# chaofengc/FeMaSR

Hardware: AMD Instinct MI355X
Metric: SR output megapixels/sec at x4 (128->512) (higher is better)
Workload: dtype f32 (1x1 convs / nn.Linear: every fp32 operand split EXACTLY into three bf16 terms, six partial products, fp32 accumulation on the bf16 matrix pipe - closer to fp64 than the fp32 fmaf chain, bit-identical to the CPU oracle)

## Files before the change

femasr_amd/_lib.py:

```python
import ctypes
import os

_HERE = os.path.dirname(os.path.abspath(__file__))
SO_PATH = os.path.join(_HERE, 'csrc', 'libfemasr_hip.so')

c_int, c_i64, c_f32 = ctypes.c_int, ctypes.c_int64, ctypes.c_float
vp, szt = ctypes.c_void_p, ctypes.c_size_t


class FemasrError(RuntimeError):
    pass


MAX_CODEBOOKS = 3


class Config(ctypes.Structure):
    _fields_ = ([(n, ctypes.c_int32) for n in ('in_channel', 'gt_resolution', 'lq_stage', 'scale_factor', 'use_quantize',
                                               'use_residual', 'n_codebooks')] +
                [(n, ctypes.c_int32 * MAX_CODEBOOKS) for n in ('codebook_scale', 'n_e', 'e_dim')] +
                [('device', ctypes.c_int32)])


class ConvArgs(ctypes.Structure):
    _fields_ = [
        ('in_', vp), ('B', ctypes.c_int32), ('H', ctypes.c_int32), ('W', ctypes.c_int32), ('Cin', ctypes.c_int32),
        ('w', vp), ('bias', vp),
        ('Cout', ctypes.c_int32), ('ksz', ctypes.c_int32), ('stride', ctypes.c_int32), ('pad', ctypes.c_int32),
        ('up2', ctypes.c_int32), ('prologue', ctypes.c_int32),
        ('pro_a', vp), ('pro_b', vp), ('pro_c', vp),
        ('act', ctypes.c_int32),
        ('res1', vp), ('res2', vp), ('out', vp),
        ('Ho', ctypes.c_int32), ('Wo', ctypes.c_int32),
        ('w_bf16x3', vp), ('gn_part', vp), ('w_up2', vp), ('w_wino', vp), ('fast_act', ctypes.c_int32), ('in_add', vp), ('w_bf16s', vp),
    ]


ABI_VERSION = 106
PRO_NONE, PRO_GN_SILU, PRO_LN = 0, 1, 2
ACT_NONE, ACT_GELU, ACT_RELU = 0, 1, 2

SIGNATURES = {
    'femasr_last_error': (ctypes.c_char_p, []),
    'femasr_version': (c_int, []),
    'femasr_create': (c_int, [ctypes.POINTER(Config), ctypes.POINTER(vp)]),
    'femasr_destroy': (None, [vp]),
    'femasr_num_weights': (c_int, [vp]),
    'femasr_weight_info': (c_int, [vp, c_int, ctypes.POINTER(ctypes.c_char_p), ctypes.POINTER(c_i64 * 4), ctypes.POINTER(c_int)]),
    'femasr_set_weight': (c_int, [vp, ctypes.c_char_p, vp, ctypes.POINTER(c_i64), c_int]),
    'femasr_finalize_weights': (c_int, [vp]),
    'femasr_set_streams': (c_int, [vp, c_int]),
    'femasr_workspace_bytes': (c_int, [vp, c_int, c_int, c_int, c_int, ctypes.POINTER(szt)]),
    'femasr_forward_shapes': (c_int, [vp, c_int, c_int, c_int, ctypes.POINTER(c_int), ctypes.POINTER(c_int), ctypes.POINTER(c_int),
                                      ctypes.POINTER(c_int * MAX_CODEBOOKS), ctypes.POINTER(c_int * MAX_CODEBOOKS)]),
    'femasr_forward': (c_int, [vp, vp, vp, c_int, c_int, c_int, c_int, vp, vp, vp, szt]),
    'femasr_forward_u8': (c_int, [vp, vp, vp, c_int, c_int, c_int, c_int, c_int, vp, vp, vp, szt]),
    'femasr_pad_u8hwc_to_nhwc': (c_int, [vp, vp, c_int, c_int, c_int, c_int, c_int, c_int, vp]),
    'femasr_crop_nhwc_to_u8hwc': (c_int, [vp, vp, c_int, c_int, c_int, c_int, c_int, c_int, vp]),
    'femasr_decode_workspace_bytes': (c_int, [vp, c_int, c_int, c_int, ctypes.POINTER(szt)]),
    'femasr_decode_indices': (c_int, [vp, vp, vp, c_int, c_int, c_int, vp, vp, szt]),
    'femasr_profile_enable': (c_int, [vp, c_int]),
    'femasr_profile_reset': (c_int, [vp]),
    'femasr_profile_slots': (c_int, [vp]),
    'femasr_profile_name': (ctypes.c_char_p, [vp, c_int]),
    'femasr_profile_get': (c_int, [vp, c_int, ctypes.POINTER(ctypes.c_double), ctypes.POINTER(c_i64),
                                   ctypes.POINTER(ctypes.c_double), ctypes.POINTER(ctypes.c_double)]),
    'femasr_pad_nchw_to_nhwc': (c_int, [vp, vp, c_int, c_int, c_int, c_int, c_int, c_int, vp]),
    'femasr_crop_nhwc_to_nchw': (c_int, [vp, vp, c_int, c_int, c_int, c_int, c_int, c_int, vp]),
    'femasr_conv2d': (c_int, [vp, ctypes.POINTER(ConvArgs)]),
    'femasr_gn_coeffs': (c_int, [vp, vp, c_int, c_int, c_int, c_int, c_int, vp, vp, c_f32, vp, vp, vp]),
    'femasr_gn_coeffs_from_partials': (c_int, [vp, vp, c_int, c_int, c_int, c_int, c_int, c_int, vp, vp, c_f32, vp, vp]),
    'femasr_ln_stats': (c_int, [vp, vp, c_i64, c_int, c_f32, vp]),
    'femasr_layernorm': (c_int, [vp, vp, c_i64, c_int, vp, vp, c_f32, vp]),
    'femasr_gn_scratch_bytes': (szt, [c_int, c_int, c_int, c_int, c_int]),
    'femasr_window_attention': (c_int, [vp, vp, c_int, c_int, c_int, c_int, c_int, c_int, vp, vp]),
    'femasr_vq': (c_int, [vp, vp, c_i64, c_int, vp, vp, vp, c_int, vp, vp, vp]),
    'femasr_row_sqsum': (c_int, [vp, vp, c_i64, c_int, vp]),
    'femasr_vq_twopass_ok': (c_int, [c_int, c_int]),
    'femasr_vq_aux_bytes': (szt, [c_int, c_int]),
    'femasr_vq_prepare': (c_int, [vp, vp, vp, c_int, c_int, vp]),
    'femasr_vq_scratch_bytes': (szt, [c_i64, c_int]),
    'femasr_vq_twopass': (c_int, [vp, vp, c_i64, c_int, vp, vp, vp, c_int, vp, vp, vp]),
    'femasr_vq_candidates': (c_int, [vp, vp, c_i64, c_int, vp, vp, c_int, vp, vp]),
    'femasr_codebook_gather': (c_int, [vp, vp, c_i64, c_int, vp, c_int, vp]),
    'femasr_extract_tiles': (c_int, [vp, vp, c_int, c_int, c_int, c_int, vp, c_int, c_int, c_int, vp]),
    'femasr_paste_tiles': (c_int, [vp, vp, c_int, c_int, c_int, c_int, c_int, vp, c_int, c_int, c_int, vp]),
    'femasr_extract_tiles_u8': (c_int, [vp, vp, c_int, c_int, c_int, vp, c_int, c_int, c_int, vp]),
    'femasr_paste_tiles_u8': (c_int, [vp, vp, c_int, c_int, c_int, c_int, vp, c_int, c_int, c_int, vp]),
    'femasr_blend_tiles': (c_int, [vp, vp, vp, c_int, c_int, c_int, c_int, c_int, c_int, c_int, c_int, vp]),
    'femasr_blend_tiles_u8': (c_int, [vp, vp, vp, c_int, c_int, c_int, c_int, c_int, c_int, c_int, vp]),
    'femasr_concat_resize': (c_int, [vp, vp, c_int, vp, c_int, c_int, c_int, c_int, c_int, c_int, vp]),
    'femasr_repack_oihw': (c_int, [vp, vp, c_int, c_int, c_int, c_int, vp]),
    'femasr_packed_weight_floats': (szt, [c_int, c_int, c_int, c_int]),
    'femasr_up2_weight_floats': (szt, [c_int, c_int]),
    'femasr_wino_weight_floats': (szt, [c_int, c_int]),
    'femasr_repack_oihw_wino': (c_int, [vp, vp, c_int, c_int, vp]),
    'femasr_wino_up2_weight_floats': (szt, [c_int, c_int]),
    'femasr_repack_oihw_wino_up2': (c_int, [vp, vp, c_int, c_int, vp]),
    'femasr_repack_oihw_up2': (c_int, [vp, vp, c_int, c_int, vp]),
    'femasr_packed_weight_bf16x3_bytes': (szt, [c_int, c_int, c_int, c_int]),
    'femasr_repack_oihw_bf16x3': (c_int, [vp, vp, c_int, c_int, c_int, c_int, vp]),
    'femasr_set_decoder_math': (c_int, [vp, c_int]),
    'femasr_set_linear_math': (c_int, [vp, c_int]),
    'femasr_packed_weight_bf16s_bytes': (szt, [c_int, c_int]),
    'femasr_repack_k1_bf16s': (c_int, [vp, vp, c_int, c_int, vp]),
    'femasr_packed_weight_conv3x3_bf16s_bytes': (szt, [c_int, c_int]),
    'femasr_repack_oihw_bf16s': (c_int, [vp, vp, c_int, c_int, vp]),
    'femasr_gn_silu_apply': (c_int, [vp, vp, c_int, c_int, c_int, c_int, vp, vp, vp]),
    'femasr_image_u8_to_f32': (c_int, [vp, vp, c_int, c_int, c_int, vp]),
    'femasr_image_f32_to_u8': (c_int, [vp, vp, c_int, c_int, c_int, vp]),
    'femasr_lpips_create': (c_int, [c_int, c_int, ctypes.POINTER(vp)]),
    'femasr_lpips_destroy': (None, [vp]),
    'femasr_lpips_set_weight': (c_int, [vp, ctypes.c_char_p, vp, ctypes.POINTER(c_i64), c_int]),
    'femasr_lpips_finalize_weights': (c_int, [vp]),
    'femasr_lpips_workspace_bytes': (c_int, [vp, c_int, c_int, c_int, ctypes.POINTER(szt)]),
    'femasr_lpips_forward': (c_int, [vp, vp, vp, vp, c_int, c_int, c_int, vp, vp, vp, szt]),
    'femasr_lpips_scale_input': (c_int, [vp, vp, vp, c_int, c_int, c_int, vp]),
    'femasr_lpips_tap_partials': (c_int, [c_int, c_int]),
    'femasr_lpips_tap': (c_int, [vp, vp, c_int, c_int, c_int, c_int, vp, c_int, vp, vp]),
    'femasr_lpips_finalize': (c_int, [vp, vp, c_int, c_int, ctypes.POINTER(ctypes.c_int32), vp, vp]),
    'femasr_psnr_ssim_workspace_bytes': (c_int, [c_int, c_int, c_int, c_int, c_int, ctypes.POINTER(szt)]),
    'femasr_psnr_ssim': (c_int, [vp, vp, vp, c_int, c_int, c_int, c_int, c_int, vp, vp, vp, vp, szt]),
    'femasr_ssim_window': (c_int, [ctypes.POINTER(ctypes.c_double)]),
    'femasr_imresize_workspace_bytes': (c_int, [c_int, c_int, c_int, c_int, c_int, ctypes.POINTER(szt)]),
    'femasr_imresize': (c_int, [vp, vp, c_int, c_int, c_int, c_int, c_int, c_int, vp, vp, c_int, vp, vp, c_int, vp, vp, szt]),
    'femasr_niqe_workspace_bytes': (c_int, [c_int, c_int, c_int, c_int, ctypes.POINTER(szt)]),
    'femasr_niqe_plane_offsets': (c_int, [c_int, c_int, c_int, c_int, ctypes.POINTER(szt * 4)]),
    'femasr_niqe_features': (c_int, [vp, vp, c_int, c_int, c_int, c_int, vp, vp, vp, vp, c_int, vp, vp, c_int, vp, vp, vp, szt]),
    'femasr_clock_probe': (c_int, [vp, c_int, vp]),
    'femasr_clock_probe_entries': (c_int, []),
}
DEBUG_SIGNATURES = {
    'femasr_debug_set_wino_limits': (c_int, [vp, c_int, c_int]),
    'femasr_debug_mfma_bf16': (c_int, [vp, vp, vp, vp, c_int, vp]),
    'femasr_gemm_force_config': (c_int, [c_int]),
    'femasr_conv_small_launch_blocks': (c_int, [c_int]),
    'femasr_debug_conv_variant_name': (c_int, [ctypes.POINTER(ConvArgs), ctypes.c_char_p, c_int]),
}

_lib = None


def load():
    global _lib
    if _lib is not None:
        return _lib
    if not os.path.exists(SO_PATH):
        raise FemasrError(
            f'{SO_PATH} not found: the HIP extension is not built. Run `python femasr_amd/csrc/build.py` '
            '(needs hipcc; cross-compiles gfx950 without a GPU). There is no CPU fallback.')
    lib = ctypes.CDLL(SO_PATH)
    lib.femasr_version.restype = c_int
    if lib.femasr_version() != ABI_VERSION:
        raise FemasrError(f'{SO_PATH} reports ABI version {lib.femasr_version()}, this binding is written for {ABI_VERSION} '
                          '(femasr_conv_args layout): rebuild with `python femasr_amd/csrc/build.py --force`')
    for name, (res, args) in list(SIGNATURES.items()) + list(DEBUG_SIGNATURES.items()):
        fn = getattr(lib, name)
        fn.restype = res
        fn.argtypes = args
    _lib = lib
    return lib


def check(rc):
    if rc != 0:
        msg = load().femasr_last_error()
        raise FemasrError(f'libfemasr_hip error {rc}: {msg.decode() if msg else "?"}')


def ptr(t):
    return None if t is None else ctypes.c_void_p(t.data_ptr())
```

femasr_amd/csrc/common.h:

```cpp
#pragma once
#include <hip/hip_runtime.h>
#include <stdint.h>
#include <stddef.h>
#include "../../include/femasr_hip_debug.h"

int femasr_set_error(int code, const char *fmt, ...);
#define FEMASR_CHECK_HIP(expr)                                                            \
    do {                                                                                  \
        hipError_t _e = (expr);                                                           \
        if (_e != hipSuccess)                                                             \
            return femasr_set_error(FEMASR_ERR_HIP, "%s failed: %s (%s:%d)", #expr,       \
                                    hipGetErrorString(_e), __FILE__, __LINE__);           \
    } while (0)
#define FEMASR_REQUIRE(cond, ...)                                                         \
    do {                                                                                  \
        if (!(cond)) return femasr_set_error(FEMASR_ERR_INVALID, __VA_ARGS__);            \
    } while (0)

inline int femasr_allow_dynamic_lds(const void *kern, unsigned long long *devs, size_t bytes)
{
    int dev = 0;
    FEMASR_CHECK_HIP(hipGetDevice(&dev));
    if (dev < 0 || dev >= 64 || !((__atomic_load_n(devs, __ATOMIC_ACQUIRE) >> dev) & 1ull)) {
        FEMASR_CHECK_HIP(hipFuncSetAttribute(kern, hipFuncAttributeMaxDynamicSharedMemorySize, (int)bytes));
        if (dev >= 0 && dev < 64) __atomic_fetch_or(devs, 1ull << dev, __ATOMIC_RELEASE);
    }
    return FEMASR_OK;
}
#define FEMASR_CHECK(expr) do { const int _rc = (expr); if (_rc != FEMASR_OK) return _rc; } while (0)

struct conv_vq_epilogue {
    const float *zz;
    const float *ee;
    float *part;
    int nblk;
};
int femasr_conv2d_launch(hipStream_t s, const femasr_conv_args *a, const conv_vq_epilogue *vq,
                         int *variant_out, double *flops_out);
int femasr_conv2d_pick_variant(const femasr_conv_args *a);
int femasr_conv_variant_count();
const char *femasr_conv_variant_name(int v);
bool femasr_conv_halo_eligible(const femasr_conv_args *a);
inline bool femasr_gn_fusable(int cout) { const int cg = cout / 32; return cout % 32 == 0 && cg >= 1 && cg <= 32 && (cg & (cg - 1)) == 0; }

inline size_t femasr_compact_weight_floats(int O, int I, int kh, int kw)
{
    return (O <= 4 && kh == 3 && kw == 3 && (I % 32) == 0) ? (size_t)I * 9 * 4 : 0;
}

bool femasr_gemm_eligible(const femasr_conv_args *a);
int femasr_gemm_launch(hipStream_t s, const femasr_conv_args *a, const conv_vq_epilogue *vq, int *variant_out, double *flops_out);
int femasr_gemm_variant_count();
int femasr_gemm_pick_variant(const femasr_conv_args *a, bool vq);
const char *femasr_gemm_variant_name(int v);
int femasr_repack_k1(hipStream_t s, const float *in, int O, int I, float *out);

bool femasr_gemm_bf16s_shape_ok(const femasr_conv_args *a);
bool femasr_conv3x3_bf16s_shape_ok(const femasr_conv_args *a);
int femasr_gemm_bf16s_launch(hipStream_t s, const femasr_conv_args *a, const void *w_bf16s, int *variant_out, double *flops_out);
int femasr_gemm_bf16s_variant_count();
int femasr_gemm_bf16s_pick_variant(const femasr_conv_args *a);
const char *femasr_gemm_bf16s_variant_name(int v);

constexpr int FEMASR_WINO_LOG2_TOTAL = 31, FEMASR_WINO_LOG2_IMAGE = 27;
bool femasr_conv_wino_shape_ok(const femasr_conv_args *a);
bool femasr_conv_wino_shape_ok_lim(const femasr_conv_args *a, int log2_total, int log2_image);
int femasr_conv_wino_gn_tiles(int H, int W);
int femasr_conv_wino_launch(hipStream_t s, const femasr_conv_args *a, int *variant_out, double *flops_out);
int femasr_conv_wino_variant_count();
int femasr_conv_wino_pick_variant(const femasr_conv_args *a);
const char *femasr_conv_wino_variant_name(int v);
bool femasr_conv_wino_up2_shape_ok(const femasr_conv_args *a);
bool femasr_conv_wino_up2_shape_ok_lim(const femasr_conv_args *a, int log2_total, int log2_image);
int femasr_conv_wino_up2_launch(hipStream_t s, const femasr_conv_args *a, double *flops_out);
const char *femasr_conv_wino_up2_variant_name();

bool femasr_conv_bf16x3_eligible(const femasr_conv_args *a);
bool femasr_conv_bf16x3_shape_ok(const femasr_conv_args *a);
int femasr_conv_bf16x3_launch(hipStream_t s, const femasr_conv_args *a, int *variant_out, double *flops_out);
int femasr_conv_bf16x3_variant_count();
int femasr_conv_bf16x3_pick_variant(const femasr_conv_args *a);
const char *femasr_conv_bf16x3_variant_name(int v);

enum ConvForm {
    CONV_DIRECT,
    CONV_BF16X3,
    CONV_WINO,
    CONV_WINO_UP2,
    CONV_SPLIT,
    CONV_FORM_COUNT
};
int femasr_conv_form_variant_count(ConvForm f);
const char *femasr_conv_form_variant_name(ConvForm f, int v);
int femasr_conv_form_launch(hipStream_t s, ConvForm f, const femasr_conv_args *a, int *slot_out, double *flops_out);
```

femasr_amd/csrc/conv_common.h:

```cpp
#pragma once
#include "common.h"

namespace {

struct ConvParams {
    const float *in, *w, *bias, *pro_a, *pro_b, *pro_c, *res1, *res2;
    const float *w_wino;
    const float *w_up2;
    float *out;
    const float *vq_zz, *vq_ee;
    float *vq_part;
    int vq_nblk;
    double *gn_part;
    int B, H, W, Cin, Cout, ksz, stride, pad, up2, act, Ho, Wo;
    int M, K, nchunks, taps, MB, NB, NT32;
    int tilesX, tilesY;
    int kperm;
};

constexpr int BK = 32;
constexpr int ALD = BK + 1;

__device__ __forceinline__ float4 ld4(const float *p) { return *reinterpret_cast<const float4 *>(p); }

typedef __attribute__((address_space(1))) const float *gcptr_f32;
typedef __attribute__((address_space(1))) float *gptr_f32;

__device__ __forceinline__ unsigned long long uniform_u64(unsigned long long a)
{
    const unsigned lo = __builtin_amdgcn_readfirstlane((unsigned)a), hi = __builtin_amdgcn_readfirstlane((unsigned)(a >> 32));
    return ((unsigned long long)hi << 32) | lo;
}
__device__ __forceinline__ float ldg_u32(const float *ubase, unsigned byteoff)
{
    const unsigned long long a = uniform_u64(reinterpret_cast<unsigned long long>(ubase));
    return *reinterpret_cast<gcptr_f32>(a + byteoff);
}
__device__ __forceinline__ void stg_u32(float *ubase, unsigned byteoff, float v)
{
    const unsigned long long a = uniform_u64(reinterpret_cast<unsigned long long>(ubase));
    *reinterpret_cast<gptr_f32>(a + byteoff) = v;
}

typedef float f32x4_t __attribute__((ext_vector_type(4)));
__device__ __forceinline__ f32x4_t ldg4_u32(const float *ubase, unsigned byteoff)
{
    const unsigned long long a = uniform_u64(reinterpret_cast<unsigned long long>(ubase));
    return *reinterpret_cast<__attribute__((address_space(1))) const f32x4_t *>(a + byteoff);
}
__device__ __forceinline__ void stg4_u32(float *ubase, unsigned byteoff, f32x4_t v)
{
    const unsigned long long a = uniform_u64(reinterpret_cast<unsigned long long>(ubase));
    *reinterpret_cast<__attribute__((address_space(1))) f32x4_t *>(a + byteoff) = v;
}
constexpr int TPITCH = 36;
constexpr int TSCRATCH = 32 * TPITCH;

__device__ __forceinline__ float f4get(const float4 &v, int i) { return i == 0 ? v.x : (i == 1 ? v.y : (i == 2 ? v.z : v.w)); }

__device__ __forceinline__ int wtile(int n0, int t, int nt32)
{
    const int idx = (n0 >> 5) + t;
    return idx < nt32 ? idx : nt32 - 1;
}

__device__ __forceinline__ int xcd_remap(int bid, int nblk)
{
    const int q = nblk >> 3, r = nblk & 7, xcd = bid & 7, within = bid >> 3;
    return (xcd < r ? xcd * (q + 1) : r * (q + 1) + (xcd - r) * q) + within;
}


}
```

femasr_amd/csrc/kernels_conv.hip:

```cpp
#include "conv_common.h"
#include <atomic>
#include <stdlib.h>
#include <type_traits>
#include "detmath.h"

typedef float f32x16 __attribute__((ext_vector_type(16)));

namespace {


template <int BM, int BN, int WM, int WN, int PRO, bool CINVEC>
__global__ __launch_bounds__(WM * WN * 64, (WM * WN == 8) ? 4 : 2) void conv_igemm_kernel(const ConvParams p)
{
    constexpr int NT = WM * WN * 64;
    constexpr int TM = BM / (WM * 32), TN = BN / (WN * 32);
    constexpr int RSTEP = NT / 8;
    constexpr int AROWS = BM / RSTEP;
    static_assert((WM * WN == 4 || WM * WN == 8) && TM >= 1 && TN >= 1 && AROWS >= 1, "tile config");
    static_assert(CINVEC || PRO == FEMASR_PRO_NONE, "generic-Cin path has no prologue");
    static_assert(PRO != FEMASR_PRO_LN, "LayerNorm is a separate pass (femasr_layernorm)");

    extern __shared__ __attribute__((aligned(16))) float smem[];
    float *As = smem;

    const int t = threadIdx.x, lane = t & 63;
    const int wave = __builtin_amdgcn_readfirstlane(t >> 6);
    const int wm = wave / WN, wn = wave % WN;
    const int L = xcd_remap(blockIdx.x, p.MB * p.NB);
    const int nb = L % p.NB, mb = L / p.NB;
    const int m0 = mb * BM, n0 = nb * BN;

    const int kq = t & 7, mrow = t >> 3;
    int rn[AROWS], riy[AROWS], rix[AROWS];
    const int HoWo = p.Ho * p.Wo;
#pragma unroll
    for (int j = 0; j < AROWS; ++j) {
        const int r = m0 + mrow + RSTEP * j;
        if (r < p.M) {
            const int n = r / HoWo, rem = r - n * HoWo;
            const int oy = rem / p.Wo, ox = rem - oy * p.Wo;
            rn[j] = n;
            riy[j] = oy * p.stride - p.pad;
            rix[j] = ox * p.stride - p.pad;
        } else {
            rn[j] = 0;
            riy[j] = -(1 << 28);
            rix[j] = -(1 << 28);
        }
    }
    const int Hv = p.up2 ? 2 * p.H : p.H, Wv = p.up2 ? 2 * p.W : p.W;

    float4 ra[AROWS], rga[AROWS], rgb[AROWS];
    unsigned amask = 0;

    auto load_chunk = [&](int c) {
        amask = 0;
        if (CINVEC) {
            const int cc = c / p.taps, tap = c - cc * p.taps, c0 = cc * BK + 4 * kq;
            const int ky = tap / p.ksz, kx = tap - ky * p.ksz;
#pragma unroll
            for (int j = 0; j < AROWS; ++j) {
                const int iy = riy[j] + ky, ix = rix[j] + kx;
                const bool ok = (iy >= 0) & (iy < Hv) & (ix >= 0) & (ix < Wv);
                const int sy = p.up2 ? (iy >> 1) : iy, sx = p.up2 ? (ix >> 1) : ix;
                const size_t off = ok ? ((((size_t)rn[j] * p.H + sy) * p.W + sx) * p.Cin + c0) : (size_t)0;
                ra[j] = ld4(p.in + off);
                if (PRO == FEMASR_PRO_GN_SILU) {
                    rga[j] = ld4(p.pro_a + (size_t)rn[j] * p.Cin + c0);
                    rgb[j] = ld4(p.pro_b + (size_t)rn[j] * p.Cin + c0);
                }
                amask |= (ok ? 1u : 0u) << j;
            }
        } else {
#pragma unroll
            for (int j = 0; j < AROWS; ++j) {
                float v[4];
#pragma unroll
                for (int e = 0; e < 4; ++e) {
                    const int k = c * BK + 4 * kq + e;
                    v[e] = 0.f;
                    if (k < p.K) {
                        const int tap = k / p.Cin, ci = k - tap * p.Cin;
                        const int ky = tap / p.ksz, kx = tap - ky * p.ksz;
                        const int iy = riy[j] + ky, ix = rix[j] + kx;
                        if ((iy >= 0) & (iy < Hv) & (ix >= 0) & (ix < Wv)) {
                            const int sy = p.up2 ? (iy >> 1) : iy, sx = p.up2 ? (ix >> 1) : ix;
                            v[e] = p.in[(((size_t)rn[j] * p.H + sy) * p.W + sx) * p.Cin + ci];
                        }
                    }
                }
                ra[j] = make_float4(v[0], v[1], v[2], v[3]);
                amask |= 1u << j;
            }
        }
    };

    auto store_chunk = [&](int buf) {
        float *Ab = As + buf * BM * ALD;
#pragma unroll
        for (int j = 0; j < AROWS; ++j) {
            asm volatile("" : "+v"(ra[j].x), "+v"(ra[j].y), "+v"(ra[j].z), "+v"(ra[j].w));
            float4 v = ra[j];
            if (PRO == FEMASR_PRO_GN_SILU) {
                v.x = det_silu(__builtin_fmaf(v.x, rga[j].x, rgb[j].x));
                v.y = det_silu(__builtin_fmaf(v.y, rga[j].y, rgb[j].y));
                v.z = det_silu(__builtin_fmaf(v.z, rga[j].z, rgb[j].z));
                v.w = det_silu(__builtin_fmaf(v.w, rga[j].w, rgb[j].w));
            }
            if (!(amask & (1u << j))) v = make_float4(0.f, 0.f, 0.f, 0.f);
            float *dst = Ab + (mrow + RSTEP * j) * ALD + 4 * kq;
            dst[0] = v.x;
            dst[1] = v.y;
            dst[2] = v.z;
            dst[3] = v.w;
        }
    };

    f32x16 acc[TM][TN];
#pragma unroll
    for (int i = 0; i < TM; ++i)
#pragma unroll
        for (int j = 0; j < TN; ++j)
#pragma unroll
            for (int r = 0; r < 16; ++r) acc[i][j][r] = 0.f;

    const bool kp = p.kperm != 0;
    const int wgs = kp ? 256 : 4;
    const float *wl[TN];
#pragma unroll
    for (int j = 0; j < TN; ++j) {
        const size_t tile = (size_t)wtile(n0, wn * TN + j, p.NT32);
        wl[j] = kp ? p.w + tile * 1024 + lane * 4 : p.w + ((tile * 64 + lane) << 4);
    }
    const size_t wstride = (size_t)p.NT32 << 10;

    load_chunk(0);
    float4 bc[TN], bn[TN];
#pragma unroll
    for (int j = 0; j < TN; ++j) bc[j] = ld4(wl[j]);
    store_chunk(0);
    __syncthreads();

    const int arow = (wm * TM * 32 + (lane & 31)) * ALD + (kp ? 4 : 1) * (lane >> 5);
    auto kofs = [&](int kk) -> int { return kp ? 8 * (kk >> 2) + (kk & 3) : 2 * kk; };

    for (int c = 0; c < p.nchunks; ++c) {
        const int buf = c & 1;
        const int cn = (c + 1) < p.nchunks ? c + 1 : c;
        const float *Ab = As + buf * BM * ALD + arow;
        float af[2][TM];
#pragma unroll
        for (int i = 0; i < TM; ++i) af[0][i] = Ab[i * 32 * ALD];
#pragma unroll
        for (int kk = 0; kk < BK / 2; ++kk) {
            const int cur = kk & 1, nxt = cur ^ 1, g = kk >> 2, e = kk & 3;
            if (e == 0) {
                if (g < 3) {
#pragma unroll
                    for (int j = 0; j < TN; ++j) bn[j] = ld4(wl[j] + (size_t)c * wstride + wgs * (g + 1));
                } else {
#pragma unroll
                    for (int j = 0; j < TN; ++j) bn[j] = ld4(wl[j] + (size_t)cn * wstride);
                }
                if (kk == 0) load_chunk(cn);
            }
            if (kk + 1 < BK / 2) {
#pragma unroll
                for (int i = 0; i < TM; ++i) af[nxt][i] = Ab[i * 32 * ALD + kofs(kk + 1)];
            }
            __builtin_amdgcn_sched_barrier(0);
#pragma unroll
            for (int i = 0; i < TM; ++i)
#pragma unroll
                for (int j = 0; j < TN; ++j)
                    acc[i][j] = __builtin_amdgcn_mfma_f32_32x32x2f32(af[cur][i], f4get(bc[j], e), acc[i][j], 0, 0, 0);
            if (e == 3) {
#pragma unroll
                for (int j = 0; j < TN; ++j) bc[j] = bn[j];
            }
            __builtin_amdgcn_sched_barrier(0);
        }
        store_chunk(buf ^ 1);
        __syncthreads();
    }

    {
        const unsigned loff = (unsigned)((lane >> 5) * 4) * (unsigned)p.Cout + (unsigned)(lane & 31);
        const bool full = (m0 + BM <= p.M) && (n0 + BN <= p.Cout);
        const float *ra = p.res1 ? p.res1 : p.res2, *rb = (p.res1 && p.res2) ? p.res2 : nullptr;
        auto uoff = [&](int i, int j, int r) -> size_t {
            return (size_t)(m0 + (wm * TM + i) * 32 + (r & 3) + 8 * (r >> 2)) * p.Cout + (n0 + (wn * TN + j) * 32);
        };
        auto epilogue = [&](auto nres_c, auto full_c) {
            constexpr int NRES = decltype(nres_c)::value;
            constexpr bool FULL = decltype(full_c)::value;
            constexpr int DEPTH = NRES == 1 ? 2 : 1;
            float rbuf[DEPTH][NRES > 0 ? NRES : 1][16];
            auto ok_u = [&](int i, int j, int r) -> bool {
                return FULL || ((m0 + (wm * TM + i) * 32 + (r & 3) + 8 * (r >> 2)) < p.M && (n0 + (wn * TN + j) * 32) < p.Cout);
            };
            auto ok_l = [&](int i, int j, int r) -> bool {
                return FULL || ((m0 + (wm * TM + i) * 32 + (r & 3) + 8 * (r >> 2) + 4 * (lane >> 5)) < p.M &&
                                (n0 + (wn * TN + j) * 32 + (lane & 31)) < p.Cout);
            };
            auto issue = [&](int tl, int slot) {
#pragma unroll
                for (int r = 0; r < 16; ++r) {
                    const int i = tl / TN, j = tl % TN;
                    const size_t ou = ok_u(i, j, r) ? uoff(i, j, r) : (size_t)m0 * p.Cout + n0;
                    const unsigned lo = ok_l(i, j, r) ? 4u * loff : 0u;
                    if (NRES >= 1) rbuf[slot][0][r] = ldg_u32(ra + ou, lo);
                    if (NRES >= 2) rbuf[slot][NRES >= 2 ? 1 : 0][r] = ldg_u32(rb + ou, lo);
                }
            };
            if (NRES > 0) issue(0, 0);
#pragma unroll
            for (int tl = 0; tl < TM * TN; ++tl) {
                const int i = tl / TN, j = tl % TN;
                if (DEPTH == 2 && tl + 1 < TM * TN) issue(tl + 1, (tl + 1) & 1);
                const int col = n0 + (wn * TN + j) * 32 + (lane & 31);
                const float bv = (FULL || col < p.Cout) ? p.bias[FULL ? col : (col < p.Cout ? col : 0)] : 0.f;
#pragma unroll
                for (int r = 0; r < 16; ++r) {
                    float v = acc[i][j][r] + bv;
                    if (p.act == FEMASR_ACT_GELU) v = det_gelu(v);
                    else if (p.act == FEMASR_ACT_RELU) v = v > 0.f ? v : 0.f;
                    if (NRES >= 1) v = v + rbuf[tl % DEPTH][0][r];
                    if (NRES >= 2) v = v + rbuf[tl % DEPTH][NRES >= 2 ? 1 : 0][r];
                    if (ok_l(i, j, r)) stg_u32(p.out + uoff(i, j, r), 4u * loff, v);
                }
                if (NRES > 0 && DEPTH == 1 && tl + 1 < TM * TN) issue(tl + 1, 0);
            }
        };
        constexpr bool VEC_FITS = (WM * WN * TSCRATCH) <= (2 * BM * ALD);
        auto epilogue_vec = [&](auto nres_c) {
            constexpr int NRES = decltype(nres_c)::value;
            constexpr int DEPTH = NRES == 1 ? 2 : 1;
            float *T = smem + wave * TSCRATCH;
            const int trow = lane >> 3, tq = lane & 7;
            const unsigned lvec = 4u * ((unsigned)trow * (unsigned)p.Cout + 4u * (unsigned)tq);
            auto urow = [&](int i, int j, int k) -> size_t {
                return (size_t)(m0 + (wm * TM + i) * 32 + 8 * k) * p.Cout + (n0 + (wn * TN + j) * 32);
            };
            f32x4_t rbuf[DEPTH][NRES > 0 ? NRES : 1][4];
            auto issue = [&](int tl, int slot) {
#pragma unroll
                for (int k = 0; k < 4; ++k) {
                    if (NRES >= 1) rbuf[slot][0][k] = ldg4_u32(ra + urow(tl / TN, tl % TN, k), lvec);
                    if (NRES >= 2) rbuf[slot][NRES >= 2 ? 1 : 0][k] = ldg4_u32(rb + urow(tl / TN, tl % TN, k), lvec);
                }
            };
            if (NRES > 0) issue(0, 0);
#pragma unroll
            for (int tl = 0; tl < TM * TN; ++tl) {
                const int i = tl / TN, j = tl % TN;
                if (DEPTH == 2 && tl + 1 < TM * TN) issue(tl + 1, (tl + 1) & 1);
#pragma unroll
                for (int r = 0; r < 16; ++r) T[((r & 3) + 8 * (r >> 2) + 4 * (lane >> 5)) * TPITCH + (lane & 31)] = acc[i][j][r];
                const f32x4_t b4 = ldg4_u32(p.bias + n0 + (wn * TN + j) * 32, 16u * (unsigned)tq);
#pragma unroll
                for (int k = 0; k < 4; ++k) {
                    const float4 a4 = *reinterpret_cast<const float4 *>(T + (trow + 8 * k) * TPITCH + 4 * tq);
                    float v[4] = {a4.x + b4[0], a4.y + b4[1], a4.z + b4[2], a4.w + b4[3]};
                    if (p.act == FEMASR_ACT_GELU) {
                        const det_f32x2 g0 = det_gelu2(det_f32x2{v[0], v[1]}), g1 = det_gelu2(det_f32x2{v[2], v[3]});
                        v[0] = g0[0]; v[1] = g0[1]; v[2] = g1[0]; v[3] = g1[1];
                    } else if (p.act == FEMASR_ACT_RELU) {
#pragma unroll
                        for (int e = 0; e < 4; ++e) v[e] = v[e] > 0.f ? v[e] : 0.f;
                    }
#pragma unroll
                    for (int e = 0; e < 4; ++e) {
                        if (NRES >= 1) v[e] = v[e] + rbuf[tl % DEPTH][0][k][e];
                        if (NRES >= 2) v[e] = v[e] + rbuf[tl % DEPTH][NRES >= 2 ? 1 : 0][k][e];
                    }
                    stg4_u32(p.out + urow(i, j, k), lvec, f32x4_t{v[0], v[1], v[2], v[3]});
                }
                if (NRES > 0 && DEPTH == 1 && tl + 1 < TM * TN) issue(tl + 1, 0);
            }
        };
        using I0 = std::integral_constant<int, 0>;
        using I1 = std::integral_constant<int, 1>;
        using I2 = std::integral_constant<int, 2>;
        if (VEC_FITS && full && (p.Cout & 3) == 0) {
            if (rb) epilogue_vec(I2{}); else if (ra) epilogue_vec(I1{}); else epilogue_vec(I0{});
        } else if (rb) { if (full) epilogue(I2{}, std::true_type{}); else epilogue(I2{}, std::false_type{}); }
        else if (ra) { if (full) epilogue(I1{}, std::true_type{}); else epilogue(I1{}, std::false_type{}); }
        else { if (full) epilogue(I0{}, std::true_type{}); else epilogue(I0{}, std::false_type{}); }
    }
}

template <int BN, int WM, int WN, int PRO, bool UP2>
__global__ __launch_bounds__(WM * WN * 64, (WM * WN == 8) ? 4 : 2) void conv3x3_halo_kernel(const ConvParams p)
{
    constexpr int BM = 128, TW = 16;
    constexpr int PH = 10, PW = 18, PP = PH * PW;
    constexpr int NTAP = UP2 ? 4 : 9, SC = UP2 ? 2 : 1;
    static_assert(!(UP2 && PRO != FEMASR_PRO_NONE), "the phase kernel has no prologue");
    constexpr int NT = WM * WN * 64;
    constexpr int PUNITS = (PP * 8 + NT - 1) / NT;
    constexpr int PROWS = NT / 8;
    constexpr int TM = BM / (WM * 32), TN = BN / (WN * 32);
    static_assert((WM * WN == 4 || WM * WN == 8) && TM >= 1 && TN >= 1, "tile config");
    static_assert(PRO != FEMASR_PRO_LN, "no LayerNorm prologue on 3x3 convs");
    static_assert(2 + PUNITS <= BK / 2, "patch slices must fit the 16 k-pair steps of one tap");

    extern __shared__ __attribute__((aligned(16))) float smem[];
    constexpr int PSZ = (((PP + 1) * ALD + 3) / 4) * 4;
    float *Ps = smem;

    const int t = threadIdx.x, lane = t & 63, wave = t >> 6;
    const int wm = wave / WN, wn = wave % WN;
    const int L = xcd_remap(blockIdx.x, p.MB * p.NB);
    const int nb = L % p.NB;
    int tile = L / p.NB;
    const int pha = UP2 ? (tile >> 1) & 1 : 0, phb = UP2 ? tile & 1 : 0;
    if (UP2) tile >>= 2;
    const int tx = tile % p.tilesX;
    tile /= p.tilesX;
    const int ty = tile % p.tilesY;
    const int n = tile / p.tilesY;
    const int oy0 = ty * 8, ox0 = tx * TW, n0 = nb * BN;
    const int sy0 = oy0 - 1, sx0 = ox0 - 1;

    const int kq = t & 7;
    unsigned poff[PUNITS];
    unsigned pmask = 0;
#pragma unroll
    for (int i = 0; i < PUNITS; ++i) {
        const int pix = (t >> 3) + PROWS * i;
        const int ppy = pix / PW, ppx = pix - ppy * PW;
        const int sy = sy0 + ppy, sx = sx0 + ppx;
        const bool ok = (pix < PP) & (sy >= 0) & (sy < p.H) & (sx >= 0) & (sx < p.W);
        poff[i] = ok ? (unsigned)((((size_t)n * p.H + sy) * p.W + sx) * p.Cin + 4 * kq) : 0u;
        pmask |= (ok ? 1u : 0u) << i;
    }

    float4 rp[PUNITS], ga, gb;

    auto load_patch = [&](int cc) {
#pragma unroll
        for (int i = 0; i < PUNITS; ++i) rp[i] = ld4(p.in + (size_t)poff[i] + (size_t)cc * BK);
        if (PRO == FEMASR_PRO_GN_SILU) {
            ga = ld4(p.pro_a + (size_t)n * p.Cin + cc * BK + 4 * kq);
            gb = ld4(p.pro_b + (size_t)n * p.Cin + cc * BK + 4 * kq);
        }
    };
    auto store_patch_unit = [&](int buf, int i) {
        float *Pb = Ps + buf * PSZ;
        const int pix = (t >> 3) + PROWS * i;
        if (PP % PROWS != 0 && i == PUNITS - 1 && pix >= PP) return;
        float4 v = rp[i];
        if (PRO == FEMASR_PRO_GN_SILU) {
            const det_f32x2 s0 = det_silu2(__builtin_elementwise_fma(det_f32x2{v.x, v.y}, det_f32x2{ga.x, ga.y}, det_f32x2{gb.x, gb.y}));
            const det_f32x2 s1 = det_silu2(__builtin_elementwise_fma(det_f32x2{v.z, v.w}, det_f32x2{ga.z, ga.w}, det_f32x2{gb.z, gb.w}));
            v = make_float4(s0[0], s0[1], s1[0], s1[1]);
        }
        if (!(pmask & (1u << i))) v = make_float4(0.f, 0.f, 0.f, 0.f);
        float *dst = Pb + pix * ALD + 4 * kq;
        dst[0] = v.x;
        dst[1] = v.y;
        dst[2] = v.z;
        dst[3] = v.w;
    };

    f32x16 acc[TM][TN];
#pragma unroll
    for (int i = 0; i < TM; ++i)
#pragma unroll
        for (int j = 0; j < TN; ++j)
#pragma unroll
            for (int r = 0; r < 16; ++r) acc[i][j][r] = 0.f;

    const size_t wstride = (size_t)p.NT32 << 10;
    const float *wbase = UP2 ? p.w_up2 + (size_t)(pha * 2 + phb) * ((size_t)(p.Cin / BK) * NTAP) * wstride : p.w;
    const float *wl[TN];
#pragma unroll
    for (int j = 0; j < TN; ++j)
        wl[j] = wbase + ((((size_t)wtile(n0, wn * TN + j, p.NT32)) * 64 + lane) << 4);

    const int ncc = p.Cin / BK;
    load_patch(0);
    float4 bc[TN], bn[TN];
#pragma unroll
    for (int j = 0; j < TN; ++j) bc[j] = ld4(wl[j]);
#pragma unroll
    for (int i = 0; i < PUNITS; ++i) store_patch_unit(0, i);
    __syncthreads();

    int py[TM], px;
    {
        const int m = wm * TM * 32 + (lane & 31);
        px = m & 15;
#pragma unroll
        for (int i = 0; i < TM; ++i) py[i] = (m >> 4) + 2 * i;
    }

    const int abase = ((py[0] + pha) * PW + px + phb) * ALD;
    auto patch_idx = [&](int tap, int (&idx)[TM]) {
        const int ky = UP2 ? tap >> 1 : tap / 3, kx = UP2 ? tap & 1 : tap - ky * 3;
#pragma unroll
        for (int i = 0; i < TM; ++i) idx[i] = abase + ((2 * i + ky) * PW + kx) * ALD;
    };

    const int nq = ncc * NTAP;
    for (int cc = 0; cc < ncc; ++cc) {
        const float *Pb = Ps + (cc & 1) * PSZ + (lane >> 5);
        const int ccn = cc + 1 < ncc ? cc + 1 : cc;
        const bool more = cc + 1 < ncc;
        const int nbuf = (cc + 1) & 1;
        float af[2][TM];
        int aidx[TM];
        patch_idx(0, aidx);
#pragma unroll
        for (int i = 0; i < TM; ++i) af[0][i] = Pb[aidx[i]];
#pragma unroll
        for (int tap = 0; tap < NTAP; ++tap) {
            const int q = cc * NTAP + tap;
            const size_t qn = (size_t)(q + 1 < nq ? q + 1 : nq - 1);
            int nidx[TM];
            patch_idx(tap < NTAP - 1 ? tap + 1 : NTAP - 1, nidx);
#pragma unroll
            for (int kk = 0; kk < BK / 2; ++kk) {
                const int cur = kk & 1, nxt = cur ^ 1, g = kk >> 2, e = kk & 3;
                if (e == 0) {
                    if (g < 3) {
#pragma unroll
                        for (int j = 0; j < TN; ++j) bn[j] = ld4(wl[j] + (size_t)q * wstride + 4 * (g + 1));
                    } else {
#pragma unroll
                        for (int j = 0; j < TN; ++j) bn[j] = ld4(wl[j] + qn * wstride);
                    }
                    if (tap == 0 && kk == 0) load_patch(ccn);
                }
                if (kk + 1 < BK / 2) {
#pragma unroll
                    for (int i = 0; i < TM; ++i) af[nxt][i] = Pb[aidx[i] + 2 * (kk + 1)];
                } else if (tap < NTAP - 1) {
#pragma unroll
                    for (int i = 0; i < TM; ++i) af[nxt][i] = Pb[nidx[i]];
                }
                __builtin_amdgcn_sched_barrier(0);
#pragma unroll
                for (int i = 0; i < TM; ++i)
#pragma unroll
                    for (int j = 0; j < TN; ++j)
                        acc[i][j] = __builtin_amdgcn_mfma_f32_32x32x2f32(af[cur][i], f4get(bc[j], e), acc[i][j], 0, 0, 0);
                if (e == 3) {
#pragma unroll
                    for (int j = 0; j < TN; ++j) bc[j] = bn[j];
                }
                if (tap == 1 && kk >= 2 && kk < 2 + PUNITS && more) store_patch_unit(nbuf, kk - 2);
                __builtin_amdgcn_sched_barrier(0);
            }
#pragma unroll
            for (int i = 0; i < TM; ++i) aidx[i] = nidx[i];
        }
        __syncthreads();
    }

    const int Hl = UP2 ? p.H : p.Ho, Wl = UP2 ? p.W : p.Wo;
    const bool full = (oy0 + 8 <= Hl) && (ox0 + TW <= Wl) && (n0 + BN <= p.Cout);
    const float *ra = p.res1 ? p.res1 : p.res2, *rb = (p.res1 && p.res2) ? p.res2 : nullptr;
    const size_t obase = (((size_t)n * p.Ho + SC * oy0 + pha) * p.Wo + SC * ox0 + phb) * p.Cout + n0;
    const unsigned loff = (unsigned)(SC * 4 * (lane >> 5)) * (unsigned)p.Cout + (unsigned)(lane & 31);
    const int wmu = __builtin_amdgcn_readfirstlane(wm), wnu = __builtin_amdgcn_readfirstlane(wn);
    auto uoff = [&](int i, int j, int r) -> size_t {
        return obase + (size_t)(SC * ((2 * (wmu * TM + i) + (r >> 3)) * p.Wo + (r & 3) + 8 * ((r >> 2) & 1))) * p.Cout + (wnu * TN + j) * 32;
    };
    const bool gnp = p.gn_part != nullptr;
    double gs[TM][TN], gss[TM][TN];
#pragma unroll
    for (int i = 0; i < TM; ++i)
#pragma unroll
        for (int j = 0; j < TN; ++j) { gs[i][j] = 0.0; gss[i][j] = 0.0; }
    auto epilogue = [&](auto nres_c, auto full_c) {
        constexpr int NRES = decltype(nres_c)::value;
        constexpr bool FULL = decltype(full_c)::value;
        constexpr int DEPTH = NRES == 1 ? 2 : 1;
        float rbuf[DEPTH][NRES > 0 ? NRES : 1][16];
        auto ok_u = [&](int i, int j, int r) -> bool {
            return FULL || ((oy0 + 2 * (wmu * TM + i) + (r >> 3)) < Hl && (ox0 + (r & 3) + 8 * ((r >> 2) & 1)) < Wl &&
                            (n0 + (wnu * TN + j) * 32) < p.Cout);
        };
        auto ok_l = [&](int i, int j, int r) -> bool {
            return FULL || ((oy0 + 2 * (wmu * TM + i) + (r >> 3)) < Hl &&
                            (ox0 + (r & 3) + 8 * ((r >> 2) & 1) + 4 * (lane >> 5)) < Wl &&
                            (n0 + (wnu * TN + j) * 32 + (lane & 31)) < p.Cout);
        };
        auto issue = [&](int tl, int slot) {
#pragma unroll
            for (int r = 0; r < 16; ++r) {
                const int i = tl / TN, j = tl % TN;
                const size_t ou = ok_u(i, j, r) ? uoff(i, j, r) : obase;
                const unsigned lo = ok_l(i, j, r) ? 4u * loff : 0u;
                if (NRES >= 1) rbuf[slot][0][r] = ldg_u32(ra + ou, lo);
                if (NRES >= 2) rbuf[slot][NRES >= 2 ? 1 : 0][r] = ldg_u32(rb + ou, lo);
            }
        };
        if (NRES > 0) issue(0, 0);
#pragma unroll
        for (int tl = 0; tl < TM * TN; ++tl) {
            const int i = tl / TN, j = tl % TN;
            if (DEPTH == 2 && tl + 1 < TM * TN) issue(tl + 1, (tl + 1) & 1);
            const int col = n0 + (wnu * TN + j) * 32 + (lane & 31);
            const float bv = (FULL || col < p.Cout) ? p.bias[FULL ? col : (col < p.Cout ? col : 0)] : 0.f;
#pragma unroll
            for (int r = 0; r < 16; ++r) {
                float v = acc[i][j][r] + bv;
                if (p.act == FEMASR_ACT_RELU) v = v > 0.f ? v : 0.f;
                if (NRES >= 1) v = v + rbuf[tl % DEPTH][0][r];
                if (NRES >= 2) v = v + rbuf[tl % DEPTH][NRES >= 2 ? 1 : 0][r];
                if (ok_l(i, j, r)) {
                    stg_u32(p.out + uoff(i, j, r), 4u * loff, v);
                    if (gnp) {
                        const double d = (double)v;
                        gs[i][j] = gs[i][j] + d;
                        gss[i][j] = __builtin_fma(d, d, gss[i][j]);
                    }
                }
            }
            if (NRES > 0 && DEPTH == 1 && tl + 1 < TM * TN) issue(tl + 1, 0);
        }
    };
    using I0 = std::integral_constant<int, 0>;
    using I1 = std::integral_constant<int, 1>;
    using I2 = std::integral_constant<int, 2>;
    if (rb) { if (full) epilogue(I2{}, std::true_type{}); else epilogue(I2{}, std::false_type{}); }
    else if (ra) { if (full) epilogue(I1{}, std::true_type{}); else epilogue(I1{}, std::false_type{}); }
    else { if (full) epilogue(I0{}, std::true_type{}); else epilogue(I0{}, std::false_type{}); }

    if (gnp) {
        const int cg = p.Cout >> 5;
        const int gpb = BN / cg;
        double *red = reinterpret_cast<double *>(smem);
#pragma unroll
        for (int i = 0; i < TM; ++i)
#pragma unroll
            for (int j = 0; j < TN; ++j) {
                double a = gs[i][j] + __shfl_xor(gs[i][j], 32, 64);
                double b = gss[i][j] + __shfl_xor(gss[i][j], 32, 64);
                for (int d = 1; d < cg; d <<= 1) {
                    a = a + __shfl_xor(a, d, 64);
                    b = b + __shfl_xor(b, d, 64);
                }
                const int cl = (wnu * TN + j) * 32 + (lane & 31);
                if (lane < 32 && (cl & (cg - 1)) == 0) {
                    double *dst = red + ((size_t)(wmu * TM + i) * gpb + cl / cg) * 2;
                    dst[0] = a;
                    dst[1] = b;
                }
            }
        __syncthreads();
        if (t < gpb) {
            const int g = n0 / cg + t;
            if (g < 32) {
                double S = red[(0 * gpb + t) * 2], SS = red[(0 * gpb + t) * 2 + 1];
#pragma unroll
                for (int q = 1; q < 4; ++q) {
                    S = S + red[((size_t)q * gpb + t) * 2];
                    SS = SS + red[((size_t)q * gpb + t) * 2 + 1];
                }
                const size_t tidx = (size_t)n * p.tilesY * p.tilesX + (size_t)ty * p.tilesX + tx;
                double *dst = p.gn_part + ((UP2 ? tidx * 4 + (pha * 2 + phb) : tidx) * 32 + g) * 2;
                dst[0] = S;
                dst[1] = SS;
            }
        }
    }
}

constexpr int C3_TH = 8, C3_TW = 32, C3_PW = C3_TW + 2, C3_PP = (C3_TH + 2) * C3_PW, C3_PITCH = 36;

__global__ __launch_bounds__(256) void conv3x3_cout3_kernel(const ConvParams p, const float *__restrict__ wc)
{
    extern __shared__ __attribute__((aligned(16))) float smem[];
    const int t = threadIdx.x;
    int tile = blockIdx.x;
    const int tx = tile % p.tilesX;
    tile /= p.tilesX;
    const int ty = tile % p.tilesY;
    const int n = tile / p.tilesY;
    const int oy0 = ty * C3_TH, ox0 = tx * C3_TW;
    const int py = t >> 5, px = t & 31;
    float acc0 = 0.f, acc1 = 0.f, acc2 = 0.f;
    const int ncb = p.Cin >> 5;
    constexpr int NU = (C3_PP * 8 + 255) / 256;
    unsigned uoff[NU];
    unsigned umask = 0;
#pragma unroll
    for (int i = 0; i < NU; ++i) {
        const int u = t + 256 * i, pix = u >> 3, kq = u & 7;
        const int sy = oy0 - 1 + pix / C3_PW, sx = ox0 - 1 + pix % C3_PW;
        const bool ok = u < C3_PP * 8 && sy >= 0 && sy < p.H && sx >= 0 && sx < p.W;
        uoff[i] = ok ? (unsigned)((((size_t)n * p.H + sy) * p.W + sx) * p.Cin + 4 * kq) : 0u;
        umask |= (ok ? 1u : 0u) << i;
    }
    float4 ru[NU];
    auto fetch = [&](int cb) {
#pragma unroll
        for (int i = 0; i < NU; ++i) ru[i] = ld4(p.in + (size_t)uoff[i] + cb * 32);
    };
    auto stage = [&]() {
#pragma unroll
        for (int i = 0; i < NU; ++i) {
            const int u = t + 256 * i;
            if (u < C3_PP * 8)
                *reinterpret_cast<float4 *>(smem + (u >> 3) * C3_PITCH + 4 * (u & 7)) = (umask >> i) & 1u ? ru[i] : make_float4(0.f, 0.f, 0.f, 0.f);
        }
    };
    fetch(0);
    for (int cb = 0; cb < ncb; ++cb) {
        if (cb) __syncthreads();
        stage();
        __syncthreads();
        fetch(cb + 1 < ncb ? cb + 1 : cb);
#pragma unroll
        for (int tap = 0; tap < 9; ++tap) {
            const float *src = smem + ((py + tap / 3) * C3_PW + px + tap % 3) * C3_PITCH;
            const float *w = wc + ((size_t)(cb * 9 + tap) * 32) * 4;
#pragma unroll
            for (int c4 = 0; c4 < 8; ++c4) {
                const float4 x4 = *reinterpret_cast<const float4 *>(src + 4 * c4);
                const float xs[4] = {x4.x, x4.y, x4.z, x4.w};
#pragma unroll
                for (int e = 0; e < 4; ++e) {
                    const float *wk = w + (4 * c4 + e) * 4;
                    acc0 = __builtin_fmaf(xs[e], wk[0], acc0);
                    acc1 = __builtin_fmaf(xs[e], wk[1], acc1);
                    acc2 = __builtin_fmaf(xs[e], wk[2], acc2);
                }
            }
        }
    }
    const int oy = oy0 + py, ox = ox0 + px;
    if (oy < p.Ho && ox < p.Wo) {
        const size_t o = (((size_t)n * p.Ho + oy) * p.Wo + ox) * 3;
        float v[3] = {acc0 + p.bias[0], acc1 + p.bias[1], acc2 + p.bias[2]};
#pragma unroll
        for (int c = 0; c < 3; ++c) {
            if (p.res1) v[c] = v[c] + p.res1[o + c];
            if (p.res2) v[c] = v[c] + p.res2[o + c];
            p.out[o + c] = v[c];
        }
    }
}

template <bool UP2>
constexpr size_t halo_lds_bytes()
{
    return (size_t)(2 * ((((180 + 1) * ALD + 3) / 4) * 4)) * sizeof(float);
}

template <int BM>
constexpr size_t conv_lds_bytes() { return (size_t)(2 * BM * ALD) * sizeof(float); }

struct Variant {
    const char *name;
    int bm, bn;
    void (*kern)(const ConvParams);
    size_t lds;
    unsigned long long attr_devs;
    int threads;
};

#define FEMASR_VARIANT(BM, BN, WM, WN, PRO, VEC)                                                            \
    { "conv_igemm<" #BM "x" #BN "," #PRO ",cinvec=" #VEC ",waves=" #WM "x" #WN ">",                         \
      BM, BN, conv_igemm_kernel<BM, BN, WM, WN, PRO, VEC>, conv_lds_bytes<BM>(), 0ull, WM * WN * 64 }
#define FEMASR_HALO(BN, WM, WN, PRO, UP2)                                                                  \
    { "conv3x3_halo<8x16x" #BN "," #PRO ",up2=" #UP2 ",waves=" #WM "x" #WN ">", 128, BN,                   \
      conv3x3_halo_kernel<BN, WM, WN, PRO, UP2>, halo_lds_bytes<UP2>(), 0ull, WM * WN * 64 }

Variant g_variants[] = {
    FEMASR_VARIANT(128, 128, 4, 2, FEMASR_PRO_NONE, true),
    FEMASR_VARIANT(128, 128, 4, 2, FEMASR_PRO_GN_SILU, true),
    FEMASR_VARIANT(128, 64, 4, 2, FEMASR_PRO_NONE, true),
    FEMASR_VARIANT(128, 64, 4, 2, FEMASR_PRO_GN_SILU, true),
    FEMASR_VARIANT(128, 32, 4, 1, FEMASR_PRO_NONE, true),
    FEMASR_VARIANT(128, 32, 4, 1, FEMASR_PRO_GN_SILU, true),
    FEMASR_VARIANT(128, 128, 4, 2, FEMASR_PRO_NONE, false),
    FEMASR_VARIANT(128, 64, 4, 2, FEMASR_PRO_NONE, false),
    FEMASR_VARIANT(128, 32, 4, 1, FEMASR_PRO_NONE, false),
    FEMASR_HALO(128, 2, 2, FEMASR_PRO_NONE, false),
    FEMASR_HALO(128, 2, 2, FEMASR_PRO_GN_SILU, false),
    FEMASR_HALO(128, 2, 2, FEMASR_PRO_NONE, true),
    FEMASR_HALO(64, 2, 2, FEMASR_PRO_NONE, false),
    FEMASR_HALO(64, 2, 2, FEMASR_PRO_GN_SILU, false),
    FEMASR_HALO(64, 2, 2, FEMASR_PRO_NONE, true),
    FEMASR_HALO(32, 4, 1, FEMASR_PRO_NONE, false),
    FEMASR_HALO(32, 4, 1, FEMASR_PRO_GN_SILU, false),
    FEMASR_HALO(32, 4, 1, FEMASR_PRO_NONE, true),
    { "conv3x3_cout3<8x32,valu>", 256, 4, nullptr, (size_t)C3_PP * C3_PITCH * sizeof(float), 0ull, 256 },
};
constexpr int kNumVariants = sizeof(g_variants) / sizeof(g_variants[0]);
constexpr int kFirstHalo = 9;

std::atomic<int> g_small_blocks{-1};
int small_blocks_default()
{
    static const int v = [] {
        int dev = 0, cus = 0;
        if (hipGetDevice(&dev) == hipSuccess && hipDeviceGetAttribute(&cus, hipDeviceAttributeMultiprocessorCount, dev) == hipSuccess && cus > 0)
            return cus + cus / 2;
        return 384;
    }();
    return v;
}
int small_launch_blocks()
{
    const int v = g_small_blocks.load(std::memory_order_relaxed);
    return v >= 0 ? v : small_blocks_default();
}

int pick_variant(const femasr_conv_args *a, int Ho, int Wo)
{
    const bool vec = (a->Cin % BK) == 0;
    int cls = a->Cout > 64 ? 0 : (a->Cout > 32 ? 1 : 2);
    const bool halo = femasr_conv_halo_eligible(a);
    if (cls == 0 && (halo || vec)) {
        const long long mb = halo ? (long long)a->B * (((a->up2 ? a->W : Wo) + 15) / 16) * (((a->up2 ? a->H : Ho) + 7) / 8) * (a->up2 ? 4 : 1)
                                  : ((long long)a->B * Ho * Wo + 127) / 128;
        if (mb * ((a->Cout + 127) / 128) < small_launch_blocks()) cls = 1;
    }
    if (halo) return kFirstHalo + cls * 3 + (a->up2 ? 2 : a->prologue);
    if (!vec) return 6 + cls;
    return cls * 2 + a->prologue;
}

}

extern "C" int femasr_conv_small_launch_blocks(int blocks)
{
    const int prev = small_launch_blocks();
    g_small_blocks.store(blocks >= 0 ? blocks : -1, std::memory_order_relaxed);
    return prev;
}

bool femasr_conv_halo_eligible(const femasr_conv_args *a)
{
    return a->ksz == 3 && a->stride == 1 && a->pad == 1 && (a->Cin % BK) == 0 && a->prologue != FEMASR_PRO_LN &&
           (a->act == FEMASR_ACT_NONE || a->act == FEMASR_ACT_RELU) && !(a->up2 && a->prologue != FEMASR_PRO_NONE) &&
           (size_t)a->B * a->H * a->W * a->Cin < ((size_t)1 << 31);
}

int femasr_conv_variant_count() { return kNumVariants + femasr_gemm_variant_count(); }
const char *femasr_conv_variant_name(int v)
{
    if (v >= kNumVariants) return femasr_gemm_variant_name(v - kNumVariants);
    return v >= 0 ? g_variants[v].name : "?";
}

static bool conv_is_cout3(const femasr_conv_args *a)
{
    return femasr_conv_halo_eligible(a) && a->Cout == 3 && !a->up2 && a->prologue == FEMASR_PRO_NONE && a->act == FEMASR_ACT_NONE && !a->gn_part;
}

int femasr_conv2d_pick_variant(const femasr_conv_args *a)
{
    if (femasr_gemm_eligible(a)) return kNumVariants + femasr_gemm_pick_variant(a, false);
    if (conv_is_cout3(a)) return kNumVariants - 1;
    const int Hv = a->up2 ? 2 * a->H : a->H, Wv = a->up2 ? 2 * a->W : a->W;
    return pick_variant(a, (Hv + 2 * a->pad - a->ksz) / a->stride + 1, (Wv + 2 * a->pad - a->ksz) / a->stride + 1);
}

int femasr_conv2d_launch(hipStream_t s, const femasr_conv_args *a, const conv_vq_epilogue *vq,
                         int *variant_out, double *flops_out)
{
    FEMASR_REQUIRE(a && a->in && a->w && a->B > 0 && a->H > 0 && a->W > 0 && a->Cin > 0 && a->Cout > 0,
                   "conv2d: null pointer or empty shape");
    FEMASR_REQUIRE(vq || (a->bias && a->out), "conv2d: bias/out must be set");
    FEMASR_REQUIRE(a->ksz >= 1 && a->ksz <= 11 && (a->stride == 1 || a->stride == 2 || a->stride == 4) && a->pad >= 0,
                   "conv2d: unsupported ksz=%d stride=%d pad=%d", a->ksz, a->stride, a->pad);
    FEMASR_REQUIRE(a->act == FEMASR_ACT_NONE || a->act == FEMASR_ACT_GELU || a->act == FEMASR_ACT_RELU, "conv2d: bad activation %d", a->act);
    FEMASR_REQUIRE(a->prologue == FEMASR_PRO_NONE || a->prologue == FEMASR_PRO_GN_SILU,
                   "conv2d: bad prologue %d (LayerNorm is a separate pass: femasr_layernorm)", a->prologue);
    const int Hv = a->up2 ? 2 * a->H : a->H, Wv = a->up2 ? 2 * a->W : a->W;
    const int Ho = (Hv + 2 * a->pad - a->ksz) / a->stride + 1, Wo = (Wv + 2 * a->pad - a->ksz) / a->stride + 1;
    FEMASR_REQUIRE(Ho == a->Ho && Wo == a->Wo, "conv2d: Ho/Wo mismatch (%d,%d) vs expected (%d,%d)", a->Ho, a->Wo, Ho, Wo);
    if (femasr_gemm_eligible(a)) {
        int gv = 0;
        const int rc = femasr_gemm_launch(s, a, vq, &gv, flops_out);
        if (variant_out) *variant_out = kNumVariants + gv;
        return rc;
    }
    FEMASR_REQUIRE(!vq, "conv2d: the VQ epilogue needs a 1x1 layer with Cin %% 32 == 0");
    const bool vec = (a->Cin % BK) == 0;
    FEMASR_REQUIRE(vec || a->prologue == FEMASR_PRO_NONE, "conv2d: prologue needs Cin %% 32 == 0 (Cin=%d)", a->Cin);
    if (a->prologue == FEMASR_PRO_GN_SILU) FEMASR_REQUIRE(a->pro_a && a->pro_b, "conv2d: GN prologue needs a,b");
    const long long M = (long long)a->B * Ho * Wo;
    FEMASR_REQUIRE(M < (1ll << 31) - 256, "conv2d: too many output pixels");

    ConvParams p{};
    p.in = a->in; p.w = a->w; p.bias = a->bias; p.pro_a = a->pro_a; p.pro_b = a->pro_b; p.pro_c = a->pro_c;
    p.res1 = a->res1; p.res2 = a->res2; p.out = a->out;
    p.B = a->B; p.H = a->H; p.W = a->W; p.Cin = a->Cin; p.Cout = a->Cout; p.ksz = a->ksz; p.stride = a->stride;
    p.pad = a->pad; p.up2 = a->up2; p.act = a->act; p.Ho = Ho; p.Wo = Wo;
    p.M = (int)M; p.K = a->ksz * a->ksz * a->Cin; p.nchunks = (p.K + BK - 1) / BK; p.taps = a->ksz * a->ksz;
    p.NT32 = (a->Cout + 31) / 32;
    p.gn_part = a->gn_part;
    p.kperm = (a->ksz == 1 && vec) ? 1 : 0;
    if (conv_is_cout3(a)) {
        const size_t tail = femasr_compact_weight_floats(a->Cout, a->Cin, 3, 3);
        const float *wc = a->w + (size_t)p.nchunks * p.NT32 * 1024;
        p.tilesX = (Wo + C3_TW - 1) / C3_TW;
        p.tilesY = (Ho + C3_TH - 1) / C3_TH;
        (void)tail;
        hipLaunchKernelGGL(conv3x3_cout3_kernel, dim3((unsigned)(a->B * p.tilesX * p.tilesY)), dim3(256), (size_t)C3_PP * C3_PITCH * sizeof(float), s,
                           p, wc);
        FEMASR_CHECK_HIP(hipGetLastError());
        if (variant_out) *variant_out = kNumVariants - 1;
        if (flops_out) *flops_out = 2.0 * (double)M * (double)a->Cout * (double)p.K;
        return FEMASR_OK;
    }
    const int vi = pick_variant(a, Ho, Wo);
    Variant &v = g_variants[vi];
    p.MB = (p.M + v.bm - 1) / v.bm;
    p.NB = (p.Cout + v.bn - 1) / v.bn;
    const bool phases = vi >= kFirstHalo && a->up2;
    if (vi >= kFirstHalo) {
        p.tilesX = ((phases ? a->W : Wo) + 15) / 16;
        p.tilesY = ((phases ? a->H : Ho) + 7) / 8;
        p.MB = a->B * p.tilesX * p.tilesY * (phases ? 4 : 1);
    }
    FEMASR_REQUIRE(!phases || a->w_up2, "conv2d: a 3x3 nearest-x2 conv with Cin %% 32 == 0 needs w_up2 (femasr_repack_oihw_up2)");
    p.w_up2 = a->w_up2;
    FEMASR_REQUIRE(!a->gn_part || (vi >= kFirstHalo && femasr_gn_fusable(a->Cout)),
                   "conv2d: gn_part (fused GroupNorm partial moments) needs a 3x3 stride-1 halo conv and 32 | Cout, Cout/32 a power of two <= 32");
    FEMASR_CHECK(femasr_allow_dynamic_lds((const void *)v.kern, &v.attr_devs, v.lds));
    hipLaunchKernelGGL(v.kern, dim3((unsigned)(p.MB * p.NB)), dim3((unsigned)v.threads), v.lds, s, p);
    FEMASR_CHECK_HIP(hipGetLastError());
    if (variant_out) *variant_out = vi;
    if (flops_out) *flops_out = 2.0 * (double)M * (double)a->Cout * (double)p.K;
    return FEMASR_OK;
}
```

femasr_amd/csrc/kernels_misc.hip:

```cpp
#include "common.h"
#include "detmath.h"
#include <stdlib.h>
#include <string.h>
#include <type_traits>

namespace {

__device__ __forceinline__ float4 ld4(const float *p) { return *reinterpret_cast<const float4 *>(p); }

__device__ __forceinline__ int xcd_remap_misc(int bid, int nblk)
{
    const int q = nblk >> 3, r = nblk & 7, xcd = bid & 7, within = bid >> 3;
    return (xcd < r ? xcd * (q + 1) : r * (q + 1) + (xcd - r) * q) + within;
}

__global__ void pad_nchw_to_nhwc_kernel(const float *__restrict__ in, int B, int C, int H, int W, int Hp, int Wp,
                                        float *__restrict__ out, size_t total)
{
    for (size_t i = blockIdx.x * (size_t)blockDim.x + threadIdx.x; i < total; i += (size_t)gridDim.x * blockDim.x) {
        const int c = (int)(i % C);
        size_t r = i / C;
        const int x = (int)(r % Wp);
        r /= Wp;
        const int y = (int)(r % Hp);
// ... 843 lines not shown
    FEMASR_REQUIRE(x && gamma && beta && a && b && scratch, "gn_coeffs: null pointer");
    FEMASR_REQUIRE(B > 0 && H > 0 && W > 0 && G > 0 && C % G == 0, "gn_coeffs: bad shape C=%d G=%d", C, G);
    const int cg = C / G;
    hipStream_t s = (hipStream_t)stream;
    double *part = (double *)scratch;
    if (G == 32 && femasr_gn_fusable(C)) {
        const int tilesX = (W + 15) / 16, tilesY = (H + 7) / 8;
        hipLaunchKernelGGL(gn_tile_partials_kernel, dim3((unsigned)((size_t)B * tilesY * tilesX * (C / 32))), dim3(64), 0, s, x, H, W, C,
                           tilesX, tilesY, part);
        FEMASR_CHECK_HIP(hipGetLastError());
        return femasr_gn_coeffs_from_partials(stream, part, B, tilesX * tilesY, H, W, C, G, gamma, beta, eps, a, b);
    }
    const size_t total = (size_t)B * H * G;
    const dim3 grid((unsigned)((total + 255) / 256)), blk(256);
    if (cg == 8 && C % 4 == 0)
        hipLaunchKernelGGL(gn_rows_kernel<8>, grid, blk, 0, s, x, B, H, W, C, G, part);
    else if (cg == 4 && C % 4 == 0)
        hipLaunchKernelGGL(gn_rows_kernel<4>, grid, blk, 0, s, x, B, H, W, C, G, part);
    else if (cg == 2)
        hipLaunchKernelGGL(gn_rows_kernel<2>, grid, blk, 0, s, x, B, H, W, C, G, part);
    else
        hipLaunchKernelGGL(gn_rows_generic_kernel, grid, blk, 0, s, x, B, H, W, C, G, cg, part);
    FEMASR_CHECK_HIP(hipGetLastError());
    FEMASR_REQUIRE(G <= 256, "gn_coeffs: at most 256 groups");
    hipLaunchKernelGGL(gn_finalize_kernel, dim3((unsigned)B), dim3(256), (size_t)GN_SLAB * G * 2 * sizeof(double), s, part, B, H, H,
                       W, C, G, gamma, beta, eps, a, b);
    FEMASR_CHECK_HIP(hipGetLastError());
    return FEMASR_OK;
}

int femasr_gn_coeffs_from_partials(void *stream, const double *part, int B, int tiles, int H, int W, int C, int G,
                                   const float *gamma, const float *beta, float eps, float *a, float *b)
{
    FEMASR_REQUIRE(part && gamma && beta && a && b && B > 0 && tiles > 0 && H > 0 && W > 0, "gn_coeffs_from_partials: bad args");
    FEMASR_REQUIRE(G == 32 && C % G == 0, "gn_coeffs_from_partials: 32 groups");
    FEMASR_REQUIRE(C / G <= 64, "gn_coeffs_from_partials: at most 64 channels per group");
    hipLaunchKernelGGL(gn_finalize_partials_kernel, dim3((unsigned)(B * G)), dim3(64), 0, (hipStream_t)stream, part, tiles, H, W, C,
                       G, gamma, beta, eps, a, b);
    FEMASR_CHECK_HIP(hipGetLastError());
    return FEMASR_OK;
}

int femasr_gn_silu_apply(void *stream, const float *x, int B, int H, int W, int C, const float *a, const float *b, float *y)
{
    FEMASR_REQUIRE(x && a && b && y && B > 0 && H > 0 && W > 0 && C > 0 && (C % 4) == 0, "gn_silu_apply: bad args (C %% 4 == 0)");
    const size_t total4 = (size_t)B * H * W * (C / 4);
    hipLaunchKernelGGL(gn_silu_apply_kernel, dim3(grid_for(total4)), dim3(256), 0, (hipStream_t)stream, x, C, (long long)H * W, a, b, y, total4);
    FEMASR_CHECK_HIP(hipGetLastError());
    return FEMASR_OK;
}

int femasr_ln_stats(void *stream, const float *x, int64_t rows, int C, float eps, float *stats)
{
    FEMASR_REQUIRE(x && stats && rows > 0, "ln_stats: bad args");
    FEMASR_REQUIRE(C == 256, "ln_stats: only C == 256 (Swin embed_dim, femasr_arch.py:115) is built, got %d", C);
    hipLaunchKernelGGL(ln_stats_kernel, dim3((unsigned)((rows + 3) / 4)), dim3(256), 0, (hipStream_t)stream, x,
                       (long long)rows, eps, stats);
    FEMASR_CHECK_HIP(hipGetLastError());
    return FEMASR_OK;
}

int femasr_layernorm(void *stream, const float *x, int64_t rows, int C, const float *gamma, const float *beta, float eps, float *y)
{
    FEMASR_REQUIRE(x && y && gamma && beta && rows > 0, "layernorm: bad args");
    FEMASR_REQUIRE(C == 256, "layernorm: only C == 256 (Swin embed_dim, femasr_arch.py:115) is built, got %d", C);
    hipLaunchKernelGGL(layernorm_kernel, dim3((unsigned)((rows + 3) / 4)), dim3(256), 0, (hipStream_t)stream, x, (long long)rows,
                       gamma, beta, eps, y);
    FEMASR_CHECK_HIP(hipGetLastError());
    return FEMASR_OK;
}

int femasr_window_attention(void *stream, const float *qkv, int B, int H, int W, int C, int heads, int shift,
                            const float *table, float *out)
{
    FEMASR_REQUIRE(qkv && table && out && B > 0, "window_attention: bad args");
    FEMASR_REQUIRE(H % 8 == 0 && W % 8 == 0 && H >= 8 && W >= 8, "window_attention: H,W must be multiples of 8 (%d,%d)", H, W);
    FEMASR_REQUIRE(heads > 0 && heads <= 8 && C == heads * ATT_HD, "window_attention: head_dim must be 32, at most 8 heads (C=%d heads=%d)", C, heads);
    FEMASR_REQUIRE(shift >= 0 && shift < 8, "window_attention: bad shift %d", shift);
    FEMASR_REQUIRE((size_t)H * W * 3 * C < ((size_t)1 << 30), "window_attention: image too large for 32-bit offsets");
    const size_t total = (size_t)B * (H / 8) * (W / 8) * heads;
    FEMASR_REQUIRE(total < ((size_t)1 << 31), "window_attention: too many (window, head) units");
    hipLaunchKernelGGL(window_attention_reg_kernel<1>, dim3((unsigned)total), dim3(64), 0, (hipStream_t)stream, qkv, B, H, W, C, heads, shift, table,
                       out, (int)total);
    FEMASR_CHECK_HIP(hipGetLastError());
    return FEMASR_OK;
}

int femasr_row_sqsum(void *stream, const float *x, int64_t rows, int D, float *out)
{
    FEMASR_REQUIRE(x && out && rows > 0 && D > 0 && D % 4 == 0, "row_sqsum: bad args");
    hipLaunchKernelGGL(row_sqsum_kernel, dim3((unsigned)((rows + 63) / 64)), dim3(64), 0, (hipStream_t)stream, x,
                       (long long)rows, D, out);
    FEMASR_CHECK_HIP(hipGetLastError());
    return FEMASR_OK;
}

int femasr_vq(void *stream, const float *z, int64_t M, int D, const float *cb, const float *cbT, const float *ee,
              int n_e, int64_t *idx, float *zq, void *scratch)
{
    FEMASR_REQUIRE(z && cb && cbT && ee && idx && zq && scratch && M > 0, "vq: bad args");
    FEMASR_REQUIRE(D % 32 == 0 && n_e % 128 == 0, "vq: needs e_dim %% 32 == 0 and n_e %% 128 == 0 (D=%d n_e=%d)", D, n_e);
    FEMASR_REQUIRE(M < (1ll << 31) - 256, "vq: too many rows");
    hipStream_t s = (hipStream_t)stream;
    float *zz = (float *)scratch;
    float *part = zz + ((M + 63) / 64) * 64;
    const int nblk = n_e / 128;
    int rc = femasr_row_sqsum(stream, z, M, D, zz);
    if (rc) return rc;
    femasr_conv_args a{};
    a.in = z; a.B = 1; a.H = (int)M; a.W = 1; a.Cin = D; a.w = cbT; a.bias = nullptr; a.Cout = n_e;
    a.ksz = 1; a.stride = 1; a.pad = 0; a.up2 = 0; a.prologue = FEMASR_PRO_NONE; a.act = 0;
    a.Ho = (int)M; a.Wo = 1;
    conv_vq_epilogue ep{zz, ee, part, nblk};
    rc = femasr_conv2d_launch(s, &a, &ep, nullptr, nullptr);
    if (rc) return rc;
    hipLaunchKernelGGL(vq_finalize_kernel, dim3((unsigned)((M + 3) / 4)), dim3(256), 0, s, z, (long long)M, D, cb, part,
                       nblk, n_e, (long long *)idx, zq);
    FEMASR_CHECK_HIP(hipGetLastError());
    return FEMASR_OK;
}

int femasr_codebook_gather(void *stream, const int64_t *idx, int64_t M, int D, const float *cb, int n_e, float *zq)
{
    FEMASR_REQUIRE(idx && cb && zq && M > 0 && D % 4 == 0 && n_e > 0, "codebook_gather: bad args");
    hipLaunchKernelGGL(codebook_gather_kernel, dim3((unsigned)((M + 3) / 4)), dim3(256), 0, (hipStream_t)stream,
                       (const long long *)idx, (long long)M, D, cb, n_e, zq);
    FEMASR_CHECK_HIP(hipGetLastError());
    return FEMASR_OK;
}

int femasr_extract_tiles(void *stream, const float *in, int B, int C, int H, int W, const int32_t *yx_dev, int n, int th, int tw, float *out)
{
    FEMASR_REQUIRE(in && yx_dev && out && B > 0 && C > 0 && n > 0 && th > 0 && tw > 0 && th <= H && tw <= W, "extract_tiles: bad args");
    const size_t total = (size_t)n * B * C * th * tw;
    hipLaunchKernelGGL(extract_tiles_kernel, dim3(grid_for(total)), dim3(256), 0, (hipStream_t)stream, in, B, C, H, W, yx_dev, n, th, tw, out, total);
    FEMASR_CHECK_HIP(hipGetLastError());
    return FEMASR_OK;
}

int femasr_paste_tiles(void *stream, const float *tiles, int B, int C, int n, int th, int tw, const int32_t *rects_dev, int hmax,
                       int Ho, int Wo, float *out)
{
    FEMASR_REQUIRE(tiles && rects_dev && out && B > 0 && C > 0 && n > 0 && th > 0 && tw > 0 && hmax > 0 && hmax <= th, "paste_tiles: bad args");
    const size_t rows = (size_t)n * B * C * hmax;
    FEMASR_REQUIRE(rows < ((size_t)1 << 31), "paste_tiles: too many rows");
    hipLaunchKernelGGL(paste_tiles_kernel, dim3((unsigned)rows), dim3(256), 0, (hipStream_t)stream, tiles, B, C, th, tw, rects_dev, n, Ho, Wo, out, hmax);
    FEMASR_CHECK_HIP(hipGetLastError());
    return FEMASR_OK;
}

int femasr_extract_tiles_u8(void *stream, const uint8_t *in, int B, int H, int W, const int32_t *yx_dev, int n, int th, int tw, uint8_t *out)
{
    FEMASR_REQUIRE(in && yx_dev && out && B > 0 && n > 0 && th > 0 && tw > 0 && th <= H && tw <= W, "extract_tiles_u8: bad args");
    const size_t total = (size_t)n * B * th * tw * 3;
    hipLaunchKernelGGL(extract_tiles_u8_kernel, dim3(grid_for(total)), dim3(256), 0, (hipStream_t)stream, in, B, H, W, yx_dev, n, th, tw, out, total);
    FEMASR_CHECK_HIP(hipGetLastError());
    return FEMASR_OK;
}

int femasr_paste_tiles_u8(void *stream, const uint8_t *tiles, int B, int n, int th, int tw, const int32_t *rects_dev, int hmax, int Ho, int Wo, uint8_t *out)
{
    FEMASR_REQUIRE(tiles && rects_dev && out && B > 0 && n > 0 && th > 0 && tw > 0 && hmax > 0 && hmax <= th, "paste_tiles_u8: bad args");
    const size_t rows = (size_t)n * B * hmax;
    FEMASR_REQUIRE(rows < ((size_t)1 << 31), "paste_tiles_u8: too many rows");
    hipLaunchKernelGGL(paste_tiles_u8_kernel, dim3((unsigned)rows), dim3(256), 0, (hipStream_t)stream, tiles, B, th, tw, rects_dev, n, Ho, Wo, out, hmax);
    FEMASR_CHECK_HIP(hipGetLastError());
    return FEMASR_OK;
}

static int blend_launch(bool u8, void *stream, const uint64_t *tile_ptrs_dev, const int32_t *geom_dev, int n, int tiles_y, int tiles_x,
                        int pitch, int B, int C, int Ho, int Wo, void *out)
{
    const char *who = u8 ? "blend_tiles_u8" : "blend_tiles";
    FEMASR_REQUIRE(tile_ptrs_dev && geom_dev && out, "%s: null pointer", who);
    FEMASR_REQUIRE(n > 0 && B > 0 && C > 0 && tiles_y > 0 && tiles_x > 0 && pitch > 0 && Ho > 0 && Wo > 0, "%s: bad sizes", who);
    FEMASR_REQUIRE((long long)tiles_y * tiles_x == n, "%s: %d tiles given for a %d x %d grid", who, n, tiles_y, tiles_x);
    FEMASR_REQUIRE(tiles_x <= 65535, "%s: more than 65535 tile columns", who);
    const size_t rows = (size_t)B * C * Ho;
    FEMASR_REQUIRE(rows < ((size_t)1 << 31), "%s: too many rows", who);
    const dim3 grid((unsigned)rows, (unsigned)tiles_x);
    if (u8)
        hipLaunchKernelGGL(blend_tiles_kernel<true>, grid, dim3(256), 0, (hipStream_t)stream, (const unsigned long long *)tile_ptrs_dev,
                           geom_dev, tiles_y, tiles_x, pitch, 1, Ho, Wo, out);
    else
        hipLaunchKernelGGL(blend_tiles_kernel<false>, grid, dim3(256), 0, (hipStream_t)stream, (const unsigned long long *)tile_ptrs_dev,
                           geom_dev, tiles_y, tiles_x, pitch, C, Ho, Wo, out);
    FEMASR_CHECK_HIP(hipGetLastError());
    return FEMASR_OK;
}

int femasr_blend_tiles(void *stream, const uint64_t *tile_ptrs_dev, const int32_t *geom_dev, int n, int tiles_y, int tiles_x, int pitch,
                       int B, int C, int Ho, int Wo, float *out)
{
    return blend_launch(false, stream, tile_ptrs_dev, geom_dev, n, tiles_y, tiles_x, pitch, B, C, Ho, Wo, out);
}

int femasr_blend_tiles_u8(void *stream, const uint64_t *tile_ptrs_dev, const int32_t *geom_dev, int n, int tiles_y, int tiles_x, int pitch,
                          int B, int Ho, int Wo, uint8_t *out)
{
    return blend_launch(true, stream, tile_ptrs_dev, geom_dev, n, tiles_y, tiles_x, pitch, B, 1, Ho, Wo, out);
}

int femasr_concat_resize(void *stream, const float *a, int Ca, const float *b, int Hb, int Wb, int Cb, int B, int H, int W, float *out)
{
    FEMASR_REQUIRE(a && b && out && B > 0 && H > 0 && W > 0 && Hb > 0 && Wb > 0, "concat_resize: bad args");
    FEMASR_REQUIRE(Ca > 0 && Cb > 0 && Ca % 4 == 0 && Cb % 4 == 0, "concat_resize: channel counts must be multiples of 4 (%d, %d)", Ca, Cb);
    const size_t total4 = (size_t)B * H * W * ((Ca + Cb) / 4);
    hipLaunchKernelGGL(concat_resize_kernel, dim3(grid_for(total4)), dim3(256), 0, (hipStream_t)stream, a, Ca, b, Hb, Wb, Cb, H, W, out,
                       total4);
    FEMASR_CHECK_HIP(hipGetLastError());
    return FEMASR_OK;
}

size_t femasr_packed_weight_floats(int O, int I, int kh, int kw)
{
    if (O <= 0 || I <= 0 || kh <= 0 || kw <= 0) return 0;
    const size_t K = (size_t)I * kh * kw;
    return ((K + 31) / 32) * (size_t)((O + 31) / 32) * 1024 + femasr_compact_weight_floats(O, I, kh, kw);
}

int femasr_repack_oihw(void *stream, const float *in, int O, int I, int kh, int kw, float *out)
{
    FEMASR_REQUIRE(in && out && O > 0 && I > 0 && kh > 0 && kw > 0, "repack: bad args");
    if (kh == 1 && kw == 1 && (I % 32) == 0) return femasr_repack_k1((hipStream_t)stream, in, O, I, out);
    const size_t tail = femasr_compact_weight_floats(O, I, kh, kw);
    const size_t total = femasr_packed_weight_floats(O, I, kh, kw) - tail;
    if (tail) {
        hipLaunchKernelGGL(repack_compact_kernel, dim3(grid_for(tail)), dim3(256), 0, (hipStream_t)stream, in, O, I, kh, kw, out + total, tail);
        FEMASR_CHECK_HIP(hipGetLastError());
    }
    hipLaunchKernelGGL(repack_oihw_kernel, dim3(grid_for(total)), dim3(256), 0, (hipStream_t)stream, in, O, I, kh, kw, out,
                       total);
    FEMASR_CHECK_HIP(hipGetLastError());
    return FEMASR_OK;
}

size_t femasr_up2_weight_floats(int O, int I)
{
    return (I % 32) == 0 ? 4 * femasr_packed_weight_floats(O, I, 2, 2) : 0;
}

int femasr_repack_oihw_up2(void *stream, const float *in, int O, int I, float *out)
{
    FEMASR_REQUIRE(in && out && O > 0 && I > 0 && (I % 32) == 0, "repack_up2: needs a 3x3 OIHW weight with I %% 32 == 0");
    const size_t per = femasr_packed_weight_floats(O, I, 2, 2);
    hipLaunchKernelGGL(repack_up2_kernel, dim3(grid_for(4 * per)), dim3(256), 0, (hipStream_t)stream, in, O, I, out, per);
    FEMASR_CHECK_HIP(hipGetLastError());
    return FEMASR_OK;
}

int femasr_image_u8_to_f32(void *stream, const uint8_t *in_hwc, int H, int W, int swap_rb, float *out_chw)
{
    FEMASR_REQUIRE(in_hwc && out_chw && H > 0 && W > 0, "image_u8_to_f32: bad args");
    const size_t total = (size_t)3 * H * W;
    hipLaunchKernelGGL(image_u8_to_f32_kernel, dim3(grid_for(total)), dim3(256), 0, (hipStream_t)stream, in_hwc, H, W,
                       swap_rb, out_chw, total);
    FEMASR_CHECK_HIP(hipGetLastError());
    return FEMASR_OK;
}

int femasr_image_f32_to_u8(void *stream, const float *in_chw, int H, int W, int swap_rb, uint8_t *out_hwc)
{
    FEMASR_REQUIRE(in_chw && out_hwc && H > 0 && W > 0, "image_f32_to_u8: bad args");
    const size_t total = (size_t)3 * H * W;
    hipLaunchKernelGGL(image_f32_to_u8_kernel, dim3(grid_for(total)), dim3(256), 0, (hipStream_t)stream, in_chw, H, W,
                       swap_rb, out_hwc, total);
    FEMASR_CHECK_HIP(hipGetLastError());
    return FEMASR_OK;
}

int femasr_clock_probe_entries(void) { return FEMASR_CLOCK_PROBE_BLOCKS * 4; }

int femasr_clock_probe(void *stream, int mfmas_per_wave, unsigned long long *ticks)
{
    FEMASR_REQUIRE(ticks && mfmas_per_wave >= 4, "clock_probe: bad args");
    hipLaunchKernelGGL(clock_probe_kernel, dim3(FEMASR_CLOCK_PROBE_BLOCKS), dim3(256), 0, (hipStream_t)stream, mfmas_per_wave / 4, 1.0001f, 0.5f, ticks);
    FEMASR_CHECK_HIP(hipGetLastError());
    return FEMASR_OK;
}

}

int femasr_conv_form_variant_count(ConvForm f)
{
    const int n[CONV_FORM_COUNT] = {femasr_conv_variant_count(), femasr_conv_bf16x3_variant_count(), femasr_conv_wino_variant_count(), 1,
                                    femasr_gemm_bf16s_variant_count()};
    return n[f];
}

const char *femasr_conv_form_variant_name(ConvForm f, int v)
{
    switch (f) {
    case CONV_BF16X3: return femasr_conv_bf16x3_variant_name(v);
    case CONV_WINO: return femasr_conv_wino_variant_name(v);
    case CONV_WINO_UP2: return femasr_conv_wino_up2_variant_name();
    case CONV_SPLIT: return femasr_gemm_bf16s_variant_name(v);
    default: return femasr_conv_variant_name(v);
    }
}

int femasr_conv_form_launch(hipStream_t s, ConvForm f, const femasr_conv_args *a, int *slot_out, double *flops_out)
{
    int v = 0, r;
    switch (f) {
    case CONV_BF16X3: r = femasr_conv_bf16x3_launch(s, a, &v, flops_out); break;
    case CONV_WINO: r = femasr_conv_wino_launch(s, a, &v, flops_out); break;
    case CONV_WINO_UP2: r = femasr_conv_wino_up2_launch(s, a, flops_out); break;
    case CONV_SPLIT: r = femasr_gemm_bf16s_launch(s, a, a->w_bf16s, &v, flops_out); break;
    default: r = femasr_conv2d_launch(s, a, nullptr, &v, flops_out); break;
    }
    for (int g = 0; g < f; ++g) v += femasr_conv_form_variant_count((ConvForm)g);
    if (slot_out) *slot_out = v;
    return r;
}

static ConvForm conv2d_form(const femasr_conv_args *a)
{
    return !a ? CONV_DIRECT : a->w_bf16s ? CONV_SPLIT : a->w_bf16x3 ? CONV_BF16X3 : !a->w_wino ? CONV_DIRECT : a->up2 ? CONV_WINO_UP2 : CONV_WINO;
}

extern "C" int femasr_debug_conv_variant_name(const femasr_conv_args *a, char *name, int cap)
{
    FEMASR_REQUIRE(a && name && cap > 0, "debug_conv_variant_name: bad args");
    FEMASR_REQUIRE(a->B > 0 && a->H > 0 && a->W > 0 && a->Cin > 0 && a->Cout > 0 && a->ksz >= 1 && a->ksz <= 11 &&
                   (a->stride == 1 || a->stride == 2 || a->stride == 4) && a->pad >= 0,
                   "debug_conv_variant_name: empty shape or unsupported ksz=%d stride=%d pad=%d", a->ksz, a->stride, a->pad);
    const ConvForm f = conv2d_form(a);
    int v = 0;
    switch (f) {
    case CONV_BF16X3: v = femasr_conv_bf16x3_pick_variant(a); break;
    case CONV_WINO: v = femasr_conv_wino_pick_variant(a); break;
    case CONV_WINO_UP2: v = 0; break;
    case CONV_SPLIT: v = femasr_gemm_bf16s_pick_variant(a); break;
    default: v = femasr_conv2d_pick_variant(a); break;
    }
    const char *s = femasr_conv_form_variant_name(f, v);
    const size_t n = strlen(s);
    FEMASR_REQUIRE(n < (size_t)cap, "debug_conv_variant_name: the name needs %zu bytes, the buffer holds %d", n + 1, cap);
    memcpy(name, s, n + 1);
    return FEMASR_OK;
}

extern "C" int femasr_conv2d(void *stream, const femasr_conv_args *a)
{
    FEMASR_REQUIRE(!a || !a->in_add || (a->w_wino && a->up2 && !a->w_bf16x3 && !a->w_bf16s),
                   "conv2d: in_add is only taken by the x2 Winograd-type form (up2 = 1 with w_wino, no w_bf16x3 / w_bf16s)");
    const ConvForm f = conv2d_form(a);
    FEMASR_REQUIRE(f != CONV_SPLIT || femasr_gemm_bf16s_shape_ok(a),
                   "conv2d: w_bf16s given but the layer is neither a 1x1 stride-1 layer nor a 3x3 pad-1 conv of stride 1 or 2, with Cin %% 64 == 0 and no prologue");
    FEMASR_REQUIRE(f != CONV_BF16X3 || femasr_conv_bf16x3_eligible(a), "conv2d: w_bf16x3 given but the layer is not eligible for the bf16x3 path");
    FEMASR_REQUIRE(f != CONV_WINO_UP2 || femasr_conv_wino_up2_shape_ok(a),
                   "conv2d: w_wino given with up2 but the layer is not a 3x3 stride-1 pad-1 conv with Cin %% 32 == 0, Cout %% 64 == 0, no prologue");
    FEMASR_REQUIRE(f != CONV_WINO || femasr_conv_wino_shape_ok(a), "conv2d: w_wino given but the layer is not a 3x3 stride-1 pad-1 conv with Cin %% 32 == 0, Cout %% 64 == 0");
    return femasr_conv_form_launch((hipStream_t)stream, f, a, nullptr, nullptr);
}
```

femasr_amd/csrc/kernels_wino.hip:

```cpp
#define FEMASR_WTT_BUF g_wi_ttbuf
#include "wino_common.h"

namespace {

template <int PRO, bool FAST, int NRES>
__global__ __launch_bounds__(W4_NT, 2) void conv3x3_wino4_kernel(const WinoParams p)
{
    constexpr bool HAS1 = NRES >= 1, HAS2 = NRES >= 2;
        extern __shared__ __attribute__((aligned(16))) float smem[];
    float *Ps = smem;
    float *Vs = smem + 2 * W4_PSZ;
    float *ABs = smem + W4_MAIN;

    const int t = threadIdx.x, lane = t & 63;
    const int wave = __builtin_amdgcn_readfirstlane(t >> 6);
    WTT_INIT
    const int c31 = lane & 31, hh = lane >> 5;
    const int L = xcd_remap(blockIdx.x, p.MB * p.NB);
    const int nb = L % p.NB, mb = L / p.NB;
    const int n0 = nb * 64;

    int sn[2], sy0[2], sx0[2], sbi[2];
    bool sval[2];
#pragma unroll
    for (int z = 0; z < 2; ++z) {
        const int sb = 2 * mb + z, per = p.sbY * p.sbX;
        sval[z] = sb < p.nsb;
        const int sbc = sval[z] ? sb : 0;
        sn[z] = sbc / per;
        sbi[z] = sbc - sn[z] * per;
        const int by = sbi[z] / p.sbX, bx = sbi[z] - by * p.sbX;
        sy0[z] = 16 * by;
        sx0[z] = 16 * bx;
    }

    const int quad = t & 1;
    unsigned goff[3];
    unsigned pmask = 0, rmask = 0;
#pragma unroll
    for (int i = 0; i < 3; ++i) {
        const int u = i < 2 ? t + 512 * i : 1024 + wave * 34 + lane;
        const bool real = i < 2 || lane < 34;
        const int z = u >= W4_UNITS_SB ? 1 : 0;
        const int pix = (u - W4_UNITS_SB * z) >> 1;
        const int py = pix / W4_PW, px = pix - py * W4_PW;
        const int y = (z ? sy0[1] : sy0[0]) - 1 + py, x = (z ? sx0[1] : sx0[0]) - 1 + px;
        const bool ok = real && (z ? sval[1] : sval[0]) && y >= 0 && y < p.H && x >= 0 && x < p.W;
        goff[i] = ok ? (unsigned)((((size_t)(z ? sn[1] - sn[0] : 0) * p.H + y) * p.W + x) * p.Cin + 4 * quad) * 4u : 0u;
        pmask |= (ok ? 1u : 0u) << i;
        rmask |= (real ? 1u : 0u) << i;
    }
    const int slot0 = (t >> 1) * W4_PS + 4 * quad;
    const int slot2d = (512 - 15 * wave) * W4_PS;
    auto unit_slot = [&](int i) -> int { return i == 0 ? slot0 : (i == 1 ? slot0 + 256 * W4_PS : slot0 + slot2d); };
    constexpr int KINDS = 2;
    const int zo1 = t >= W4_UNITS_SB - 512 ? KINDS * p.Cin : 0;
    const __amdgpu_buffer_rsrc_t rsrc_in = __builtin_amdgcn_make_buffer_rsrc((void *)(p.in + (size_t)sn[0] * p.H * p.W * p.Cin), 0, 0x7fffffff, 0x00020000);
    const __amdgpu_buffer_rsrc_t rsrc_u = __builtin_amdgcn_make_buffer_rsrc((void *)p.u, 0, 0x7fffffff, 0x00020000);
    float4 rp[3];
    auto load_patch_to = [&](float4 (&rr)[3], int s) {
        const int sc = s < p.nsteps ? s : p.nsteps - 1;
#pragma unroll
        for (int i = 0; i < 3; ++i) {
            const u32x4_t v = __builtin_amdgcn_raw_buffer_load_b128(rsrc_in, goff[i], sc * 32, 0);
            rr[i] = make_float4(__uint_as_float(v[0]), __uint_as_float(v[1]), __uint_as_float(v[2]), __uint_as_float(v[3]));
        }
    };
    auto load_patch = [&](int s) { load_patch_to(rp, s); };
    auto store_patch_from = [&](const float4 (&rr)[3], int s, int buf) {
        float *Pb = Ps + buf * W4_PSZ;
#pragma unroll
        for (int i = 0; i < 3; ++i) {
            float4 v = rr[i];
            if (PRO == FEMASR_PRO_GN_SILU) {
                const float *ab = ABs + (i == 0 ? 0 : (i == 1 ? zo1 : KINDS * p.Cin)) + s * 8 + 4 * quad;
                const float4 ga = ld4(ab), gb = ld4(ab + p.Cin);
                if (FAST) {
                    const tf2 x01 = __builtin_elementwise_fma(tf2{v.x, v.y}, tf2{ga.x, ga.y}, tf2{gb.x, gb.y});
                    const tf2 x23 = __builtin_elementwise_fma(tf2{v.z, v.w}, tf2{ga.z, ga.w}, tf2{gb.z, gb.w});
                    const tf2 nl2e = {-1.44269504088896341f, -1.44269504088896341f}, one = {1.0f, 1.0f};
                    const tf2 e01 = x01 * nl2e, e23 = x23 * nl2e;
                    const tf2 d01 = tf2{__builtin_amdgcn_exp2f(e01[0]), __builtin_amdgcn_exp2f(e01[1])} + one;
                    const tf2 d23 = tf2{__builtin_amdgcn_exp2f(e23[0]), __builtin_amdgcn_exp2f(e23[1])} + one;
                    const tf2 y01 = x01 * tf2{__builtin_amdgcn_rcpf(d01[0]), __builtin_amdgcn_rcpf(d01[1])};
                    const tf2 y23 = x23 * tf2{__builtin_amdgcn_rcpf(d23[0]), __builtin_amdgcn_rcpf(d23[1])};
                    v = make_float4(y01[0], y01[1], y23[0], y23[1]);
                } else {
                    v.x = det_silu(__builtin_fmaf(v.x, ga.x, gb.x));
                    v.y = det_silu(__builtin_fmaf(v.y, ga.y, gb.y));
                    v.z = det_silu(__builtin_fmaf(v.z, ga.z, gb.z));
                    v.w = det_silu(__builtin_fmaf(v.w, ga.w, gb.w));
                }
            }
            if (pmask & (1u << i)) {
                float *dst = Pb + unit_slot(i);
                *reinterpret_cast<float2 *>(dst) = make_float2(v.x, v.y);
                *reinterpret_cast<float2 *>(dst + 2) = make_float2(v.z, v.w);
            }
        }
    };
    float4 rq[3];

    const int thalf = wave & 1;
    const int tm = (wave >> 1) * 8 + (lane >> 3), tch = lane & 7;
    const int tsrc = (tm >> 4) * W4_PPIX * W4_PS + ((4 * ((tm & 15) >> 2) + thalf) * W4_PW + 4 * (tm & 3)) * W4_PS + tch;
    const int tdst = thalf * 18 * 256 + tm * 8 + (tch & 1) * 4 + (tch >> 1);
    tf2 td[5][3];
    auto transform_read = [&](int pbuf) {
        const float *src = Ps + pbuf * W4_PSZ + tsrc;
#pragma unroll
        for (int a = 0; a < 5; ++a)
#pragma unroll
            for (int b = 0; b < 3; ++b) td[a][b] = tf2{src[(a * W4_PW + 2 * b) * W4_PS], src[(a * W4_PW + 2 * b + 1) * W4_PS]};
    };
    auto fma2 = [](float c, tf2 x, tf2 y) -> tf2 { return __builtin_elementwise_fma(tf2{c, c}, x, y); };
    auto transform_write = [&](int vbuf) {
        float *dst = Vs + vbuf * W4_VSZ + tdst;
        tf2 r[3][3];
        if (thalf == 0) {
#pragma unroll
            for (int b = 0; b < 3; ++b) {
                r[0][b] = fma2(4.0f, td[0][b], fma2(-5.0f, td[2][b], td[4][b]));
                const tf2 a2 = fma2(-4.0f, td[2][b], td[4][b]), b2 = fma2(-4.0f, td[1][b], td[3][b]);
                r[1][b] = a2 + b2;
                r[2][b] = a2 - b2;
            }
        } else {
#pragma unroll
            for (int b = 0; b < 3; ++b) {
                const tf2 c2 = td[3][b] - td[1][b], e2 = td[2][b] - td[0][b];
                r[0][b] = fma2(2.0f, e2, c2);
                r[1][b] = fma2(-2.0f, e2, c2);
                r[2][b] = fma2(4.0f, td[0][b], fma2(-5.0f, td[2][b], td[4][b]));
            }
        }
#pragma unroll
        for (int i = 0; i < 3; ++i) {
            float v0, v1, v2, v3, v4, v5;
            bt_lo(r[i][0][0], r[i][0][1], r[i][1][0], r[i][1][1], r[i][2][0], v0, v1, v2);
            bt_hi(r[i][0][1], r[i][1][0], r[i][1][1], r[i][2][0], r[i][2][1], v3, v4, v5);
            float *o = dst + i * 6 * 256;
            o[0 * 256] = v0;
            o[1 * 256] = v1;
            o[2 * 256] = v2;
            o[3 * 256] = v3;
            o[4 * 256] = v4;
            o[5 * 256] = v5;
        }
    };

    f32x16 acc[9];
#pragma unroll
    for (int q = 0; q < 9; ++q)
#pragma unroll
        for (int r = 0; r < 16; ++r) acc[q][r] = 0.f;
    const unsigned lw = (unsigned)lane * 16u;
    const int aoff = c31 * 8 + hh * 4;
    auto pcomp = [&](int q) -> int { return q < 8 ? 4 * wave + (q >> 1) : 32 + (wave >> 1); };
    auto pntl = [&](int q) -> int { return q < 8 ? (q & 1) : (wave & 1); };
    auto ldU = [&](int s, int q) -> u32x4_t {
        const int sc = s < p.nsteps ? s : p.nsteps - 1;
        const int pr = (sc * 36 + pcomp(q)) * p.NT32 + 2 * nb + pntl(q);
        return __builtin_amdgcn_raw_buffer_load_b128(rsrc_u, lw, pr << 10, 0);
    };
    u32x4_t ring[3], early[3], late[3];
    auto issue_early = [&](int s) {
#pragma unroll
        for (int q = 3; q < 6; ++q) early[q - 3] = ldU(s, q);
    };
    auto mphase = [&](int s, auto par_c) {
        constexpr int PAR = decltype(par_c)::value;
        const float *Vb = Vs + PAR * W4_VSZ + aoff;
#pragma unroll
        for (int q = 6; q < 9; ++q) late[q - 6] = ldU(s, q);
        f32x4_t an = *reinterpret_cast<const f32x4_t *>(Vb + pcomp(0) * 256);
        __builtin_amdgcn_sched_barrier(0);
#pragma unroll
        for (int q = 0; q < 9; ++q) {
            const f32x4_t a = an;
            if ((q & 1) && q + 1 < 9) an = *reinterpret_cast<const f32x4_t *>(Vb + pcomp(q + 1) * 256);
            const f32x4_t b = __builtin_bit_cast(f32x4_t, q < 3 ? ring[q] : (q < 6 ? early[q - 3] : late[q - 6]));
#pragma unroll
            for (int e = 0; e < 4; ++e) acc[q] = __builtin_amdgcn_mfma_f32_32x32x2f32(a[e], b[e], acc[q], 0, 0, 0);
            if (q < 3) ring[q] = ldU(s + 1, q);
            if (q == 5) {
                if (PAR) load_patch_to(rp, s + 3);
                else load_patch_to(rq, s + 3);
            }
            __builtin_amdgcn_sched_barrier(0);
        }
    };

    load_patch(0);
    load_patch_to(rq, 1);
#pragma unroll
    for (int q = 0; q < 3; ++q) ring[q] = ldU(0, q);
    if (PRO == FEMASR_PRO_GN_SILU) {
        for (int i = t; i < 2 * KINDS * p.Cin; i += W4_NT) {
            const int z = i / (KINDS * p.Cin), r = i - z * KINDS * p.Cin, kind = r / p.Cin, c = r - kind * p.Cin;
            const float v = ((kind & 1) ? p.pro_b : p.pro_a)[(size_t)(z ? sn[1] : sn[0]) * p.Cin + c];
            ABs[i] = v;
        }
    }
#pragma unroll
    for (int i = 0; i < 3; ++i) {
        if (((rmask & ~pmask) >> i) & 1u) {
            float *dst = Ps + unit_slot(i);
            *reinterpret_cast<float2 *>(dst) = make_float2(0.f, 0.f);
            *reinterpret_cast<float2 *>(dst + 2) = make_float2(0.f, 0.f);
            *reinterpret_cast<float2 *>(dst + W4_PSZ) = make_float2(0.f, 0.f);
            *reinterpret_cast<float2 *>(dst + W4_PSZ + 2) = make_float2(0.f, 0.f);
        }
    }
    __syncthreads();
    store_patch_from(rp, 0, 0);
    load_patch_to(rp, 2);
    if (1 < p.nsteps) store_patch_from(rq, 1, 1);
    __syncthreads();
    transform_read(0);
    transform_write(0);
    issue_early(0);
    __syncthreads();
    WTT(0)

    constexpr bool HOIST = FAST || PRO == FEMASR_PRO_NONE;
    auto step = [&](int s, auto par_c) {
        constexpr int PAR = decltype(par_c)::value;
        mphase(s, par_c);
        if (HOIST) transform_read(PAR ^ 1);
        __builtin_amdgcn_sched_barrier(0);
        if (s < 24) WTT(64 + 2 * s)
        auto stage = [&]() {
            if (s + 2 < p.nsteps) { if (PAR) store_patch_from(rq, s + 2, PAR); else store_patch_from(rp, s + 2, PAR); }
        };
        if (HOIST) {
            transform_write(PAR ^ 1);
            __builtin_amdgcn_sched_barrier(0);
            stage();
        } else {
            stage();
            __builtin_amdgcn_sched_barrier(0);
            transform_read(PAR ^ 1);
            transform_write(PAR ^ 1);
        }
        __builtin_amdgcn_sched_barrier(0);
        issue_early(s + 1);
        if (s < 24) WTT(65 + 2 * s)
        __syncthreads();
        if (s < 40) WTT(16 + s)
    };
    for (int s = 0; s < p.nsteps; s += 2) {
        step(s, std::integral_constant<int, 0>{});
        step(s + 1, std::integral_constant<int, 1>{});
    }
    WTT(1)

    float *Mx = smem;
    double *red = reinterpret_cast<double *>(smem + W4_MX);
    const bool gnp = p.gn_part != nullptr;
    const int cg = p.Cout >> 5;
    const int gpt = 32 / (cg < 32 ? cg : 32);
    const int pi = t >> 5;
    const int ez = wave >> 2, ety = wave & 3, etx = 2 * hh;
    unsigned vmask[2] = {0xffffu, 0xffffu}, ooff;
    bool full = true;
#pragma unroll
    for (int z = 0; z < 2; ++z) full = full && (z ? sval[1] : sval[0]) && (z ? sy0[1] : sy0[0]) + 16 <= p.H && (z ? sx0[1] : sx0[0]) + 16 <= p.W;
    {
        const int oy = (ez ? sy0[1] : sy0[0]) + 4 * ety, ox = (ez ? sx0[1] : sx0[0]) + 4 * etx;
        if (!full) {
#pragma unroll
            for (int e = 0; e < 2; ++e) {
                unsigned m = 0;
#pragma unroll
                for (int k = 0; k < 16; ++k) m |= ((ez ? sval[1] : sval[0]) && oy + (k >> 2) < p.H && ox + 4 * e + (k & 3) < p.W ? 1u : 0u) << k;
                vmask[e] = m;
            }
        }
        ooff = (unsigned)((((ez ? sn[1] - sn[0] : 0) * p.H + oy) * p.W + ox) * p.Cout + n0 + c31) * 4u;
    }
    const size_t img0 = (size_t)sn[0] * p.H * p.W * p.Cout;
    const __amdgpu_buffer_rsrc_t rs_out = __builtin_amdgcn_make_buffer_rsrc((void *)(p.out + img0), 0, 0x7fffffff, 0x00020000);
    const __amdgpu_buffer_rsrc_t rs_r1 = __builtin_amdgcn_make_buffer_rsrc((void *)((HAS1 ? p.res1 : p.out) + img0), 0, 0x7fffffff, 0x00020000);
    const __amdgpu_buffer_rsrc_t rs_r2 = __builtin_amdgcn_make_buffer_rsrc((void *)((HAS2 ? p.res2 : p.out) + img0), 0, 0x7fffffff, 0x00020000);
    int cs_u = 0, rs_u = 0;
    auto soff = [&](int k, int e, int r) -> int { return (k >> 2) * rs_u + (4 * e + (k & 3)) * cs_u + 128 * r; };
    auto oob = [&](int e, int k) -> unsigned { return ~(unsigned)((int)(vmask[e] << (31 - k)) >> 31); };
    auto voff = [&](auto fullc, int e, int k) -> unsigned {
        if (decltype(fullc)::value) return ooff;
        return ooff | oob(e, k);
    };
    auto fetch = [&](auto fullc, const __amdgpu_buffer_rsrc_t rs, int r, tf2 (&dst)[16], int k0, int k1) {
#pragma unroll
        for (int k = 0; k < 16; ++k) {
            if (k < k0 || k >= k1) continue;
            dst[k][0] = __uint_as_float(__builtin_amdgcn_raw_buffer_load_b32(rs, voff(fullc, 0, k), soff(k, 0, r), 0));
            dst[k][1] = __uint_as_float(__builtin_amdgcn_raw_buffer_load_b32(rs, voff(fullc, 1, k), soff(k, 1, r), 0));
        }
    };
    auto round = [&](auto fullc, int r) {
        constexpr bool FULL = decltype(fullc)::value;
        tf2 r1[16], r2[16];
        if (!FULL) asm volatile("" : "+v"(vmask[0]), "+v"(vmask[1]));
        cs_u = __builtin_amdgcn_readfirstlane(p.Cout * 4);
        rs_u = __builtin_amdgcn_readfirstlane(p.W * p.Cout * 4);
        asm volatile("" : "+s"(cs_u), "+s"(rs_u));
        if (FULL) {
            if (HAS1) fetch(fullc, rs_r1, r, r1, 0, HAS2 ? 8 : 16);
            if (HAS2) fetch(fullc, rs_r2, r, r2, 0, 8);
        }
        const float bv = p.bias[n0 + 32 * r + c31];
        __syncthreads();
        WTT(3 + 4 * r)
        int so1 = (16 * 512 + pi * 32 + c31) * 8, so2 = (32 * 512 + pi * 32 + c31) * 8;
        asm volatile("" : "+v"(so1), "+v"(so2));
        const tf2 *src0 = reinterpret_cast<const tf2 *>(Mx) + pi * 32 + c31;
        const tf2 *src1 = reinterpret_cast<const tf2 *>(reinterpret_cast<const char *>(Mx) + so1), *src2 = reinterpret_cast<const tf2 *>(reinterpret_cast<const char *>(Mx) + so2);
        auto mx = [&](int c) -> tf2 { return c < 16 ? src0[c * 512] : (c < 32 ? src1[(c - 16) * 512] : src2[(c - 32) * 512]); };
        tf2 tt[4][6];
#pragma unroll
        for (int j = 0; j < 6; ++j) {
            at6(mx(0 * 6 + j), mx(1 * 6 + j), mx(2 * 6 + j), mx(3 * 6 + j), mx(4 * 6 + j), mx(5 * 6 + j), tt[0][j], tt[1][j], tt[2][j], tt[3][j]);
            if (j & 1) __builtin_amdgcn_sched_barrier(0);
        }
        if (FULL && HAS2) { fetch(fullc, rs_r1, r, r1, 8, 16); fetch(fullc, rs_r2, r, r2, 8, 16); }
        const tf2 bv2 = {bv, bv};
        tf2 s2 = {0.f, 0.f}, ss2 = {0.f, 0.f};
#pragma unroll
        for (int a = 0; a < 4; ++a) {
            tf2 y[4];
            if (!FULL) {
                __builtin_amdgcn_sched_barrier(0);
                if (HAS1) fetch(fullc, rs_r1, r, r1, 4 * a, 4 * a + 4);
                if (HAS2) fetch(fullc, rs_r2, r, r2, 4 * a, 4 * a + 4);
                __builtin_amdgcn_sched_barrier(0);
            }
            at6(tt[a][0], tt[a][1], tt[a][2], tt[a][3], tt[a][4], tt[a][5], y[0], y[1], y[2], y[3]);
#pragma unroll
            for (int b = 0; b < 4; ++b) {
                const int k = 4 * a + b;
                tf2 v = y[b] + bv2;
                if (HAS1) v = v + r1[k];
                if (HAS2) v = v + r2[k];
                __builtin_amdgcn_raw_buffer_store_b32(__float_as_uint(v[0]), rs_out, voff(fullc, 0, k), soff(k, 0, r), 0);
                __builtin_amdgcn_raw_buffer_store_b32(__float_as_uint(v[1]), rs_out, voff(fullc, 1, k), soff(k, 1, r), 0);
                if (gnp) {
                    if (!FULL) {
                        v[0] = __uint_as_float(__float_as_uint(v[0]) & ~oob(0, k));
                        v[1] = __uint_as_float(__float_as_uint(v[1]) & ~oob(1, k));
                    }
                    s2 = s2 + v;
                    ss2 = __builtin_elementwise_fma(v, v, ss2);
                }
            }
        }
        if (gnp) {
            double gs = (double)s2[0] + (double)s2[1], gss = (double)ss2[0] + (double)ss2[1];
            for (int d = 1; d < cg && d < 32; d <<= 1) {
                gs = gs + __shfl_xor(gs, d, 64);
                gss = gss + __shfl_xor(gss, d, 64);
            }
            const double a2 = gs + __shfl_xor(gs, 32, 64), b2 = gss + __shfl_xor(gss, 32, 64);
            if (lane < 32 && (c31 & (cg - 1)) == 0) {
                double *dst = red + ((size_t)wave * 16 + c31 / cg) * 2;
                dst[0] = a2;
                dst[1] = b2;
            }
        }
        WTT(4 + 4 * r)
    };
    int wo0 = (4 * wave) * 4096 + hh * 512 + c31 * 8, wo1 = (32 + (wave >> 1)) * 4096 + hh * 512 + c31 * 8;
    asm volatile("" : "+v"(wo0), "+v"(wo1));
    char *wb0 = reinterpret_cast<char *>(Mx) + wo0, *wb1 = reinterpret_cast<char *>(Mx) + wo1;
    auto write_acc = [&](auto rc) {
        constexpr int R = decltype(rc)::value;
#pragma unroll
        for (int q = 0; q < 9; ++q) {
            if (pntl(q) == R) {
                char *dst = q < 8 ? wb0 + (q >> 1) * 4096 : wb1;
#pragma unroll
                for (int e = 0; e < 16; e += 2)
                    *reinterpret_cast<tf2 *>(dst + (((e & 3) >> 1) + 4 * (e >> 2)) * 256) = tf2{acc[q][e], acc[q][e + 1]};
            }
        }
    };
    write_acc(std::integral_constant<int, 0>{});
#pragma unroll 1
    for (int r = 0; r < 2; ++r) {
        if (r == 1) write_acc(std::integral_constant<int, 1>{});
        WTT(2 + 4 * r)
        if (full) round(std::true_type{}, r); else round(std::false_type{}, r);
        __syncthreads();
        WTT(5 + 4 * r)
        if (gnp && t < 2 * gpt) {
            const int z = t / gpt, gl = t - z * gpt;
            if (z ? sval[1] : sval[0]) {
                double S = red[((size_t)(4 * z) * 16 + gl) * 2], SS = red[((size_t)(4 * z) * 16 + gl) * 2 + 1];
#pragma unroll
                for (int w = 1; w < 4; ++w) {
                    S = S + red[((size_t)(4 * z + w) * 16 + gl) * 2];
                    SS = SS + red[((size_t)(4 * z + w) * 16 + gl) * 2 + 1];
                }
                const int g = (n0 + 32 * r) / cg + gl;
                double *dst = p.gn_part + (((size_t)(z ? sn[1] : sn[0]) * p.sbY * p.sbX + (z ? sbi[1] : sbi[0])) * 32 + g) * 2;
                dst[0] = S;
                dst[1] = SS;
            }
        }
    }
    WTT_END
}

__global__ void repack_wino_kernel(const float *__restrict__ in, int O, int I, float *__restrict__ out, size_t total)
{
    const int NT32 = (O + 31) / 32;
    for (size_t idx = blockIdx.x * (size_t)blockDim.x + threadIdx.x; idx < total; idx += (size_t)gridDim.x * blockDim.x) {
        const int e = (int)(idx & 3), lane = (int)((idx >> 2) & 63);
        size_t rest = idx >> 8;
        const int ntile = (int)(rest % NT32);
        rest /= NT32;
        const int comp = (int)(rest % 36), step = (int)(rest / 36);
        const int ci = 8 * step + 2 * e + (lane >> 5), o = ntile * 32 + (lane & 31);
        float v = 0.f;
        if (ci < I && o < O) {
            const int i = comp / 6, j = comp - 6 * i;
            const float *gw = in + ((size_t)o * I + ci) * 9;
            float ur[3];
#pragma unroll
            for (int x = 0; x < 3; ++x) ur[x] = wino_g6(i, gw[x], gw[3 + x], gw[6 + x]);
            v = wino_g6(j, ur[0], ur[1], ur[2]);
        }
        out[idx] = v;
    }
}

struct WVariant {
    const char *name;
    void (*kern)(const WinoParams);
    unsigned long long attr_devs;
};
#define FEMASR_WINO(PRO, FAST, NRES) { "conv3x3_wino4<2x16x16px x64," #PRO "," #FAST ",res=" #NRES ",waves=8>", conv3x3_wino4_kernel<PRO, FAST, NRES>, 0ull }
#define FEMASR_WINO3(PRO, FAST) FEMASR_WINO(PRO, FAST, 0), FEMASR_WINO(PRO, FAST, 1), FEMASR_WINO(PRO, FAST, 2)
WVariant g_wv[] = {
    FEMASR_WINO3(FEMASR_PRO_NONE, false),
    FEMASR_WINO3(FEMASR_PRO_GN_SILU, false),
    FEMASR_WINO3(FEMASR_PRO_GN_SILU, true),
};
constexpr int kNumW = sizeof(g_wv) / sizeof(g_wv[0]);

}

bool femasr_conv_wino_shape_ok_lim(const femasr_conv_args *a, int log2_total, int log2_image)
{
    const size_t tot = (size_t)1 << log2_total, img = (size_t)1 << log2_image;
    return a->ksz == 3 && a->stride == 1 && a->pad == 1 && !a->up2 && a->act == FEMASR_ACT_NONE && (a->Cin % BK) == 0 && a->Cin <= W4_MAX_CIN &&
           (a->Cout % 64) == 0 && (a->prologue == FEMASR_PRO_NONE || a->prologue == FEMASR_PRO_GN_SILU) &&
           (size_t)a->B * a->H * a->W * a->Cin < tot && (size_t)a->B * a->H * a->W * a->Cout < tot &&
           (size_t)a->H * a->W * a->Cin < img &&
           (size_t)a->H * a->W * a->Cout < img &&
           (size_t)36 * a->Cin * a->Cout < ((size_t)1 << 29);
}
bool femasr_conv_wino_shape_ok(const femasr_conv_args *a) { return femasr_conv_wino_shape_ok_lim(a, FEMASR_WINO_LOG2_TOTAL, FEMASR_WINO_LOG2_IMAGE); }
int femasr_conv_wino_variant_count() { return kNumW; }
const char *femasr_conv_wino_variant_name(int v) { return v >= 0 && v < kNumW ? g_wv[v].name : "?"; }
int femasr_conv_wino_gn_tiles(int H, int W) { return ((H + 15) / 16) * ((W + 15) / 16); }

int femasr_conv_wino_pick_variant(const femasr_conv_args *a)
{
    return 3 * (a->prologue == FEMASR_PRO_GN_SILU ? (a->fast_act ? 2 : 1) : 0) + (a->res1 ? (a->res2 ? 2 : 1) : 0);
}

int femasr_conv_wino_launch(hipStream_t s, const femasr_conv_args *a, int *variant_out, double *flops_out)
{
    FEMASR_REQUIRE(a && a->in && a->w_wino && a->bias && a->out && femasr_conv_wino_shape_ok(a), "conv_wino: bad arguments / shape");
    FEMASR_REQUIRE(a->Ho == a->H && a->Wo == a->W, "conv_wino: Ho/Wo mismatch");
    const bool gn = a->prologue == FEMASR_PRO_GN_SILU;
    if (gn) FEMASR_REQUIRE(a->pro_a && a->pro_b, "conv_wino: GN prologue needs a,b");
    FEMASR_REQUIRE(!a->gn_part || femasr_gn_fusable(a->Cout), "conv_wino: gn_part needs 32 | Cout and Cout/32 a power of two <= 32");
    WinoParams p{};
    p.in = a->in; p.u = (const float *)a->w_wino; p.bias = a->bias; p.pro_a = a->pro_a; p.pro_b = a->pro_b;
    p.res1 = a->res1; p.res2 = a->res2; p.out = a->out; p.gn_part = a->gn_part;
    p.B = a->B; p.H = a->H; p.W = a->W; p.Cin = a->Cin; p.Cout = a->Cout;
    p.sbX = (a->W + 15) / 16;
    p.sbY = (a->H + 15) / 16;
    p.nsb = a->B * p.sbX * p.sbY;
    p.MB = (p.nsb + 1) / 2;
    p.NB = a->Cout / 64;
    p.nsteps = a->Cin / 8;
    p.NT32 = a->Cout / 32;
    FEMASR_REQUIRE(a->res1 || !a->res2, "conv_wino: res2 without res1");
    FEMASR_REQUIRE(!a->in_add, "conv_wino: in_add is only taken by the x2 form");
    const int vi = femasr_conv_wino_pick_variant(a);
    WVariant &v = g_wv[vi];
    FEMASR_CHECK(femasr_allow_dynamic_lds((const void *)v.kern, &v.attr_devs, wino_lds_bytes(W4_MAX_CIN, true)));
    const size_t lds = wino_lds_bytes(a->Cin, gn);
    hipLaunchKernelGGL(v.kern, dim3((unsigned)(p.MB * p.NB)), dim3(W4_NT), lds, s, p);
    FEMASR_CHECK_HIP(hipGetLastError());
    if (variant_out) *variant_out = vi;
    if (flops_out) *flops_out = 2.0 * (double)a->B * a->H * a->W * 9.0 * (double)a->Cin * (double)a->Cout;
    return FEMASR_OK;
}

extern "C" {

#ifdef FEMASR_WINO_TT
int femasr_debug_wino_ttbuf(unsigned long long *dev_buf)
{
    return (int)hipMemcpyToSymbol(HIP_SYMBOL(g_wi_ttbuf), &dev_buf, sizeof(dev_buf));
}
#endif

size_t femasr_wino_weight_floats(int O, int I) { return (I % 32) == 0 ? (size_t)(I / 8) * 36 * ((O + 31) / 32) * 256 : 0; }

int femasr_repack_oihw_wino(void *stream, const float *in, int O, int I, float *out)
{
    FEMASR_REQUIRE(in && out && O > 0 && I > 0 && (I % 32) == 0, "repack_wino: needs a 3x3 OIHW weight with I %% 32 == 0");
    const size_t total = femasr_wino_weight_floats(O, I);
    size_t blocks = (total + 255) / 256;
    if (blocks > 65535) blocks = 65535;
    hipLaunchKernelGGL(repack_wino_kernel, dim3((unsigned)blocks), dim3(256), 0, (hipStream_t)stream, in, O, I, out, total);
    FEMASR_CHECK_HIP(hipGetLastError());
    return FEMASR_OK;
}

}
```

femasr_amd/csrc/model.hip:

```cpp
#include <stdarg.h>
#include <stdio.h>
#include <stdlib.h>
#include <string.h>

#include <algorithm>
#include <array>
#include <map>
#include <string>
#include <vector>

#include "common.h"

static thread_local char g_err[1024] = "";

int femasr_set_error(int code, const char *fmt, ...)
{
    va_list ap;
    va_start(ap, fmt);
    vsnprintf(g_err, sizeof(g_err), fmt, ap);
    va_end(ap);
    return code;
}

namespace {

struct DeviceGuard {
    int prev = -1;
    bool ok = true;
    explicit DeviceGuard(int dev)
    {
        if (hipGetDevice(&prev) != hipSuccess) prev = -1;
        if (prev != dev) ok = hipSetDevice(dev) == hipSuccess;
    }
    ~DeviceGuard() { if (prev >= 0) (void)hipSetDevice(prev); }
};

int channels_at(int res)
{
    switch (res) {
    case 8: case 16: case 32: case 64: return 256;
    case 128: return 128;
    case 256: return 64;
    case 512: return 32;
    default: return -1;
    }
}

int ilog2(int v)
{
    int r = 0;
    while ((1 << (r + 1)) <= v) ++r;
    return r;
}

enum WKind { W_CONV, W_LINEAR, W_VEC, W_TABLE, W_CODEBOOK };

struct WSpec {
    std::string key;
    WKind kind;
    int64_t shape[4];
    int ndim;
    float *dev = nullptr;
    float *up2w = nullptr;
    void *bf16x3 = nullptr;
    float *wino = nullptr;
    void *bf16s = nullptr;
    bool up2 = false;
    bool set = false;
    size_t numel() const { size_t n = 1; for (int i = 0; i < ndim; ++i) n *= (size_t)shape[i]; return n; }
};

bool behind_every_lookup(const femasr_config &cfg, int encode_depth, int last_quant_stage, const std::string &k)
{
    const bool dec = k.rfind("decoder_group.", 0) == 0, aq = k.rfind("after_quant_group.", 0) == 0, oc = k.rfind("out_conv", 0) == 0;
    if (cfg.n_codebooks == 1) {
        if (dec || aq || oc) return true;
        const std::string pre = "multiscale_encoder.blocks.";
        return cfg.lq_stage && k.rfind(pre, 0) == 0 && atoi(k.c_str() + pre.size()) > encode_depth;
    }
    if (oc) return true;
    if (aq) return atoi(k.c_str() + 18) == cfg.n_codebooks - 1;
    if (dec) return atoi(k.c_str() + 14) >= last_quant_stage;
    return false;
}

struct T {
    float *p = nullptr;
    int B = 0, H = 0, W = 0, C = 0;
    double *gn_part = nullptr;
    int gn_tiles = 0;
    size_t numel() const { return (size_t)B * H * W * C; }
};

struct Arena {
    char *base = nullptr;
    size_t cap = 0, peak = 0;
    bool dry = true;
    std::map<size_t, size_t> free_;
    std::map<size_t, size_t> used_;
    void reset(void *b, size_t c, bool d)
    {
        base = d ? (char *)4096 : (char *)b; cap = c; dry = d; peak = 0;
        free_.clear(); used_.clear();
        free_[0] = d ? ((size_t)1 << 60) : c;
    }
    void *alloc(size_t bytes)
    {
        bytes = (bytes + 255) & ~(size_t)255;
        if (bytes == 0) bytes = 256;
        for (auto it = free_.begin(); it != free_.end(); ++it) {
            if (it->second >= bytes) {
                const size_t off = it->first, rest = it->second - bytes;
                free_.erase(it);
                if (rest) free_[off + bytes] = rest;
                used_[off] = bytes;
                peak = std::max(peak, off + bytes);
                return base + off;
            }
        }
        return nullptr;
    }
    void release(void *ptr)
    {
        const size_t off = (size_t)((char *)ptr - base);
        auto it = used_.find(off);
        if (it == used_.end()) return;
        size_t sz = it->second, o = off;
        used_.erase(it);
        auto nx = free_.lower_bound(o);
        if (nx != free_.end() && o + sz == nx->first) { sz += nx->second; nx = free_.erase(nx); }
        if (nx != free_.begin()) {
            auto pv = std::prev(nx);
            if (pv->first + pv->second == o) { o = pv->first; sz += pv->second; free_.erase(pv); }
        }
        free_[o] = sz;
    }
};

struct ProfRec { int slot; hipEvent_t e0, e1; double flops, bytes; };

struct ConvModes {
    int decoder_math = 0;
    int linear_math = 1;
    int wino_log2_total = FEMASR_WINO_LOG2_TOTAL, wino_log2_image = FEMASR_WINO_LOG2_IMAGE;
};

}

struct femasr_handle {
    femasr_config cfg;
    int scale = 1, max_depth = 0, encode_depth = 0;
    int last_quant_stage = 0;
    std::vector<WSpec> specs;
    std::map<std::string, int> index;
    float *cbT[FEMASR_MAX_CODEBOOKS] = {nullptr, nullptr, nullptr}, *ee[FEMASR_MAX_CODEBOOKS] = {nullptr, nullptr, nullptr};
    void *vq_aux[FEMASR_MAX_CODEBOOKS] = {nullptr, nullptr, nullptr};
    bool finalized = false;
    bool prof = false;
    std::vector<ProfRec> recs;
    std::vector<hipEvent_t> pool;
    size_t pool_used = 0;
    std::vector<double> acc_ms, acc_flops, acc_bytes;
    std::vector<int64_t> acc_n;
    std::vector<std::string> slot_names;
    ConvModes modes;
    int nsub = 1;
    std::vector<hipStream_t> sub_streams;
    std::vector<hipEvent_t> sub_done;
    hipEvent_t ev_fork = nullptr;
    std::map<std::array<int, 4>, std::vector<size_t>> plans;
};

namespace {

enum { SLOT_GN = 0, SLOT_LN, SLOT_ATTN, SLOT_VQ, SLOT_LAYOUT, SLOT_SMALL_COUNT };
const char *kSmallNames[SLOT_SMALL_COUNT] = {"gn_moments", "layernorm", "window_attention", "vq(codebook lookup)",
                                             "pad/crop/gather layout"};

struct Scope {
    femasr_handle *h;
    ProfRec rec{};
    bool on;
    hipStream_t st;
    Scope(femasr_handle *hh, hipStream_t stream, bool dry, int slot, double flops, double bytes)
        : h(hh), on(hh->prof && !dry), st(stream)
    {
        if (!on) return;
        auto get = [&]() {
            if (h->pool_used == h->pool.size()) {
                hipEvent_t e;
                (void)hipEventCreate(&e);
                h->pool.push_back(e);
            }
            return h->pool[h->pool_used++];
        };
        rec.slot = slot; rec.flops = flops; rec.bytes = bytes;
        rec.e0 = get(); rec.e1 = get();
        (void)hipEventRecord(rec.e0, st);
    }
    void set_slot(int s) { rec.slot = s; }
    void set_flops(double f) { rec.flops = f; }
    void set_bytes(double b) { rec.bytes = b; }
    ~Scope()
    {
        if (!on) return;
        (void)hipEventRecord(rec.e1, st);
        h->recs.push_back(rec);
    }
};

void add_conv(femasr_handle *h, const std::string &p, int cin, int cout, int k, bool up2 = false)
{
    WSpec w; w.key = p + ".weight"; w.kind = W_CONV; w.ndim = 4;
    w.shape[0] = cout; w.shape[1] = cin; w.shape[2] = k; w.shape[3] = k;
    w.up2 = up2;
    h->specs.push_back(w);
    WSpec b; b.key = p + ".bias"; b.kind = W_VEC; b.ndim = 1; b.shape[0] = cout;
    h->specs.push_back(b);
}
void add_linear(femasr_handle *h, const std::string &p, int cin, int cout)
{
    WSpec w; w.key = p + ".weight"; w.kind = W_LINEAR; w.ndim = 2; w.shape[0] = cout; w.shape[1] = cin;
    h->specs.push_back(w);
    WSpec b; b.key = p + ".bias"; b.kind = W_VEC; b.ndim = 1; b.shape[0] = cout;
    h->specs.push_back(b);
}
void add_norm(femasr_handle *h, const std::string &p, int c)
{
    for (const char *leaf : {".weight", ".bias"}) {
        WSpec w; w.key = p + leaf; w.kind = W_VEC; w.ndim = 1; w.shape[0] = c;
        h->specs.push_back(w);
    }
}
void add_resblock(femasr_handle *h, const std::string &p, int c)
{
    add_norm(h, p + ".conv.0.norm", c);
    add_conv(h, p + ".conv.2", c, c, 3);
    add_norm(h, p + ".conv.3.norm", c);
    add_conv(h, p + ".conv.5", c, c, 3);
}

int build_specs(femasr_handle *h)
{
    const femasr_config &c = h->cfg;
    const std::string enc = "multiscale_encoder";
    int res = c.gt_resolution / h->scale;
    FEMASR_REQUIRE(channels_at(res) > 0, "unsupported encoder input resolution %d", res);
    add_conv(h, enc + ".in_conv", c.in_channel, channels_at(res), 4);
    int bi = 0;
    for (int i = 0; i < h->encode_depth; ++i, ++bi) {
        const int ic = channels_at(res), oc = channels_at(res / 2);
        FEMASR_REQUIRE(ic > 0 && oc > 0, "unsupported resolution %d", res);
        const std::string p = enc + ".blocks." + std::to_string(bi);
        add_conv(h, p + ".0", ic, oc, 3);
        add_resblock(h, p + ".1", oc);
        add_resblock(h, p + ".2", oc);
        res /= 2;
    }
    if (c.lq_stage) {
        FEMASR_REQUIRE(channels_at(res) == 256, "Swin stage needs 256 channels at res %d", res);
        const std::string sp = enc + ".blocks." + std::to_string(bi++);
        for (int r = 0; r < 4; ++r) {
            const std::string rp = sp + ".swin_blks." + std::to_string(r);
            for (int k = 0; k < 6; ++k) {
                const std::string bp = rp + ".residual_group.blocks." + std::to_string(k);
                add_norm(h, bp + ".norm1", 256);
                WSpec tb; tb.key = bp + ".attn.relative_position_bias_table"; tb.kind = W_TABLE; tb.ndim = 2;
                tb.shape[0] = 225; tb.shape[1] = 8;
                h->specs.push_back(tb);
                add_linear(h, bp + ".attn.qkv", 256, 768);
                add_linear(h, bp + ".attn.proj", 256, 256);
                add_norm(h, bp + ".norm2", 256);
                add_linear(h, bp + ".mlp.fc1", 256, 1024);
                add_linear(h, bp + ".mlp.fc2", 1024, 256);
            }
            add_conv(h, rp + ".conv", 256, 256, 3);
        }
        for (int u = 0; u < 2; ++u, ++bi) {
            const int ic = channels_at(res), oc = channels_at(res * 2);
            const std::string p = enc + ".blocks." + std::to_string(bi);
            add_conv(h, p + ".1", ic, oc, 3, true);
            add_resblock(h, p + ".2", oc);
            add_resblock(h, p + ".3", oc);
            res *= 2;
        }
    }
    int out_ch = 0;
    for (int i = 0; i < h->max_depth; ++i) {
        const int r = c.gt_resolution / (1 << h->max_depth) * (1 << i);
        const int ic = channels_at(r), oc = channels_at(r * 2);
        FEMASR_REQUIRE(ic > 0 && oc > 0, "unsupported decoder resolution %d", r);
        const std::string p = "decoder_group." + std::to_string(i) + ".block";
        add_conv(h, p + ".1", ic, oc, 3, true);
        add_resblock(h, p + ".2", oc);
        add_resblock(h, p + ".3", oc);
        out_ch = oc;
    }
    add_conv(h, "out_conv", out_ch, 3, 3);
    for (int q = 0; q < c.n_codebooks; ++q) {
        const std::string qs = std::to_string(q);
        WSpec cb; cb.key = "quantize_group." + qs + ".embedding.weight"; cb.kind = W_CODEBOOK; cb.ndim = 2;
        cb.shape[0] = c.n_e[q]; cb.shape[1] = c.e_dim[q];
        h->specs.push_back(cb);
        const int qc = channels_at(c.codebook_scale[q]);
        FEMASR_REQUIRE(qc > 0, "unsupported codebook scale %d", c.codebook_scale[q]);
        add_conv(h, "before_quant_group." + qs, q == 0 ? qc : 2 * qc, c.e_dim[q], 1);
        add_conv(h, "after_quant_group." + qs + ".conv", q == 0 ? c.e_dim[0] : c.e_dim[q - 1] + c.e_dim[q], qc, 3);
    }
    for (size_t i = 0; i < h->specs.size(); ++i) h->index[h->specs[i].key] = (int)i;
    return FEMASR_OK;
}

ConvForm conv_form(const femasr_handle *h, const ConvModes &m, const std::string &key, const femasr_conv_args &a)
{
    const bool behind = behind_every_lookup(h->cfg, h->encode_depth, h->last_quant_stage, key);
    if (behind && m.decoder_math == 1 && a.Cout > 4 && femasr_conv_bf16x3_shape_ok(&a)) return CONV_BF16X3;
    if (behind && (m.decoder_math == 0 || m.decoder_math == 3)) {
        if (femasr_conv_wino_up2_shape_ok_lim(&a, m.wino_log2_total, m.wino_log2_image)) return CONV_WINO_UP2;
        if (femasr_conv_wino_shape_ok_lim(&a, m.wino_log2_total, m.wino_log2_image)) return CONV_WINO;
    }
    if (m.linear_math == 1) {
        femasr_conv_args plain = a;
        plain.prologue = FEMASR_PRO_NONE;
        if (!behind && (a.prologue == FEMASR_PRO_NONE || a.prologue == FEMASR_PRO_GN_SILU) && femasr_conv3x3_bf16s_shape_ok(&plain)) return CONV_SPLIT;
        if (a.ksz == 1 && femasr_gemm_bf16s_shape_ok(&a)) return CONV_SPLIT;
    }
    return CONV_DIRECT;
}

int gn_tiles(ConvForm f, const femasr_conv_args &a)
{
    const bool fusable = femasr_gn_fusable(a.Cout);
    switch (f) {
    case CONV_SPLIT: return 0;
    case CONV_BF16X3: return fusable && a.Cout <= 256 ? ((a.Ho + 7) / 8) * ((a.Wo + 15) / 16) : 0;
    case CONV_WINO:
    case CONV_WINO_UP2: return femasr_conv_halo_eligible(&a) && fusable ? femasr_conv_wino_gn_tiles(a.Ho, a.Wo) : 0;
    default:
        if (!femasr_conv_halo_eligible(&a) || !fusable) return 0;
        return a.up2 ? 4 * ((a.H + 7) / 8) * ((a.W + 15) / 16) : ((a.Ho + 7) / 8) * ((a.Wo + 15) / 16);
    }
}

std::array<bool, CONV_FORM_COUNT> layer_forms(const femasr_handle *h, const WSpec &w)
{
    femasr_conv_args a{};
    a.B = 1; a.H = 16; a.W = 16; a.Cin = (int)w.shape[1]; a.Cout = (int)w.shape[0];
    a.ksz = w.kind == W_CONV ? (int)w.shape[2] : 1; a.stride = 1; a.pad = a.ksz / 2; a.up2 = w.up2;
    std::array<bool, CONV_FORM_COUNT> can{};
    ConvModes m;
    for (m.decoder_math = 0; m.decoder_math <= 3; ++m.decoder_math)
        for (m.linear_math = 0; m.linear_math <= 1; ++m.linear_math) can[conv_form(h, m, w.key, a)] = true;
    return can;
}

struct Ctx {
    femasr_handle *h;
    Arena *arena;
    hipStream_t stream;
    int rc = 0;
    int io_u8 = 0, swap_rb = 0;
    bool dry() const { return arena->dry; }
    hipStream_t s() const { return stream; }

    const WSpec *spec(const std::string &key)
    {
        auto it = h->index.find(key);
        if (it == h->index.end()) { if (!rc) rc = femasr_set_error(FEMASR_ERR_WEIGHT, "internal: unknown weight %s", key.c_str()); return nullptr; }
        return &h->specs[it->second];
    }
    const float *Wt(const std::string &key) { const WSpec *w = spec(key); return w ? w->dev : nullptr; }
    float *alloc_f(size_t n)
    {
        void *p = arena->alloc(n * sizeof(float));
        if (!p && !rc) rc = femasr_set_error(FEMASR_ERR_WORKSPACE, "workspace too small (need > %zu bytes)", arena->cap);
        return (float *)p;
    }
    T alloc_t(int B, int H, int W, int C)
    {
        T t; t.B = B; t.H = H; t.W = W; t.C = C;
        t.p = alloc_f(t.numel());
        return t;
    }
    void release(void *p) { if (p) arena->release(p); }
    void release(T &t) { release(t.p); t.p = nullptr; }

    struct ConvOpt {
        int ksz = 3, stride = 1, pad = 1, up2 = 0, act = 0;
        int pro = FEMASR_PRO_NONE;
        const float *pa = nullptr, *pb = nullptr, *pc = nullptr;
        const float *res1 = nullptr, *res2 = nullptr;
        const float *in_add = nullptr;
        bool want_gn = false;
    };
    femasr_conv_args conv_args(const T &x, int cout, const ConvOpt &o) const
    {
        const int Hv = o.up2 ? 2 * x.H : x.H, Wv = o.up2 ? 2 * x.W : x.W;
        femasr_conv_args a{};
        a.in = x.p; a.B = x.B; a.H = x.H; a.W = x.W; a.Cin = x.C;
        a.Cout = cout; a.ksz = o.ksz; a.stride = o.stride; a.pad = o.pad; a.up2 = o.up2;
        a.prologue = o.pro; a.pro_a = o.pa; a.pro_b = o.pb; a.pro_c = o.pc;
        a.act = o.act; a.res1 = o.res1; a.res2 = o.res2; a.in_add = o.in_add;
        a.Ho = (Hv + 2 * o.pad - o.ksz) / o.stride + 1; a.Wo = (Wv + 2 * o.pad - o.ksz) / o.stride + 1;
        return a;
    }

    T conv(const T &x, const std::string &prefix, int cout, const ConvOpt &o)
    {
        femasr_conv_args a = conv_args(x, cout, o);
        T y = alloc_t(x.B, a.Ho, a.Wo, cout);
        a.out = y.p;
        const ConvForm f = conv_form(h, h->modes, prefix, a);
        if (o.in_add && f != CONV_WINO_UP2 && !rc)
            rc = femasr_set_error(FEMASR_ERR_INVALID, "conv %s: a second input was scheduled for a conv that does not run in the x2 Winograd-type form", prefix.c_str());
        float *act_tmp = (f == CONV_SPLIT && o.pro == FEMASR_PRO_GN_SILU) ? alloc_f(x.numel()) : nullptr;
        if (o.want_gn && (y.gn_tiles = gn_tiles(f, a)) > 0) {
            y.gn_part = (double *)arena->alloc((size_t)x.B * y.gn_tiles * 32 * 2 * sizeof(double));
            if (!y.gn_part && !rc) rc = femasr_set_error(FEMASR_ERR_WORKSPACE, "workspace too small");
        }
        if (rc || dry()) { release(act_tmp); return y; }
        const WSpec *w = spec(prefix + ".weight");
        a.bias = Wt(prefix + ".bias");
        if (rc) { release(act_tmp); return y; }
        a.w = w->dev; a.gn_part = y.gn_part;
        if (o.up2) a.w_up2 = w->up2w;
        const void *image = a.w;
        switch (f) {
        case CONV_BF16X3: image = a.w_bf16x3 = w->bf16x3; break;
        case CONV_WINO:
        case CONV_WINO_UP2: image = a.w_wino = w->wino; a.fast_act = h->modes.decoder_math == 0 ? 1 : 0; break;
        case CONV_SPLIT: image = a.w_bf16s = w->bf16s; break;
        default: break;
        }
        if (!image) {
            rc = femasr_set_error(FEMASR_ERR_WEIGHT, "internal: conv %s: the weights of its form %d were not packed", prefix.c_str(), (int)f);
            release(act_tmp);
            return y;
        }
        if (act_tmp) {
            Scope sa(h, s(), dry(), SLOT_GN, 0.0, (double)x.numel() * 8.0);
            const int ra = femasr_gn_silu_apply(s(), x.p, x.B, x.H, x.W, x.C, o.pa, o.pb, act_tmp);
            if (ra && !rc) rc = ra;
            a.in = act_tmp;
            a.prologue = FEMASR_PRO_NONE; a.pro_a = nullptr; a.pro_b = nullptr;
        }
        Scope sc(h, s(), dry(), 0, 0.0, 0.0);
        int slot = 0; double flops = 0;
        const int r = femasr_conv_form_launch(s(), f, &a, &slot, &flops);
        sc.set_slot(SLOT_SMALL_COUNT + slot);
        sc.set_flops(flops);
        sc.set_bytes(4.0 * ((double)x.numel() * (o.in_add ? 2 : 1) + (double)y.numel() * (1 + (o.res1 ? 1 : 0) + (o.res2 ? 1 : 0)) +
                            (double)cout * x.C * o.ksz * o.ksz + cout));
        if (r && !rc) rc = r;
        release(act_tmp);
        return y;
    }

    float *gn(T &x, const std::string &norm_prefix)
    {
        float *ab = alloc_f((size_t)2 * x.B * x.C);
        if (x.gn_part) {
            if (!rc && !dry()) {
                Scope sc(h, s(), dry(), SLOT_GN, 0.0, (double)x.B * x.gn_tiles * 32 * 16.0);
                const int r = femasr_gn_coeffs_from_partials(s(), x.gn_part, x.B, x.gn_tiles, x.H, x.W, x.C, 32, Wt(norm_prefix + ".weight"),
                                                             Wt(norm_prefix + ".bias"), 1e-6f, ab, ab + (size_t)x.B * x.C);
                if (r && !rc) rc = r;
            }
            release(x.gn_part);
            x.gn_part = nullptr;
            return ab;
        }
        void *scratch = arena->alloc(femasr_gn_scratch_bytes(x.B, x.H, x.W, x.C, 32));
        if (!scratch && !rc) rc = femasr_set_error(FEMASR_ERR_WORKSPACE, "workspace too small");
        if (!rc && !dry()) {
            Scope sc(h, s(), dry(), SLOT_GN, 0.0, (double)x.numel() * 4.0);
            const int r = femasr_gn_coeffs(s(), x.p, x.B, x.H, x.W, x.C, 32, Wt(norm_prefix + ".weight"), Wt(norm_prefix + ".bias"),
                                           1e-6f, ab, ab + (size_t)x.B * x.C, scratch);
            if (r && !rc) rc = r;
        }
        release(scratch);
        return ab;
    }

    T resblock(T x, const std::string &p, const float *res2, bool free_x, bool out_gn = false)
    {
        const size_t bc = (size_t)x.B * x.C;
        float *ab = gn(x, p + ".conv.0.norm");
        ConvOpt o1; o1.pro = FEMASR_PRO_GN_SILU; o1.pa = ab; o1.pb = ab ? ab + bc : nullptr; o1.want_gn = true;
        T u = conv(x, p + ".conv.2", x.C, o1);
        release(ab);
        float *ab2 = gn(u, p + ".conv.3.norm");
        ConvOpt o2; o2.pro = FEMASR_PRO_GN_SILU; o2.pa = ab2; o2.pb = ab2 ? ab2 + bc : nullptr;
        o2.res1 = x.p; o2.res2 = res2; o2.want_gn = out_gn;
        T y = conv(u, p + ".conv.5", x.C, o2);
        release(ab2);
        release(u);
        if (free_x) release(x);
        return y;
    }

    T swin_block(const T &y, int B, int H, int W, const std::string &bp, int shift)
    {
        const int rows = B * H * W, C = 256;
        auto ln = [&](const T &t, const std::string &np) {
            T o = alloc_t(1, rows, 1, C);
            if (rc || dry()) return o;
            Scope sc(h, s(), dry(), SLOT_LN, 0.0, (double)t.numel() * 8.0);
            const int r = femasr_layernorm(s(), t.p, rows, C, Wt(np + ".weight"), Wt(np + ".bias"), 1e-5f, o.p);
            if (r && !rc) rc = r;
            return o;
        };
        T n1 = ln(y, bp + ".norm1");
        ConvOpt oq; oq.ksz = 1; oq.pad = 0;
        T qkv = conv(n1, bp + ".attn.qkv", 3 * C, oq);
        release(n1);
        T att = alloc_t(1, rows, 1, C);
        if (!rc && !dry()) {
            Scope sc(h, s(), dry(), SLOT_ATTN, 4.0 * (double)rows * 64.0 * C, (double)rows * C * 16.0);
            const int r = femasr_window_attention(s(), qkv.p, B, H, W, C, 8, shift, Wt(bp + ".attn.relative_position_bias_table"), att.p);
            if (r && !rc) rc = r;
        }
        release(qkv);
        ConvOpt op; op.ksz = 1; op.pad = 0; op.res1 = y.p;
        T y1 = conv(att, bp + ".attn.proj", C, op);
        release(att);
        T n2 = ln(y1, bp + ".norm2");
        ConvOpt o1; o1.ksz = 1; o1.pad = 0; o1.act = FEMASR_ACT_GELU;
        T hdn = conv(n2, bp + ".mlp.fc1", 4 * C, o1);
        release(n2);
        ConvOpt o2; o2.ksz = 1; o2.pad = 0; o2.res1 = y1.p;
        T y2 = conv(hdn, bp + ".mlp.fc2", C, o2);
        release(hdn);
        release(y1);
        return y2;
    }

    T swin_layers(T x, const std::string &sp)
    {
        const int B = x.B, H = x.H, W = x.W, C = x.C;
        for (int r = 0; r < 4; ++r) {
            const std::string rp = sp + ".swin_blks." + std::to_string(r);
            T y; y.p = x.p; y.B = 1; y.H = B * H * W; y.W = 1; y.C = C;
            for (int k = 0; k < 6; ++k) {
                T yn = swin_block(y, B, H, W, rp + ".residual_group.blocks." + std::to_string(k), (k & 1) ? 4 : 0);
                if (y.p != x.p) release(y);
                y = yn;
            }
            T yi; yi.p = y.p; yi.B = B; yi.H = H; yi.W = W; yi.C = C;
            ConvOpt o; o.res1 = x.p;
            T nx = conv(yi, rp + ".conv", C, o);
            release(y);
            release(x);
            x = nx;
        }
        return x;
    }

    T up_block(const T &x, const std::string &p, int cout, const float *res2_last, const float *in_add = nullptr)
    {
        ConvOpt o; o.up2 = 1; o.want_gn = true; o.in_add = in_add;
        T c = conv(x, p + ".1", cout, o);
        T r1 = resblock(c, p + ".2", nullptr, true, true);
        return resblock(r1, p + ".3", res2_last, true, false);
    }
};

struct Geometry {
    int Hp, Wp;
    int eh, ew;
    int out_h, out_w;
    int crop_h, crop_w;
    int nq;
    int qh[FEMASR_MAX_CODEBOOKS], qw[FEMASR_MAX_CODEBOOKS];
};

bool quant_at(const femasr_handle *h, int i, int *which)
{
    const int cur_res = h->cfg.gt_resolution / (1 << h->max_depth) * (1 << i);
    for (int q = 0; q < h->cfg.n_codebooks; ++q)
        if (h->cfg.codebook_scale[q] == cur_res) { if (which) *which = q; return true; }
    return false;
}

int plan_geometry(const femasr_handle *h, int H, int W, int pad_mode, Geometry *g)
{
    g->Hp = H; g->Wp = W;
    if (pad_mode) {
        const int wsz = 8 / h->scale * 8;
        g->Hp = (H / wsz + 1) * wsz;
        g->Wp = (W / wsz + 1) * wsz;
        if (h->cfg.lq_stage) {
            FEMASR_REQUIRE(g->Hp - H <= H && g->Wp - W <= W, "test(): image %dx%d smaller than its mirror pad", H, W);
        } else {
            g->Hp = std::min(g->Hp, 2 * H);
            g->Wp = std::min(g->Wp, 2 * W);
        }
    }
    FEMASR_REQUIRE(g->Hp >= 2 && g->Wp >= 2, "input too small");
    int eh = g->Hp - 1, ew = g->Wp - 1;
    for (int i = 0; i < h->encode_depth; ++i) { eh = (eh - 1) / 2 + 1; ew = (ew - 1) / 2 + 1; }
    FEMASR_REQUIRE(eh >= 1 && ew >= 1, "input too small");
    if (h->cfg.lq_stage) FEMASR_REQUIRE(eh % 8 == 0 && ew % 8 == 0, "Swin stage needs a feature map divisible by 8, got %dx%d", eh, ew);
    g->eh = eh; g->ew = ew;
    g->out_h = eh << h->max_depth; g->out_w = ew << h->max_depth;
    const int s_out = pad_mode ? h->scale : 1;
    g->crop_h = pad_mode ? std::min(H * s_out, g->out_h) : g->out_h;
    g->crop_w = pad_mode ? std::min(W * s_out, g->out_w) : g->out_w;
    g->nq = 0;
    for (int i = 0; i < h->max_depth; ++i) {
        int q;
        if (quant_at(h, i, &q)) { g->qh[g->nq] = eh << i; g->qw[g->nq] = ew << i; ++g->nq; }
    }
    return FEMASR_OK;
}

int run_tail(Ctx &c, T x, std::vector<T> &feats, bool fuse_skip, bool with_encoder, int64_t *const *idx_out, float *out_nchw,
             int crop_h, int crop_w)
{
    femasr_handle *h = c.h;
    const femasr_config &cfg = h->cfg;
    T prev_dec, prev_q, pending_add;
    int nq_done = 0;
    for (int i = 0; i < h->max_depth; ++i) {
        const int r = cfg.gt_resolution / (1 << h->max_depth) * (1 << i);
        int q = 0;
        if (with_encoder && quant_at(h, i, &q)) {
            const std::string qs = std::to_string(q);
            T zin = feats[i];
            if (prev_dec.p || (c.dry() && i > 0)) {
                if (feats[i].H != x.H || feats[i].W != x.W) {
                    if (!c.rc) c.rc = femasr_set_error(FEMASR_ERR_INVALID, "multi-codebook: encoder feature %dx%d and decoder feature %dx%d differ", feats[i].H, feats[i].W, x.H, x.W);
                    return c.rc;
                }
                zin = c.alloc_t(x.B, x.H, x.W, feats[i].C + x.C);
                if (!c.rc && !c.dry()) {
                    Scope sc(h, c.s(), c.dry(), SLOT_LAYOUT, 0.0, (double)zin.numel() * 8.0);
                    const int rr = femasr_concat_resize(c.s(), feats[i].p, feats[i].C, x.p, x.H, x.W, x.C, x.B, x.H, x.W, zin.p);
                    if (rr && !c.rc) c.rc = rr;
                }
                c.release(feats[i]);
                c.release(x);
            }
            Ctx::ConvOpt oq; oq.ksz = 1; oq.pad = 0;
            T z = c.conv(zin, "before_quant_group." + qs, cfg.e_dim[q], oq);
            c.release(zin);
            const int64_t M = (int64_t)z.B * z.H * z.W;
            T zq = c.alloc_t(z.B, z.H, z.W, cfg.e_dim[q]);
            int64_t *idx = idx_out ? idx_out[nq_done] : nullptr, *idx_tmp = nullptr;
            if (!idx) idx = idx_tmp = (int64_t *)c.arena->alloc((size_t)M * 8);
            {
                float *scratch = c.alloc_f(femasr_vq_scratch_bytes(M, cfg.n_e[q]) / sizeof(float));
                if (!c.rc && !c.dry()) {
                    Scope sc(h, c.s(), c.dry(), SLOT_VQ, 2.0 * (double)M * cfg.n_e[q] * cfg.e_dim[q],
                             (double)M * cfg.e_dim[q] * 8.0 + (double)cfg.n_e[q] * cfg.e_dim[q] * 4.0 + M * 8.0);
                    const float *cbw = c.Wt("quantize_group." + qs + ".embedding.weight");
                    const int rr = h->vq_aux[q]
                        ? femasr_vq_twopass(c.s(), z.p, M, cfg.e_dim[q], cbw, h->vq_aux[q], h->ee[q], cfg.n_e[q], idx, zq.p, scratch)
                        : femasr_vq(c.s(), z.p, M, cfg.e_dim[q], cbw, h->cbT[q], h->ee[q], cfg.n_e[q], idx, zq.p, scratch);
                    if (rr && !c.rc) c.rc = rr;
                }
                c.release(scratch);
            }
            if (idx_tmp) c.release(idx_tmp);
            ++nq_done;
            T qv = cfg.use_quantize ? zq : z;
            c.release(cfg.use_quantize ? z : zq);
            T ain = qv;
            if (prev_q.p || (c.dry() && nq_done > 1)) {
                ain = c.alloc_t(qv.B, qv.H, qv.W, qv.C + prev_q.C);
                if (!c.rc && !c.dry()) {
                    Scope sc(h, c.s(), c.dry(), SLOT_LAYOUT, 0.0, (double)ain.numel() * 8.0);
                    const int rr = femasr_concat_resize(c.s(), qv.p, qv.C, prev_q.p, prev_q.H, prev_q.W, prev_q.C, qv.B, qv.H, qv.W, ain.p);
                    if (rr && !c.rc) c.rc = rr;
                }
                c.release(prev_q);
            }
            x = c.conv(ain, "after_quant_group." + qs + ".conv", channels_at(cfg.codebook_scale[q]), Ctx::ConvOpt{});
            if (ain.p != qv.p) c.release(ain);
            bool later = false;
            for (int k = i + 1; k < h->max_depth; ++k) later = later || quant_at(h, k, nullptr);
            if (later) prev_q = qv; else c.release(qv);
        }
        const bool next_skip = with_encoder && fuse_skip && i + 1 < h->max_depth && !quant_at(h, i + 1, nullptr);
        const int cout_i = channels_at(r * 2);
        T nx; nx.B = x.B; nx.H = 2 * x.H; nx.W = 2 * x.W; nx.C = cout_i;
        Ctx::ConvOpt ou; ou.up2 = 1;
        const bool skip_by_next = next_skip && conv_form(h, h->modes, "decoder_group." + std::to_string(i + 1) + ".block.1",
                                                         c.conv_args(nx, channels_at(r * 4), ou)) == CONV_WINO_UP2;
        const float *skip = (next_skip && !skip_by_next) ? feats[i + 1].p : nullptr;
        T y = c.up_block(x, "decoder_group." + std::to_string(i) + ".block", cout_i, skip, pending_add.p);
        c.release(x);
        if (pending_add.p) { c.release(pending_add); pending_add = T{}; }
        if (next_skip) { if (skip_by_next) pending_add = feats[i + 1]; else c.release(feats[i + 1]); }
        x = y;
        prev_dec = x;
    }
    T img = c.conv(x, "out_conv", 3, Ctx::ConvOpt{});
    c.release(x);
    if (!c.rc && !c.dry()) {
        Scope sc(h, c.s(), c.dry(), SLOT_LAYOUT, 0.0, (double)img.B * 3.0 * crop_h * crop_w * 8.0);
        const int r = (c.io_u8 & 2) ? femasr_crop_nhwc_to_u8hwc(c.s(), img.p, img.B, img.H, img.W, crop_h, crop_w, c.swap_rb, (uint8_t *)out_nchw)
                                    : femasr_crop_nhwc_to_nchw(c.s(), img.p, img.B, img.H, img.W, 3, crop_h, crop_w, out_nchw);
        if (r && !c.rc) c.rc = r;
    }
    c.release(img);
    return c.rc;
}

int run_forward(femasr_handle *h, Arena *arena, hipStream_t stream, const float *in_nchw, int B, int H, int W, int pad_mode,
                float *out_nchw, int64_t *const *idx_out, int io_u8 = 0, int swap_rb = 0)
{
    const femasr_config &cfg = h->cfg;
    Ctx c{h, arena, stream};
    c.io_u8 = io_u8; c.swap_rb = swap_rb;
    Geometry g;
    int rc = plan_geometry(h, H, W, pad_mode, &g);
    if (rc) return rc;
    const bool fuse_skip = cfg.lq_stage && cfg.use_residual;
    auto needed = [&](int i) {
        return i == 0 || quant_at(h, i, nullptr) || fuse_skip;
    };

    T x0 = c.alloc_t(B, g.Hp, g.Wp, cfg.in_channel);
    if (!c.rc && !c.dry()) {
        Scope sc(h, c.s(), c.dry(), SLOT_LAYOUT, 0.0, (double)x0.numel() * 8.0);
        const int r = (c.io_u8 & 1) ? femasr_pad_u8hwc_to_nhwc(c.s(), (const uint8_t *)in_nchw, B, H, W, c.swap_rb, g.Hp, g.Wp, x0.p)
                                    : femasr_pad_nchw_to_nhwc(c.s(), in_nchw, B, cfg.in_channel, H, W, g.Hp, g.Wp, x0.p);
        if (r) c.rc = r;
    }
    const std::string enc = "multiscale_encoder";
    int res = cfg.gt_resolution / h->scale;
    Ctx::ConvOpt oin; oin.ksz = 4; oin.pad = 1;
    T t = c.conv(x0, enc + ".in_conv", channels_at(res), oin);
    c.release(x0);
    int bi = 0;
    std::vector<T> outs;
    bool t_kept = false;
    for (int i = 0; i < h->encode_depth; ++i, ++bi) {
        const std::string p = enc + ".blocks." + std::to_string(bi);
        Ctx::ConvOpt od; od.stride = 2;
        T d = c.conv(t, p + ".0", channels_at(res / 2), od);
        if (!t_kept) c.release(t);
        t = c.resblock(d, p + ".1", nullptr, true, true);
        t = c.resblock(t, p + ".2", nullptr, true);
        res /= 2;
        t_kept = false;
        if (!cfg.lq_stage) {
            const int fi = h->encode_depth - 1 - i;
            outs.push_back(t);
            t_kept = fi < h->max_depth && needed(fi) && i + 1 < h->encode_depth;
        }
    }
    std::vector<T> feats(FEMASR_MAX_CODEBOOKS + 1);
    if (cfg.lq_stage) {
        t = c.swin_layers(t, enc + ".blocks." + std::to_string(bi++));
        feats[0] = t;
        int last = 0;
        for (int u = 1; u <= 2 && u < h->max_depth; ++u) if (needed(u)) last = u;
        for (int u = 0; u < last; ++u, ++bi) {
            feats[u + 1] = c.up_block(feats[u], enc + ".blocks." + std::to_string(bi), channels_at(res * 2), nullptr);
            res *= 2;
        }
        for (int u = 1; u < last; ++u)
            if (!needed(u)) c.release(feats[u]);
    } else {
        for (int i = 0; i < h->encode_depth; ++i) {
            const int fi = h->encode_depth - 1 - i;
            if (fi < (int)feats.size() && fi < h->max_depth && needed(fi)) feats[fi] = outs[i];
        }
    }
    return run_tail(c, feats[0], feats, fuse_skip, true, idx_out, out_nchw, g.crop_h, g.crop_w);
}

int run_decode_indices(femasr_handle *h, Arena *arena, hipStream_t stream, const int64_t *indices, int B, int hq, int wq,
                       float *out_nchw)
{
    const femasr_config &cfg = h->cfg;
    Ctx c{h, arena, stream};
    T zq = c.alloc_t(B, hq, wq, cfg.e_dim[0]);
    if (!c.rc && !c.dry()) {
        Scope sc(h, c.s(), c.dry(), SLOT_LAYOUT, 0.0, (double)zq.numel() * 8.0);
        const int r = femasr_codebook_gather(c.s(), indices, (int64_t)B * hq * wq, cfg.e_dim[0], c.Wt("quantize_group.0.embedding.weight"), cfg.n_e[0], zq.p);
        if (r) c.rc = r;
    }
    T x = c.conv(zq, "after_quant_group.0.conv", channels_at(cfg.codebook_scale[0]), Ctx::ConvOpt{});
    c.release(zq);
    std::vector<T> feats(FEMASR_MAX_CODEBOOKS + 1);
    return run_tail(c, x, feats, false, false, nullptr, out_nchw, hq << h->max_depth, wq << h->max_depth);
}

int check_ready(const femasr_handle *h)
{
    FEMASR_REQUIRE(h, "null handle");
    if (!h->finalized) return femasr_set_error(FEMASR_ERR_WEIGHT, "weights not finalized: call femasr_set_weight for every key, then femasr_finalize_weights");
    return FEMASR_OK;
}

}

extern "C" {

const char *femasr_last_error(void) { return g_err; }
int femasr_version(void) { return 106; }

int femasr_create(const femasr_config *cfg, femasr_handle **out)
{
    FEMASR_REQUIRE(cfg && out, "create: null argument");
    FEMASR_REQUIRE(cfg->in_channel == 3, "create: in_channel must be 3");
    FEMASR_REQUIRE(cfg->n_codebooks >= 1 && cfg->n_codebooks <= FEMASR_MAX_CODEBOOKS, "create: n_codebooks must be 1..%d", FEMASR_MAX_CODEBOOKS);
    for (int q = 0; q < cfg->n_codebooks; ++q) {
        FEMASR_REQUIRE(cfg->n_e[q] > 0 && cfg->n_e[q] % 128 == 0 && cfg->e_dim[q] > 0 && cfg->e_dim[q] % 32 == 0,
                       "create: codebook %dx%d unsupported (n_e %% 128, e_dim %% 32)", cfg->n_e[q], cfg->e_dim[q]);
        FEMASR_REQUIRE(cfg->codebook_scale[q] > 0 && cfg->gt_resolution % cfg->codebook_scale[q] == 0, "create: bad codebook scale");
        FEMASR_REQUIRE(q == 0 || cfg->codebook_scale[q] > cfg->codebook_scale[q - 1], "create: codebook scales must ascend");
    }
    femasr_handle *h = new femasr_handle();
    h->cfg = *cfg;
    h->scale = cfg->lq_stage ? cfg->scale_factor : 1;
    if (!(h->scale == 1 || h->scale == 2 || h->scale == 4)) { delete h; return femasr_set_error(FEMASR_ERR_INVALID, "create: scale_factor %d unsupported", h->scale); }
    h->max_depth = ilog2(cfg->gt_resolution / cfg->codebook_scale[0]);
    h->last_quant_stage = ilog2(cfg->codebook_scale[cfg->n_codebooks - 1] / cfg->codebook_scale[0]);
    h->encode_depth = ilog2(cfg->gt_resolution / h->scale / cfg->codebook_scale[0]);
    if (h->max_depth < 1 || h->max_depth > 3) { delete h; return femasr_set_error(FEMASR_ERR_INVALID, "create: max_depth %d unsupported", h->max_depth); }
    for (int q = 1; q < cfg->n_codebooks; ++q) {
        bool hit = false;
        for (int i = 0; i < h->max_depth; ++i) hit = hit || (cfg->gt_resolution / (1 << h->max_depth) * (1 << i)) == cfg->codebook_scale[q];
        if (!hit) { delete h; return femasr_set_error(FEMASR_ERR_INVALID, "create: codebook scale %d is not a decoder resolution", cfg->codebook_scale[q]); }
    }
    DeviceGuard guard(cfg->device);
    if (!guard.ok) { delete h; return femasr_set_error(FEMASR_ERR_HIP, "hipSetDevice(%d) failed", cfg->device); }
    const int rc = build_specs(h);
    if (rc) { delete h; return rc; }
    for (int i = 0; i < SLOT_SMALL_COUNT; ++i) h->slot_names.push_back(kSmallNames[i]);
    for (int f = 0; f < CONV_FORM_COUNT; ++f)
        for (int v = 0; v < femasr_conv_form_variant_count((ConvForm)f); ++v) h->slot_names.push_back(femasr_conv_form_variant_name((ConvForm)f, v));
    const size_t nslots = h->slot_names.size();
    h->acc_ms.assign(nslots, 0.0); h->acc_flops.assign(nslots, 0.0); h->acc_bytes.assign(nslots, 0.0); h->acc_n.assign(nslots, 0);
    *out = h;
    return FEMASR_OK;
}

void femasr_destroy(femasr_handle *h)
{
    if (!h) return;
    for (auto &w : h->specs)
        for (void *p : {(void *)w.dev, (void *)w.up2w, w.bf16x3, (void *)w.wino, w.bf16s}) if (p) (void)hipFree(p);
    for (int q = 0; q < FEMASR_MAX_CODEBOOKS; ++q) {
        if (h->cbT[q]) (void)hipFree(h->cbT[q]);
        if (h->ee[q]) (void)hipFree(h->ee[q]);
        if (h->vq_aux[q]) (void)hipFree(h->vq_aux[q]);
    }
    for (auto e : h->pool) (void)hipEventDestroy(e);
    for (auto e : h->sub_done) (void)hipEventDestroy(e);
    for (auto st : h->sub_streams) (void)hipStreamDestroy(st);
    if (h->ev_fork) (void)hipEventDestroy(h->ev_fork);
    delete h;
}

int femasr_num_weights(const femasr_handle *h) { return h ? (int)h->specs.size() : 0; }

int femasr_weight_info(const femasr_handle *h, int i, const char **key, int64_t shape[4], int *ndim)
{
    FEMASR_REQUIRE(h && i >= 0 && i < (int)h->specs.size(), "weight_info: bad index");
    const WSpec &w = h->specs[i];
    if (key) *key = w.key.c_str();
    if (shape) for (int k = 0; k < 4; ++k) shape[k] = k < w.ndim ? w.shape[k] : 1;
    if (ndim) *ndim = w.ndim;
    return FEMASR_OK;
}

int femasr_set_weight(femasr_handle *h, const char *key, const float *dev_ptr, const int64_t *shape, int ndim)
{
    FEMASR_REQUIRE(h && key && dev_ptr && shape, "set_weight: null argument");
    const std::string k(key);
    if (k.size() > 24 && (k.rfind(".relative_position_index") == k.size() - 24)) return FEMASR_OK;
    if (k.size() > 10 && (k.rfind(".attn_mask") == k.size() - 10)) return FEMASR_OK;
    auto it = h->index.find(k);
    if (it == h->index.end()) return femasr_set_error(FEMASR_ERR_WEIGHT, "set_weight: unknown key '%s'", key);
    DeviceGuard guard(h->cfg.device);
    FEMASR_REQUIRE(guard.ok, "set_weight: hipSetDevice(%d) failed", h->cfg.device);
    WSpec &w = h->specs[it->second];
    bool same = (ndim == w.ndim);
    for (int i = 0; same && i < ndim; ++i) same = (shape[i] == w.shape[i]);
    if (!same) return femasr_set_error(FEMASR_ERR_WEIGHT, "set_weight: shape mismatch for '%s'", key);
    if (w.kind != W_CONV && w.kind != W_LINEAR) {
        if (!w.dev) FEMASR_CHECK_HIP(hipMalloc((void **)&w.dev, w.numel() * sizeof(float)));
        FEMASR_CHECK_HIP(hipMemcpyAsync(w.dev, dev_ptr, w.numel() * sizeof(float), hipMemcpyDeviceToDevice, nullptr));
    } else {
        const int O = (int)w.shape[0], I = (int)w.shape[1], kk = w.kind == W_CONV ? (int)w.shape[2] : 1;
        const std::array<bool, CONV_FORM_COUNT> can = layer_forms(h, w);
        if (!w.dev) FEMASR_CHECK_HIP(hipMalloc((void **)&w.dev, femasr_packed_weight_floats(O, I, kk, kk) * sizeof(float)));
        int rc = femasr_repack_oihw(nullptr, dev_ptr, O, I, kk, kk, w.dev);
        if (!rc && w.up2 && femasr_up2_weight_floats(O, I)) {
            if (!w.up2w) FEMASR_CHECK_HIP(hipMalloc((void **)&w.up2w, femasr_up2_weight_floats(O, I) * sizeof(float)));
            rc = femasr_repack_oihw_up2(nullptr, dev_ptr, O, I, w.up2w);
        }
        if (!rc && can[CONV_BF16X3]) {
            if (!w.bf16x3) FEMASR_CHECK_HIP(hipMalloc(&w.bf16x3, femasr_packed_weight_bf16x3_bytes(O, I, 3, 3)));
            rc = femasr_repack_oihw_bf16x3(nullptr, dev_ptr, O, I, 3, 3, w.bf16x3);
        }
        if (!rc && (can[CONV_WINO] || can[CONV_WINO_UP2])) {
            if (!w.wino) FEMASR_CHECK_HIP(hipMalloc((void **)&w.wino, (w.up2 ? femasr_wino_up2_weight_floats(O, I) : femasr_wino_weight_floats(O, I)) * sizeof(float)));
            rc = w.up2 ? femasr_repack_oihw_wino_up2(nullptr, dev_ptr, O, I, w.wino) : femasr_repack_oihw_wino(nullptr, dev_ptr, O, I, w.wino);
        }
        if (!rc && can[CONV_SPLIT]) {
            if (!w.bf16s) FEMASR_CHECK_HIP(hipMalloc(&w.bf16s, kk == 1 ? femasr_packed_weight_bf16s_bytes(O, I) : femasr_packed_weight_conv3x3_bf16s_bytes(O, I)));
            rc = kk == 1 ? femasr_repack_k1_bf16s(nullptr, dev_ptr, O, I, w.bf16s) : femasr_repack_oihw_bf16s(nullptr, dev_ptr, O, I, w.bf16s);
        }
        if (rc) return rc;
    }
    FEMASR_CHECK_HIP(hipStreamSynchronize(nullptr));
    w.set = true;
    h->finalized = false;
    return FEMASR_OK;
}

int femasr_finalize_weights(femasr_handle *h)
{
    FEMASR_REQUIRE(h, "finalize: null handle");
    for (const auto &w : h->specs)
        if (!w.set) return femasr_set_error(FEMASR_ERR_WEIGHT, "finalize: weight '%s' was never set", w.key.c_str());
    DeviceGuard guard(h->cfg.device);
    FEMASR_REQUIRE(guard.ok, "finalize: hipSetDevice(%d) failed", h->cfg.device);
    for (int q = 0; q < h->cfg.n_codebooks; ++q) {
        const int n_e = h->cfg.n_e[q], D = h->cfg.e_dim[q];
        if (!h->cbT[q]) FEMASR_CHECK_HIP(hipMalloc((void **)&h->cbT[q], femasr_packed_weight_floats(n_e, D, 1, 1) * sizeof(float)));
        if (!h->ee[q]) FEMASR_CHECK_HIP(hipMalloc((void **)&h->ee[q], (size_t)n_e * sizeof(float)));
        const float *cb = h->specs[h->index["quantize_group." + std::to_string(q) + ".embedding.weight"]].dev;
        int rc = femasr_repack_oihw(nullptr, cb, n_e, D, 1, 1, h->cbT[q]);
        if (rc) return rc;
        rc = femasr_row_sqsum(nullptr, cb, n_e, D, h->ee[q]);
        if (rc) return rc;
        const char *mode = getenv("FEMASR_VQ");
        const bool two = femasr_vq_twopass_ok(n_e, D) && !(mode && !strcmp(mode, "gemm"));
        if (two) {
            if (!h->vq_aux[q]) FEMASR_CHECK_HIP(hipMalloc(&h->vq_aux[q], femasr_vq_aux_bytes(n_e, D)));
            rc = femasr_vq_prepare(nullptr, cb, h->ee[q], n_e, D, h->vq_aux[q]);
            if (rc) return rc;
        } else if (h->vq_aux[q]) {
            (void)hipFree(h->vq_aux[q]);
            h->vq_aux[q] = nullptr;
        }
    }
    FEMASR_CHECK_HIP(hipStreamSynchronize(nullptr));
    h->plans.clear();
    h->finalized = true;
    return FEMASR_OK;
}

static void sub_range(int B, int S, int i, int *lo, int *hi)
{
    const int q = B / S, r = B % S;
    *lo = i * q + (i < r ? i : r);
    *hi = *lo + q + (i < r ? 1 : 0);
}

static int plan_for(femasr_handle *h, int B, int H, int W, int pad_mode, const std::vector<size_t> **out)
{
    const std::array<int, 4> key{B, H, W, pad_mode};
    auto it = h->plans.find(key);
    if (it == h->plans.end()) {
        const int S = std::min(h->nsub, B);
        std::vector<size_t> need;
        for (int i = 0; i < S; ++i) {
            int lo, hi;
            sub_range(B, S, i, &lo, &hi);
            Arena a;
            a.reset(nullptr, 0, true);
            const int rc = run_forward(h, &a, nullptr, nullptr, hi - lo, H, W, pad_mode, nullptr, nullptr);
            if (rc) return rc;
            need.push_back((a.peak + 255) & ~(size_t)255);
        }
        if (h->plans.size() > 64) h->plans.clear();
        it = h->plans.emplace(key, std::move(need)).first;
    }
    *out = &it->second;
    return FEMASR_OK;
}

int femasr_workspace_bytes(const femasr_handle *hc, int B, int H, int W, int pad_mode, size_t *bytes)
{
    femasr_handle *h = const_cast<femasr_handle *>(hc);
    FEMASR_REQUIRE(h && bytes && B > 0 && H > 0 && W > 0, "workspace_bytes: bad args");
    const std::vector<size_t> *need = nullptr;
    const int rc = plan_for(h, B, H, W, pad_mode, &need);
    if (rc) return rc;
    size_t total = 0;
    for (size_t n : *need) total += n;
    *bytes = total + 256;
    return FEMASR_OK;
}

int femasr_forward_shapes(const femasr_handle *h, int H, int W, int pad_mode, int *out_h, int *out_w, int *n_index_maps,
                          int *idx_h, int *idx_w)
{
    FEMASR_REQUIRE(h && H > 0 && W > 0, "forward_shapes: bad args");
    Geometry g;
    const int rc = plan_geometry(h, H, W, pad_mode, &g);
    if (rc) return rc;
    if (out_h) *out_h = g.crop_h;
    if (out_w) *out_w = g.crop_w;
    if (n_index_maps) *n_index_maps = g.nq;
    for (int q = 0; q < g.nq; ++q) {
        if (idx_h) idx_h[q] = g.qh[q];
        if (idx_w) idx_w[q] = g.qw[q];
    }
    return FEMASR_OK;
}

int femasr_set_streams(femasr_handle *h, int n)
{
    FEMASR_REQUIRE(h && n >= 1 && n <= 8, "set_streams: n must be in [1, 8]");
    DeviceGuard guard(h->cfg.device);
    FEMASR_REQUIRE(guard.ok, "set_streams: hipSetDevice(%d) failed", h->cfg.device);
    while ((int)h->sub_streams.size() < n) {
        hipStream_t st;
        hipEvent_t ev;
        FEMASR_CHECK_HIP(hipStreamCreateWithFlags(&st, hipStreamNonBlocking));
        FEMASR_CHECK_HIP(hipEventCreateWithFlags(&ev, hipEventDisableTiming));
        h->sub_streams.push_back(st);
        h->sub_done.push_back(ev);
    }
    if (!h->ev_fork) FEMASR_CHECK_HIP(hipEventCreateWithFlags(&h->ev_fork, hipEventDisableTiming));
    if (h->nsub != n) h->plans.clear();
    h->nsub = n;
    return FEMASR_OK;
}

static int forward_impl(femasr_handle *h, void *stream, const float *in_nchw, int B, int H, int W, int pad_mode,
                        float *out_nchw, int64_t *indices, void *ws, size_t ws_bytes, int io_u8, int swap_rb)
{
    int rc = check_ready(h);
    if (rc) return rc;
    FEMASR_REQUIRE(in_nchw && out_nchw && ws && B > 0 && H > 0 && W > 0, "forward: bad args");
    FEMASR_REQUIRE(!io_u8 || h->cfg.in_channel == 3, "forward_u8: 3-channel images only");
    FEMASR_REQUIRE(((uintptr_t)ws & 255) == 0, "forward: workspace must be 256-byte aligned");
    DeviceGuard guard(h->cfg.device);
    FEMASR_REQUIRE(guard.ok, "forward: hipSetDevice(%d) failed", h->cfg.device);
    hipStream_t caller = (hipStream_t)stream;
    Geometry g;
    rc = plan_geometry(h, H, W, pad_mode, &g);
    if (rc) return rc;
    int64_t *qbase[FEMASR_MAX_CODEBOOKS] = {nullptr, nullptr, nullptr};
    size_t qstride[FEMASR_MAX_CODEBOOKS] = {0, 0, 0};
    {
        size_t off = 0;
        for (int q = 0; q < g.nq; ++q) {
            qstride[q] = (size_t)g.qh[q] * g.qw[q];
            qbase[q] = indices ? indices + off : nullptr;
            off += (size_t)B * qstride[q];
        }
    }
    const std::vector<size_t> *need = nullptr;
    rc = plan_for(h, B, H, W, pad_mode, &need);
    if (rc) return rc;
    const int S = (int)need->size();
    if (S <= 1) {
        Arena a;
        a.reset(ws, ws_bytes, false);
        return run_forward(h, &a, caller, in_nchw, B, H, W, pad_mode, out_nchw, indices ? qbase : nullptr, io_u8, swap_rb);
    }
    size_t total = 0;
    for (size_t n : *need) total += n;
    if (total > ws_bytes) return femasr_set_error(FEMASR_ERR_WORKSPACE, "workspace too small for %d sub-batches", S);
    const size_t in_stride = (size_t)h->cfg.in_channel * H * W * ((io_u8 & 1) ? 1 : 4);
    const size_t out_stride = (size_t)3 * g.crop_h * g.crop_w * ((io_u8 & 2) ? 1 : 4);
    FEMASR_CHECK_HIP(hipEventRecord(h->ev_fork, caller));
    size_t off = 0;
    int forked = 0;
    for (int i = 0; i < S && !rc; ++i) {
        int lo, hi;
        sub_range(B, S, i, &lo, &hi);
        Arena a;
        a.reset((char *)ws + off, (*need)[i], false);
        off += (*need)[i];
        hipStream_t st = h->sub_streams[i];
        if (hipStreamWaitEvent(st, h->ev_fork, 0) != hipSuccess) { rc = femasr_set_error(FEMASR_ERR_HIP, "hipStreamWaitEvent failed"); break; }
        forked = i + 1;
        int64_t *qsub[FEMASR_MAX_CODEBOOKS];
        for (int q = 0; q < FEMASR_MAX_CODEBOOKS; ++q) qsub[q] = qbase[q] ? qbase[q] + lo * qstride[q] : nullptr;
        rc = run_forward(h, &a, st, (const float *)((const char *)in_nchw + lo * in_stride), hi - lo, H, W, pad_mode,
                         (float *)((char *)out_nchw + lo * out_stride), indices ? qsub : nullptr, io_u8, swap_rb);
    }
    for (int i = 0; i < forked; ++i) {
        if (hipEventRecord(h->sub_done[i], h->sub_streams[i]) != hipSuccess || hipStreamWaitEvent(caller, h->sub_done[i], 0) != hipSuccess) {
            if (!rc) rc = femasr_set_error(FEMASR_ERR_HIP, "joining sub-batch stream %d failed", i);
        }
    }
    return rc;
}

int femasr_forward(femasr_handle *h, void *stream, const float *in_nchw, int B, int H, int W, int pad_mode,
                   float *out_nchw, int64_t *indices, void *ws, size_t ws_bytes)
{
    return forward_impl(h, stream, in_nchw, B, H, W, pad_mode, out_nchw, indices, ws, ws_bytes, 0, 0);
}

int femasr_forward_u8(femasr_handle *h, void *stream, const uint8_t *in_hwc, int B, int H, int W, int swap_rb, int pad_mode,
                      uint8_t *out_hwc, int64_t *indices, void *ws, size_t ws_bytes)
{
    return forward_impl(h, stream, (const float *)in_hwc, B, H, W, pad_mode, (float *)out_hwc, indices, ws, ws_bytes, 3, swap_rb ? 1 : 0);
}

int femasr_decode_workspace_bytes(const femasr_handle *hc, int B, int hq, int wq, size_t *bytes)
{
    femasr_handle *h = const_cast<femasr_handle *>(hc);
    FEMASR_REQUIRE(h && bytes && B > 0 && hq > 0 && wq > 0, "decode_workspace_bytes: bad args");
    Arena a;
    a.reset(nullptr, 0, true);
    const int rc = run_decode_indices(h, &a, nullptr, nullptr, B, hq, wq, nullptr);
    if (rc) return rc;
    *bytes = a.peak + 256;
    return FEMASR_OK;
}

int femasr_decode_indices(femasr_handle *h, void *stream, const int64_t *indices, int B, int hq, int wq,
                          float *out_nchw, void *ws, size_t ws_bytes)
{
    int rc = check_ready(h);
    if (rc) return rc;
    FEMASR_REQUIRE(indices && out_nchw && ws && B > 0 && hq > 0 && wq > 0, "decode_indices: bad args");
    FEMASR_REQUIRE(((uintptr_t)ws & 255) == 0, "decode_indices: workspace must be 256-byte aligned");
    DeviceGuard guard(h->cfg.device);
    FEMASR_REQUIRE(guard.ok, "decode_indices: hipSetDevice(%d) failed", h->cfg.device);
    Arena a;
    a.reset(ws, ws_bytes, false);
    return run_decode_indices(h, &a, (hipStream_t)stream, indices, B, hq, wq, out_nchw);
}

int femasr_set_decoder_math(femasr_handle *h, int mode)
{
    FEMASR_REQUIRE(h && mode >= 0 && mode <= 3, "set_decoder_math: mode must be 0 (fp32), 1 (bf16x3), 2 (fp32, direct convs only) or 3 (fp32, exact SiLU)");
    if (h->modes.decoder_math != mode) h->plans.clear();
    h->modes.decoder_math = mode;
    return FEMASR_OK;
}

int femasr_debug_set_wino_limits(femasr_handle *h, int log2_total, int log2_image)
{
    FEMASR_REQUIRE(h && log2_total >= 0 && log2_total <= FEMASR_WINO_LOG2_TOTAL && log2_image >= 0 && log2_image <= FEMASR_WINO_LOG2_IMAGE,
                   "debug_set_wino_limits: exponents are 0 (default) or up to %d / %d", FEMASR_WINO_LOG2_TOTAL, FEMASR_WINO_LOG2_IMAGE);
    h->modes.wino_log2_total = log2_total ? log2_total : FEMASR_WINO_LOG2_TOTAL;
    h->modes.wino_log2_image = log2_image ? log2_image : FEMASR_WINO_LOG2_IMAGE;
    h->plans.clear();
    return FEMASR_OK;
}

int femasr_set_linear_math(femasr_handle *h, int mode)
{
    FEMASR_REQUIRE(h && (mode == 0 || mode == 1), "set_linear_math: mode must be 0 (fp32 MFMA chain) or 1 (bf16 three-term split)");
    if (h->modes.linear_math != mode) h->plans.clear();
    h->modes.linear_math = mode;
    return FEMASR_OK;
}

int femasr_profile_enable(femasr_handle *h, int on)
{
    FEMASR_REQUIRE(h, "null handle");
    h->prof = on != 0;
    return FEMASR_OK;
}

static int profile_drain(femasr_handle *h)
{
    for (auto &r : h->recs) {
        FEMASR_CHECK_HIP(hipEventSynchronize(r.e1));
        float ms = 0.f;
        FEMASR_CHECK_HIP(hipEventElapsedTime(&ms, r.e0, r.e1));
        h->acc_ms[r.slot] += ms;
        h->acc_flops[r.slot] += r.flops;
        h->acc_bytes[r.slot] += r.bytes;
        h->acc_n[r.slot] += 1;
    }
    h->recs.clear();
    h->pool_used = 0;
    return FEMASR_OK;
}

int femasr_profile_reset(femasr_handle *h)
{
    FEMASR_REQUIRE(h, "null handle");
    const int rc = profile_drain(h);
    std::fill(h->acc_ms.begin(), h->acc_ms.end(), 0.0);
    std::fill(h->acc_flops.begin(), h->acc_flops.end(), 0.0);
    std::fill(h->acc_bytes.begin(), h->acc_bytes.end(), 0.0);
    std::fill(h->acc_n.begin(), h->acc_n.end(), 0);
    return rc;
}

int femasr_profile_slots(const femasr_handle *h) { return h ? (int)h->slot_names.size() : 0; }

const char *femasr_profile_name(const femasr_handle *h, int slot)
{
    return (h && slot >= 0 && slot < (int)h->slot_names.size()) ? h->slot_names[slot].c_str() : "";
}

int femasr_profile_get(femasr_handle *h, int slot, double *ms, int64_t *launches, double *flops, double *bytes)
{
    FEMASR_REQUIRE(h && slot >= 0 && slot < (int)h->slot_names.size(), "profile_get: bad slot");
    const int rc = profile_drain(h);
    if (rc) return rc;
    if (ms) *ms = h->acc_ms[slot];
    if (launches) *launches = h->acc_n[slot];
    if (flops) *flops = h->acc_flops[slot];
    if (bytes) *bytes = h->acc_bytes[slot];
    return FEMASR_OK;
}

}
```

include/femasr_hip.h:

```cpp
#ifndef FEMASR_HIP_H
#define FEMASR_HIP_H

#include <stddef.h>
#include <stdint.h>

#ifdef __cplusplus
extern "C" {
#endif

typedef enum {
    FEMASR_OK = 0,
    FEMASR_ERR_INVALID = -1,
    FEMASR_ERR_HIP = -2,
    FEMASR_ERR_WEIGHT = -3,
    FEMASR_ERR_WORKSPACE = -4
} femasr_status;

typedef struct femasr_handle femasr_handle;

#define FEMASR_MAX_CODEBOOKS 3
typedef struct {
    int32_t in_channel;
    int32_t gt_resolution;
    int32_t lq_stage;
    int32_t scale_factor;
    int32_t use_quantize;
    int32_t use_residual;
    int32_t n_codebooks;
    int32_t codebook_scale[FEMASR_MAX_CODEBOOKS];
    int32_t n_e[FEMASR_MAX_CODEBOOKS];
    int32_t e_dim[FEMASR_MAX_CODEBOOKS];
    int32_t device;
} femasr_config;

const char *femasr_last_error(void);
int femasr_version(void);

int femasr_create(const femasr_config *cfg, femasr_handle **out);
void femasr_destroy(femasr_handle *h);

int femasr_num_weights(const femasr_handle *h);
int femasr_weight_info(const femasr_handle *h, int i, const char **key, int64_t shape[4], int *ndim);

int femasr_set_weight(femasr_handle *h, const char *key, const float *dev_ptr,
                      const int64_t *shape, int ndim);
int femasr_finalize_weights(femasr_handle *h);

int femasr_set_streams(femasr_handle *h, int n);

int femasr_workspace_bytes(const femasr_handle *h, int B, int H, int W, int pad_mode, size_t *bytes);

int femasr_forward_shapes(const femasr_handle *h, int H, int W, int pad_mode, int *out_h, int *out_w, int *n_index_maps,
                          int *idx_h, int *idx_w);

int femasr_forward(femasr_handle *h, void *stream, const float *in_nchw, int B, int H, int W,
                   int pad_mode, float *out_nchw, int64_t *indices, void *ws, size_t ws_bytes);

int femasr_forward_u8(femasr_handle *h, void *stream, const uint8_t *in_hwc, int B, int H, int W, int swap_rb, int pad_mode,
                      uint8_t *out_hwc, int64_t *indices, void *ws, size_t ws_bytes);
int femasr_pad_u8hwc_to_nhwc(void *stream, const uint8_t *in, int B, int H, int W, int swap_rb, int Hp, int Wp, float *out);
int femasr_crop_nhwc_to_u8hwc(void *stream, const float *in, int B, int Hs, int Ws, int Hc, int Wc, int swap_rb, uint8_t *out);

int femasr_decode_workspace_bytes(const femasr_handle *h, int B, int hq, int wq, size_t *bytes);
int femasr_decode_indices(femasr_handle *h, void *stream, const int64_t *indices, int B, int hq, int wq,
                          float *out_nchw, void *ws, size_t ws_bytes);

int femasr_profile_enable(femasr_handle *h, int on);
int femasr_profile_reset(femasr_handle *h);
int femasr_profile_slots(const femasr_handle *h);
const char *femasr_profile_name(const femasr_handle *h, int slot);
int femasr_profile_get(femasr_handle *h, int slot, double *ms, int64_t *launches, double *flops, double *bytes);


int femasr_pad_nchw_to_nhwc(void *stream, const float *in, int B, int C, int H, int W, int Hp, int Wp, float *out);
int femasr_crop_nhwc_to_nchw(void *stream, const float *in, int B, int Hs, int Ws, int C, int Hc, int Wc, float *out);

enum { FEMASR_PRO_NONE = 0, FEMASR_PRO_GN_SILU = 1, FEMASR_PRO_LN = 2  };
enum { FEMASR_ACT_NONE = 0, FEMASR_ACT_GELU = 1, FEMASR_ACT_RELU = 2  };

typedef struct {
    const float *in;
    int32_t B, H, W, Cin;
    const float *w;
    const float *bias;
    int32_t Cout, ksz, stride, pad, up2;
    int32_t prologue;
    const float *pro_a;
    const float *pro_b;
    const float *pro_c;
    int32_t act;
    const float *res1;
    const float *res2;
    float *out;
    int32_t Ho, Wo;
    const void *w_bf16x3;
    double *gn_part;
    const float *w_up2;
    const float *w_wino;
    int32_t fast_act;
    const float *in_add;
    const void *w_bf16s;
} femasr_conv_args;
int femasr_conv2d(void *stream, const femasr_conv_args *a);

size_t femasr_gn_scratch_bytes(int B, int H, int W, int C, int G);
int femasr_gn_coeffs(void *stream, const float *x, int B, int H, int W, int C, int G,
                     const float *gamma, const float *beta, float eps, float *a, float *b, void *scratch);
int femasr_gn_coeffs_from_partials(void *stream, const double *part, int B, int tiles, int H, int W, int C, int G,
                                   const float *gamma, const float *beta, float eps, float *a, float *b);
int femasr_gn_silu_apply(void *stream, const float *x, int B, int H, int W, int C, const float *a, const float *b, float *y);
int femasr_ln_stats(void *stream, const float *x, int64_t rows, int C, float eps, float *stats);
int femasr_layernorm(void *stream, const float *x, int64_t rows, int C, const float *gamma, const float *beta,
                     float eps, float *y);
int femasr_window_attention(void *stream, const float *qkv, int B, int H, int W, int C, int heads, int shift,
                            const float *table, float *out);
int femasr_vq(void *stream, const float *z, int64_t M, int D, const float *cb, const float *cbT,
              const float *ee, int n_e, int64_t *idx, float *zq, void *scratch);
int femasr_row_sqsum(void *stream, const float *x, int64_t rows, int D, float *out);
int femasr_vq_twopass_ok(int n_e, int D);
size_t femasr_vq_aux_bytes(int n_e, int D);
int femasr_vq_prepare(void *stream, const float *cb, const float *ee, int n_e, int D, void *aux);
size_t femasr_vq_scratch_bytes(int64_t M, int n_e);
int femasr_vq_twopass(void *stream, const float *z, int64_t M, int D, const float *cb, const void *aux, const float *ee,
                      int n_e, int64_t *idx, float *zq, void *scratch);
int femasr_vq_candidates(void *stream, const float *z, int64_t M, int D, const void *aux, const float *ee, int n_e,
                         uint16_t *cand, uint16_t *cnt);
int femasr_codebook_gather(void *stream, const int64_t *idx, int64_t M, int D, const float *cb, int n_e, float *zq);
int femasr_concat_resize(void *stream, const float *a, int Ca, const float *b, int Hb, int Wb, int Cb, int B, int H, int W,
                         float *out);
int femasr_extract_tiles(void *stream, const float *in, int B, int C, int H, int W, const int32_t *yx_dev, int n, int th, int tw,
                         float *out);
int femasr_paste_tiles(void *stream, const float *tiles, int B, int C, int n, int th, int tw, const int32_t *rects_dev, int hmax,
                       int Ho, int Wo, float *out);
int femasr_extract_tiles_u8(void *stream, const uint8_t *in, int B, int H, int W, const int32_t *yx_dev, int n, int th, int tw, uint8_t *out);
int femasr_paste_tiles_u8(void *stream, const uint8_t *tiles, int B, int n, int th, int tw, const int32_t *rects_dev, int hmax,
                          int Ho, int Wo, uint8_t *out);
int femasr_blend_tiles(void *stream, const uint64_t *tile_ptrs_dev, const int32_t *geom_dev, int n, int tiles_y, int tiles_x, int pitch,
                       int B, int C, int Ho, int Wo, float *out);
int femasr_blend_tiles_u8(void *stream, const uint64_t *tile_ptrs_dev, const int32_t *geom_dev, int n, int tiles_y, int tiles_x, int pitch,
                          int B, int Ho, int Wo, uint8_t *out);

size_t femasr_packed_weight_floats(int O, int I, int kh, int kw);
int femasr_repack_oihw(void *stream, const float *in, int O, int I, int kh, int kw, float *out);
size_t femasr_up2_weight_floats(int O, int I);
size_t femasr_wino_weight_floats(int O, int I);
int femasr_repack_oihw_wino(void *stream, const float *in, int O, int I, float *out);
size_t femasr_wino_up2_weight_floats(int O, int I);
int femasr_repack_oihw_wino_up2(void *stream, const float *w_oihw, int O, int I, float *out);
int femasr_repack_oihw_up2(void *stream, const float *in, int O, int I, float *out);

size_t femasr_packed_weight_bf16s_bytes(int O, int I);
int femasr_repack_k1_bf16s(void *stream, const float *w_oi, int O, int I, void *out);
size_t femasr_packed_weight_conv3x3_bf16s_bytes(int O, int I);
int femasr_repack_oihw_bf16s(void *stream, const float *w_oihw, int O, int I, void *out);
int femasr_set_linear_math(femasr_handle *h, int mode);

size_t femasr_packed_weight_bf16x3_bytes(int O, int I, int kh, int kw);
int femasr_repack_oihw_bf16x3(void *stream, const float *in, int O, int I, int kh, int kw, void *out);
int femasr_set_decoder_math(femasr_handle *h, int mode);

int femasr_image_u8_to_f32(void *stream, const uint8_t *in_hwc, int H, int W, int swap_rb, float *out_chw);
int femasr_image_f32_to_u8(void *stream, const float *in_chw, int H, int W, int swap_rb, uint8_t *out_hwc);

typedef struct femasr_lpips_handle femasr_lpips_handle;
int femasr_lpips_create(int net , int device, femasr_lpips_handle **out);
void femasr_lpips_destroy(femasr_lpips_handle *h);
int femasr_lpips_set_weight(femasr_lpips_handle *h, const char *key, const float *dev_ptr, const int64_t *shape, int ndim);
int femasr_lpips_finalize_weights(femasr_lpips_handle *h);
int femasr_lpips_workspace_bytes(const femasr_lpips_handle *h, int B, int H, int W, size_t *bytes);
int femasr_lpips_forward(femasr_lpips_handle *h, void *stream, const float *x0_nchw, const float *x1_nchw, int B, int H, int W,
                         float *out, float *per_layer, void *ws, size_t ws_bytes);
int femasr_lpips_scale_input(void *stream, const float *x0_nchw, const float *x1_nchw, int B, int H, int W, float *out_nhwc);
int femasr_lpips_tap_partials(int H, int W);
int femasr_lpips_tap(void *stream, const float *f, int B2, int H, int W, int C, const float *w_lin, int pool, float *pooled_out,
                     double *partials);
int femasr_lpips_finalize(void *stream, const double *partials, int B, int ntaps, const int32_t *tap_hw, float *out, float *per_layer);

int femasr_psnr_ssim_workspace_bytes(int B, int H, int W, int crop_border, int test_y, size_t *bytes);
int femasr_psnr_ssim(void *stream, const uint8_t *a, const uint8_t *b, int B, int H, int W, int crop_border, int test_y, double *psnr_out,
                     double *ssim_out, double *mse_out, void *ws, size_t ws_bytes);
int femasr_ssim_window(double *win);

int femasr_imresize_workspace_bytes(int N, int H, int W, int Ho, int Wo, size_t *bytes);
int femasr_imresize(void *stream, const void *in, int is_f64, int N, int H, int W, int Ho, int Wo, const double *w_h, const int32_t *idx_h,
                    int taps_h, const double *w_w, const int32_t *idx_w, int taps_w, void *out, void *ws, size_t ws_bytes);

int femasr_niqe_workspace_bytes(int B, int H, int W, int crop_border, size_t *bytes);
int femasr_niqe_plane_offsets(int B, int H, int W, int crop_border, size_t offsets[4]);
int femasr_niqe_features(void *stream, const uint8_t *img, int B, int H, int W, int crop_border, const double *window, const double *tables,
                         const double *w_h, const int32_t *idx_h, int taps_h, const double *w_w, const int32_t *idx_w, int taps_w,
                         double *features, int32_t *positions, void *ws, size_t ws_bytes);

#define FEMASR_CLOCK_PROBE_BLOCKS 256
int femasr_clock_probe(void *stream, int mfmas_per_wave, unsigned long long *ticks);
int femasr_clock_probe_entries(void);
#ifdef __cplusplus
}
#endif
#endif
```

include/femasr_hip_debug.h:

```cpp
#ifndef FEMASR_HIP_DEBUG_H
#define FEMASR_HIP_DEBUG_H
#include "femasr_hip.h"
#ifdef __cplusplus
extern "C" {
#endif

int femasr_debug_set_wino_limits(femasr_handle *h, int log2_total, int log2_image);

int femasr_debug_mfma_bf16(void *stream, const uint16_t *a, const uint16_t *b, const float *c, int n, float *d);

int femasr_gemm_force_config(int cfg);
int femasr_conv_small_launch_blocks(int blocks);

int femasr_debug_conv_variant_name(const femasr_conv_args *a, char *name, int cap);

#ifdef __cplusplus
}
#endif
#endif
```

Measured before the change: 67.52.

## Fuse output conv with crop and restrict last decoder conv to needed rectangle

```diff
diff --git a/femasr_amd/_lib.py b/femasr_amd/_lib.py
--- a/femasr_amd/_lib.py
+++ b/femasr_amd/_lib.py
@@ -33,10 +33,11 @@
         ('res1', vp), ('res2', vp), ('out', vp),
         ('Ho', ctypes.c_int32), ('Wo', ctypes.c_int32),
         ('w_bf16x3', vp), ('gn_part', vp), ('w_up2', vp), ('w_wino', vp), ('fast_act', ctypes.c_int32), ('in_add', vp), ('w_bf16s', vp),
+        ('need_h', ctypes.c_int32), ('need_w', ctypes.c_int32),
     ]
 
 
-ABI_VERSION = 106
+ABI_VERSION = 107
 PRO_NONE, PRO_GN_SILU, PRO_LN = 0, 1, 2
 ACT_NONE, ACT_GELU, ACT_RELU = 0, 1, 2
 
@@ -68,6 +69,7 @@
     'femasr_pad_nchw_to_nhwc': (c_int, [vp, vp, c_int, c_int, c_int, c_int, c_int, c_int, vp]),
     'femasr_crop_nhwc_to_nchw': (c_int, [vp, vp, c_int, c_int, c_int, c_int, c_int, c_int, vp]),
     'femasr_conv2d': (c_int, [vp, ctypes.POINTER(ConvArgs)]),
+    'femasr_out_conv_crop': (c_int, [vp, ctypes.POINTER(ConvArgs), c_int, c_int, c_int, c_int, vp]),
     'femasr_gn_coeffs': (c_int, [vp, vp, c_int, c_int, c_int, c_int, c_int, vp, vp, c_f32, vp, vp, vp]),
     'femasr_gn_coeffs_from_partials': (c_int, [vp, vp, c_int, c_int, c_int, c_int, c_int, c_int, vp, vp, c_f32, vp, vp]),
     'femasr_ln_stats': (c_int, [vp, vp, c_i64, c_int, c_f32, vp]),
@@ -136,6 +138,8 @@
     'femasr_gemm_force_config': (c_int, [c_int]),
     'femasr_conv_small_launch_blocks': (c_int, [c_int]),
     'femasr_debug_conv_variant_name': (c_int, [ctypes.POINTER(ConvArgs), ctypes.c_char_p, c_int]),
+    'femasr_debug_need_rect': (c_int, [c_int]),
+    'femasr_debug_wino_blocks': (c_int, [c_int, c_int, c_int, c_int, c_int, c_int]),
 }
 
 _lib = None
diff --git a/femasr_amd/csrc/common.h b/femasr_amd/csrc/common.h
--- a/femasr_amd/csrc/common.h
+++ b/femasr_amd/csrc/common.h
@@ -37,6 +37,9 @@
 };
 int femasr_conv2d_launch(hipStream_t s, const femasr_conv_args *a, const conv_vq_epilogue *vq,
                          int *variant_out, double *flops_out);
+bool femasr_conv_cout3_eligible(const femasr_conv_args *a);
+int femasr_conv_cout3_crop_launch(hipStream_t s, const femasr_conv_args *a, int crop_h, int crop_w, int out_u8, int swap_rb, void *out,
+                                  int *variant_out, double *flops_out);
 int femasr_conv2d_pick_variant(const femasr_conv_args *a);
 int femasr_conv_variant_count();
 const char *femasr_conv_variant_name(int v);
@@ -66,6 +69,7 @@
 bool femasr_conv_wino_shape_ok(const femasr_conv_args *a);
 bool femasr_conv_wino_shape_ok_lim(const femasr_conv_args *a, int log2_total, int log2_image);
 int femasr_conv_wino_gn_tiles(int H, int W);
+void femasr_conv_wino_used_subblocks(int H, int W, int need_h, int need_w, int *sbY, int *sbX);
 int femasr_conv_wino_launch(hipStream_t s, const femasr_conv_args *a, int *variant_out, double *flops_out);
 int femasr_conv_wino_variant_count();
 int femasr_conv_wino_pick_variant(const femasr_conv_args *a);
diff --git a/femasr_amd/csrc/conv_common.h b/femasr_amd/csrc/conv_common.h
--- a/femasr_amd/csrc/conv_common.h
+++ b/femasr_amd/csrc/conv_common.h
@@ -16,6 +16,9 @@
     int M, K, nchunks, taps, MB, NB, NT32;
     int tilesX, tilesY;
     int kperm;
+    int cropH, cropW;
+    int readH, readW;
+    int swap_rb;
 };
 
 constexpr int BK = 32;
diff --git a/femasr_amd/csrc/kernels_conv.hip b/femasr_amd/csrc/kernels_conv.hip
--- a/femasr_amd/csrc/kernels_conv.hip
+++ b/femasr_amd/csrc/kernels_conv.hip
@@ -1,4 +1,5 @@
 #include "conv_common.h"
+#include <algorithm>
 #include <atomic>
 #include <stdlib.h>
 #include <type_traits>
@@ -572,6 +573,7 @@
 
 constexpr int C3_TH = 8, C3_TW = 32, C3_PW = C3_TW + 2, C3_PP = (C3_TH + 2) * C3_PW, C3_PITCH = 36;
 
+template <int OUT>
 __global__ __launch_bounds__(256) void conv3x3_cout3_kernel(const ConvParams p, const float *__restrict__ wc)
 {
     extern __shared__ __attribute__((aligned(16))) float smem[];
@@ -592,7 +594,7 @@
     for (int i = 0; i < NU; ++i) {
         const int u = t + 256 * i, pix = u >> 3, kq = u & 7;
         const int sy = oy0 - 1 + pix / C3_PW, sx = ox0 - 1 + pix % C3_PW;
-        const bool ok = u < C3_PP * 8 && sy >= 0 && sy < p.H && sx >= 0 && sx < p.W;
+        const bool ok = u < C3_PP * 8 && sy >= 0 && sy < p.readH && sx >= 0 && sx < p.readW;
         uoff[i] = ok ? (unsigned)((((size_t)n * p.H + sy) * p.W + sx) * p.Cin + 4 * kq) : 0u;
         umask |= (ok ? 1u : 0u) << i;
     }
@@ -634,14 +636,30 @@
         }
     }
     const int oy = oy0 + py, ox = ox0 + px;
-    if (oy < p.Ho && ox < p.Wo) {
-        const size_t o = (((size_t)n * p.Ho + oy) * p.Wo + ox) * 3;
+    if (oy < p.cropH && ox < p.cropW) {
         float v[3] = {acc0 + p.bias[0], acc1 + p.bias[1], acc2 + p.bias[2]};
-#pragma unroll
-        for (int c = 0; c < 3; ++c) {
-            if (p.res1) v[c] = v[c] + p.res1[o + c];
-            if (p.res2) v[c] = v[c] + p.res2[o + c];
-            p.out[o + c] = v[c];
+        if (OUT == 0) {
+            const size_t o = (((size_t)n * p.Ho + oy) * p.Wo + ox) * 3;
+#pragma unroll
+            for (int c = 0; c < 3; ++c) {
+                if (p.res1) v[c] = v[c] + p.res1[o + c];
+                if (p.res2) v[c] = v[c] + p.res2[o + c];
+                p.out[o + c] = v[c];
+            }
+        } else if (OUT == 1) {
+            const size_t plane = (size_t)p.cropH * p.cropW;
+            float *dst = p.out + (size_t)n * 3 * plane + (size_t)oy * p.cropW + ox;
+#pragma unroll
+            for (int c = 0; c < 3; ++c) dst[c * plane] = v[c];
+        } else {
+            unsigned char *dst = reinterpret_cast<unsigned char *>(p.out) + (((size_t)n * p.cropH + oy) * p.cropW + ox) * 3;
+#pragma unroll
+            for (int c = 0; c < 3; ++c) {
+                float x = v[p.swap_rb ? 2 - c : c];
+                x = x < 0.f ? 0.f : (x > 1.f ? 1.f : x);
+                if (!(x == x)) x = 0.f;
+                dst[c] = (unsigned char)rintf(x * 255.0f);
+            }
         }
     }
 }
@@ -754,6 +772,27 @@
 {
     return femasr_conv_halo_eligible(a) && a->Cout == 3 && !a->up2 && a->prologue == FEMASR_PRO_NONE && a->act == FEMASR_ACT_NONE && !a->gn_part;
 }
+bool femasr_conv_cout3_eligible(const femasr_conv_args *a) { return conv_is_cout3(a) && !a->res1 && !a->res2; }
+
+static int cout3_launch(hipStream_t s, const femasr_conv_args *a, ConvParams p, int crop, int crop_h, int crop_w, int swap_rb, void *out)
+{
+    const float *wc = a->w + (size_t)p.nchunks * p.NT32 * 1024;
+    p.cropH = crop ? crop_h : p.Ho;
+    p.cropW = crop ? crop_w : p.Wo;
+    p.readH = std::min(p.H, p.cropH + 1);
+    p.readW = std::min(p.W, p.cropW + 1);
+    p.swap_rb = swap_rb;
+    if (crop) { p.out = (float *)out; p.res1 = p.res2 = nullptr; }
+    p.tilesX = (p.cropW + C3_TW - 1) / C3_TW;
+    p.tilesY = (p.cropH + C3_TH - 1) / C3_TH;
+    const dim3 grid((unsigned)(a->B * p.tilesX * p.tilesY));
+    const size_t lds = (size_t)C3_PP * C3_PITCH * sizeof(float);
+    if (crop == 0) hipLaunchKernelGGL(conv3x3_cout3_kernel<0>, grid, dim3(256), lds, s, p, wc);
+    else if (crop == 1) hipLaunchKernelGGL(conv3x3_cout3_kernel<1>, grid, dim3(256), lds, s, p, wc);
+    else hipLaunchKernelGGL(conv3x3_cout3_kernel<2>, grid, dim3(256), lds, s, p, wc);
+    FEMASR_CHECK_HIP(hipGetLastError());
+    return FEMASR_OK;
+}
 
 int femasr_conv2d_pick_variant(const femasr_conv_args *a)
 {
@@ -800,14 +839,7 @@
     p.gn_part = a->gn_part;
     p.kperm = (a->ksz == 1 && vec) ? 1 : 0;
     if (conv_is_cout3(a)) {
-        const size_t tail = femasr_compact_weight_floats(a->Cout, a->Cin, 3, 3);
-        const float *wc = a->w + (size_t)p.nchunks * p.NT32 * 1024;
-        p.tilesX = (Wo + C3_TW - 1) / C3_TW;
-        p.tilesY = (Ho + C3_TH - 1) / C3_TH;
-        (void)tail;
-        hipLaunchKernelGGL(conv3x3_cout3_kernel, dim3((unsigned)(a->B * p.tilesX * p.tilesY)), dim3(256), (size_t)C3_PP * C3_PITCH * sizeof(float), s,
-                           p, wc);
-        FEMASR_CHECK_HIP(hipGetLastError());
+        FEMASR_CHECK(cout3_launch(s, a, p, 0, 0, 0, 0, nullptr));
         if (variant_out) *variant_out = kNumVariants - 1;
         if (flops_out) *flops_out = 2.0 * (double)M * (double)a->Cout * (double)p.K;
         return FEMASR_OK;
@@ -833,3 +865,26 @@
     if (flops_out) *flops_out = 2.0 * (double)M * (double)a->Cout * (double)p.K;
     return FEMASR_OK;
 }
+
+int femasr_conv_cout3_crop_launch(hipStream_t s, const femasr_conv_args *a, int crop_h, int crop_w, int out_u8, int swap_rb, void *out,
+                                  int *variant_out, double *flops_out)
+{
+    FEMASR_REQUIRE(a && a->in && a->w && a->bias && out && a->B > 0 && a->H > 0 && a->W > 0 && a->Cin > 0, "out_conv_crop: null pointer or empty shape");
+    FEMASR_REQUIRE(a->ksz == 3 && a->stride == 1 && a->pad == 1 && a->Ho == a->H && a->Wo == a->W && femasr_conv_cout3_eligible(a),
+                   "out_conv_crop: needs a 3x3 stride-1 pad-1 conv with Cout = 3, Cin %% 32 == 0, fewer than 2^31 input elements, no prologue / activation / residuals");
+    FEMASR_REQUIRE(crop_h >= 1 && crop_h <= a->H && crop_w >= 1 && crop_w <= a->W, "out_conv_crop: crop %dx%d outside the %dx%d output", crop_h, crop_w, a->H, a->W);
+    FEMASR_REQUIRE((long long)a->B * a->H * a->W < (1ll << 31) - 256, "out_conv_crop: too many output pixels");
+    ConvParams p{};
+    p.in = a->in; p.w = a->w; p.bias = a->bias;
+    p.B = a->B; p.H = a->H; p.W = a->W; p.Cin = a->Cin; p.Cout = 3; p.ksz = 3; p.stride = 1; p.pad = 1; p.Ho = a->H; p.Wo = a->W;
+    p.K = 9 * a->Cin; p.nchunks = p.K / BK; p.taps = 9; p.NT32 = 1;
+    FEMASR_CHECK(cout3_launch(s, a, p, out_u8 ? 2 : 1, crop_h, crop_w, swap_rb ? 1 : 0, out));
+    if (variant_out) *variant_out = kNumVariants - 1;
+    if (flops_out) *flops_out = 2.0 * (double)a->B * crop_h * crop_w * 3.0 * (double)p.K;
+    return FEMASR_OK;
+}
+
+extern "C" int femasr_out_conv_crop(void *stream, const femasr_conv_args *a, int crop_h, int crop_w, int out_u8, int swap_rb, void *out)
+{
+    return femasr_conv_cout3_crop_launch((hipStream_t)stream, a, crop_h, crop_w, out_u8, swap_rb, out, nullptr, nullptr);
+}
diff --git a/femasr_amd/csrc/kernels_misc.hip b/femasr_amd/csrc/kernels_misc.hip
--- a/femasr_amd/csrc/kernels_misc.hip
+++ b/femasr_amd/csrc/kernels_misc.hip
@@ -1169,6 +1169,7 @@
 int femasr_conv_form_launch(hipStream_t s, ConvForm f, const femasr_conv_args *a, int *slot_out, double *flops_out)
 {
     int v = 0, r;
+    FEMASR_REQUIRE(!a || f == CONV_WINO || (!a->need_h && !a->need_w), "conv: only the Winograd F(4x4,3x3) form (w_wino, no up2) takes a need-rectangle");
     switch (f) {
     case CONV_BF16X3: r = femasr_conv_bf16x3_launch(s, a, &v, flops_out); break;
     case CONV_WINO: r = femasr_conv_wino_launch(s, a, &v, flops_out); break;
diff --git a/femasr_amd/csrc/kernels_wino.hip b/femasr_amd/csrc/kernels_wino.hip
--- a/femasr_amd/csrc/kernels_wino.hip
+++ b/femasr_amd/csrc/kernels_wino.hip
@@ -1,5 +1,6 @@
 #define FEMASR_WTT_BUF g_wi_ttbuf
 #include "wino_common.h"
+#include <algorithm>
 
 namespace {
 
@@ -465,6 +466,12 @@
 const char *femasr_conv_wino_variant_name(int v) { return v >= 0 && v < kNumW ? g_wv[v].name : "?"; }
 int femasr_conv_wino_gn_tiles(int H, int W) { return ((H + 15) / 16) * ((W + 15) / 16); }
 
+void femasr_conv_wino_used_subblocks(int H, int W, int need_h, int need_w, int *sbY, int *sbX)
+{
+    *sbY = ((need_h > 0 && need_h < H ? need_h : H) + 15) / 16;
+    *sbX = ((need_w > 0 && need_w < W ? need_w : W) + 15) / 16;
+}
+
 int femasr_conv_wino_pick_variant(const femasr_conv_args *a)
 {
     return 3 * (a->prologue == FEMASR_PRO_GN_SILU ? (a->fast_act ? 2 : 1) : 0) + (a->res1 ? (a->res2 ? 2 : 1) : 0);
@@ -481,8 +488,10 @@
     p.in = a->in; p.u = (const float *)a->w_wino; p.bias = a->bias; p.pro_a = a->pro_a; p.pro_b = a->pro_b;
     p.res1 = a->res1; p.res2 = a->res2; p.out = a->out; p.gn_part = a->gn_part;
     p.B = a->B; p.H = a->H; p.W = a->W; p.Cin = a->Cin; p.Cout = a->Cout;
-    p.sbX = (a->W + 15) / 16;
-    p.sbY = (a->H + 15) / 16;
+    FEMASR_REQUIRE(a->need_h >= 0 && a->need_h <= a->H && a->need_w >= 0 && a->need_w <= a->W,
+                   "conv_wino: need-rectangle %dx%d outside the %dx%d output", a->need_h, a->need_w, a->H, a->W);
+    FEMASR_REQUIRE(!(a->gn_part && (a->need_h || a->need_w)), "conv_wino: a need-rectangle cannot be combined with fused GroupNorm partials (gn_part)");
+    femasr_conv_wino_used_subblocks(a->H, a->W, a->need_h, a->need_w, &p.sbY, &p.sbX);
     p.nsb = a->B * p.sbX * p.sbY;
     p.MB = (p.nsb + 1) / 2;
     p.NB = a->Cout / 64;
@@ -497,11 +506,20 @@
     hipLaunchKernelGGL(v.kern, dim3((unsigned)(p.MB * p.NB)), dim3(W4_NT), lds, s, p);
     FEMASR_CHECK_HIP(hipGetLastError());
     if (variant_out) *variant_out = vi;
-    if (flops_out) *flops_out = 2.0 * (double)a->B * a->H * a->W * 9.0 * (double)a->Cin * (double)a->Cout;
+    if (flops_out) *flops_out = 2.0 * (double)a->B * std::min(a->H, 16 * p.sbY) * std::min(a->W, 16 * p.sbX) * 9.0 * (double)a->Cin * (double)a->Cout;
     return FEMASR_OK;
 }
 
 extern "C" {
+
+int femasr_debug_wino_blocks(int B, int H, int W, int Cout, int need_h, int need_w)
+{
+    if (B <= 0 || H <= 0 || W <= 0 || Cout <= 0 || (Cout % 64) != 0 || need_h < 0 || need_h > H || need_w < 0 || need_w > W) return -1;
+    int sbY = 0, sbX = 0;
+    femasr_conv_wino_used_subblocks(H, W, need_h, need_w, &sbY, &sbX);
+    const long long blocks = (((long long)B * sbY * sbX + 1) / 2) * (Cout / 64);
+    return blocks < (1ll << 31) ? (int)blocks : -1;
+}
 
 #ifdef FEMASR_WINO_TT
 int femasr_debug_wino_ttbuf(unsigned long long *dev_buf)
diff --git a/femasr_amd/csrc/model.hip b/femasr_amd/csrc/model.hip
--- a/femasr_amd/csrc/model.hip
+++ b/femasr_amd/csrc/model.hip
@@ -5,6 +5,7 @@
 
 #include <algorithm>
 #include <array>
+#include <atomic>
 #include <map>
 #include <string>
 #include <vector>
@@ -173,6 +174,9 @@
 
 namespace {
 
+std::atomic<int> g_need_rect{1};
+bool need_rect_enabled() { return g_need_rect.load(std::memory_order_relaxed) != 0; }
+
 enum { SLOT_GN = 0, SLOT_LN, SLOT_ATTN, SLOT_VQ, SLOT_LAYOUT, SLOT_SMALL_COUNT };
 const char *kSmallNames[SLOT_SMALL_COUNT] = {"gn_moments", "layernorm", "window_attention", "vq(codebook lookup)",
                                              "pad/crop/gather layout"};
@@ -392,6 +396,7 @@
         const float *res1 = nullptr, *res2 = nullptr;
         const float *in_add = nullptr;
         bool want_gn = false;
+        int need_h = 0, need_w = 0;
     };
     femasr_conv_args conv_args(const T &x, int cout, const ConvOpt &o) const
     {
@@ -411,6 +416,13 @@
         T y = alloc_t(x.B, a.Ho, a.Wo, cout);
         a.out = y.p;
         const ConvForm f = conv_form(h, h->modes, prefix, a);
+        double used = 1.0;
+        if (f == CONV_WINO && !o.want_gn && (o.need_h || o.need_w)) {
+            int sby = 0, sbx = 0;
+            femasr_conv_wino_used_subblocks(a.Ho, a.Wo, o.need_h, o.need_w, &sby, &sbx);
+            a.need_h = o.need_h; a.need_w = o.need_w;
+            used = (double)std::min(a.Ho, 16 * sby) * std::min(a.Wo, 16 * sbx) / ((double)a.Ho * a.Wo);
+        }
         if (o.in_add && f != CONV_WINO_UP2 && !rc)
             rc = femasr_set_error(FEMASR_ERR_INVALID, "conv %s: a second input was scheduled for a conv that does not run in the x2 Winograd-type form", prefix.c_str());
         float *act_tmp = (f == CONV_SPLIT && o.pro == FEMASR_PRO_GN_SILU) ? alloc_f(x.numel()) : nullptr;
@@ -449,7 +461,7 @@
         const int r = femasr_conv_form_launch(s(), f, &a, &slot, &flops);
         sc.set_slot(SLOT_SMALL_COUNT + slot);
         sc.set_flops(flops);
-        sc.set_bytes(4.0 * ((double)x.numel() * (o.in_add ? 2 : 1) + (double)y.numel() * (1 + (o.res1 ? 1 : 0) + (o.res2 ? 1 : 0)) +
+        sc.set_bytes(4.0 * (used * ((double)x.numel() * (o.in_add ? 2 : 1) + (double)y.numel() * (1 + (o.res1 ? 1 : 0) + (o.res2 ? 1 : 0))) +
                             (double)cout * x.C * o.ksz * o.ksz + cout));
         if (r && !rc) rc = r;
         release(act_tmp);
@@ -482,7 +494,7 @@
         return ab;
     }
 
-    T resblock(T x, const std::string &p, const float *res2, bool free_x, bool out_gn = false)
+    T resblock(T x, const std::string &p, const float *res2, bool free_x, bool out_gn = false, int need_h = 0, int need_w = 0)
     {
         const size_t bc = (size_t)x.B * x.C;
         float *ab = gn(x, p + ".conv.0.norm");
@@ -492,6 +504,7 @@
         float *ab2 = gn(u, p + ".conv.3.norm");
         ConvOpt o2; o2.pro = FEMASR_PRO_GN_SILU; o2.pa = ab2; o2.pb = ab2 ? ab2 + bc : nullptr;
         o2.res1 = x.p; o2.res2 = res2; o2.want_gn = out_gn;
+        if (!out_gn) { o2.need_h = need_h; o2.need_w = need_w; }
         T y = conv(u, p + ".conv.5", x.C, o2);
         release(ab2);
         release(u);
@@ -556,12 +569,31 @@
         return x;
     }
 
-    T up_block(const T &x, const std::string &p, int cout, const float *res2_last, const float *in_add = nullptr)
+    T up_block(const T &x, const std::string &p, int cout, const float *res2_last, const float *in_add = nullptr, int need_h = 0, int need_w = 0)
     {
         ConvOpt o; o.up2 = 1; o.want_gn = true; o.in_add = in_add;
         T c = conv(x, p + ".1", cout, o);
         T r1 = resblock(c, p + ".2", nullptr, true, true);
-        return resblock(r1, p + ".3", res2_last, true, false);
+        return resblock(r1, p + ".3", res2_last, true, false, need_h, need_w);
+    }
+
+    bool out_conv_crop(const T &x, int crop_h, int crop_w, void *out)
+    {
+        femasr_conv_args a = conv_args(x, 3, ConvOpt{});
+        if (conv_form(h, h->modes, "out_conv", a) != CONV_DIRECT || !femasr_conv_cout3_eligible(&a)) return false;
+        if (rc || dry()) return true;
+        a.w = Wt("out_conv.weight");
+        a.bias = Wt("out_conv.bias");
+        if (rc) return true;
+        Scope sc(h, s(), dry(), 0, 0.0, 0.0);
+        int v = 0; double flops = 0;
+        const int r = femasr_conv_cout3_crop_launch(s(), &a, crop_h, crop_w, (io_u8 & 2) ? 1 : 0, swap_rb, out, &v, &flops);
+        sc.set_slot(SLOT_SMALL_COUNT + v);
+        sc.set_flops(flops);
+        sc.set_bytes(4.0 * ((double)x.B * std::min(x.H, crop_h + 1) * std::min(x.W, crop_w + 1) * x.C + 27.0 * x.C + 3) +
+                     (double)x.B * crop_h * crop_w * 3.0 * ((io_u8 & 2) ? 1.0 : 4.0));
+        if (r && !rc) rc = r;
+        return true;
     }
 };
 
@@ -688,16 +720,24 @@
         const bool skip_by_next = next_skip && conv_form(h, h->modes, "decoder_group." + std::to_string(i + 1) + ".block.1",
                                                          c.conv_args(nx, channels_at(r * 4), ou)) == CONV_WINO_UP2;
         const float *skip = (next_skip && !skip_by_next) ? feats[i + 1].p : nullptr;
-        T y = c.up_block(x, "decoder_group." + std::to_string(i) + ".block", cout_i, skip, pending_add.p);
+        int need_h = 0, need_w = 0;
+        if (i + 1 == h->max_depth && need_rect_enabled()) {
+            need_h = std::min(2 * x.H, crop_h + 1);
+            need_w = std::min(2 * x.W, crop_w + 1);
+            if (need_h >= 2 * x.H && need_w >= 2 * x.W) need_h = need_w = 0;
+        }
+        T y = c.up_block(x, "decoder_group." + std::to_string(i) + ".block", cout_i, skip, pending_add.p, need_h, need_w);
         c.release(x);
         if (pending_add.p) { c.release(pending_add); pending_add = T{}; }
         if (next_skip) { if (skip_by_next) pending_add = feats[i + 1]; else c.release(feats[i + 1]); }
         x = y;
         prev_dec = x;
     }
-    T img = c.conv(x, "out_conv", 3, Ctx::ConvOpt{});
+    T img = c.alloc_t(x.B, x.H, x.W, 3);
+    const bool fused = c.out_conv_crop(x, crop_h, crop_w, out_nchw);
+    if (!fused) { c.release(img); img = c.conv(x, "out_conv", 3, Ctx::ConvOpt{}); }
     c.release(x);
-    if (!c.rc && !c.dry()) {
+    if (!fused && !c.rc && !c.dry()) {
         Scope sc(h, c.s(), c.dry(), SLOT_LAYOUT, 0.0, (double)img.B * 3.0 * crop_h * crop_w * 8.0);
         const int r = (c.io_u8 & 2) ? femasr_crop_nhwc_to_u8hwc(c.s(), img.p, img.B, img.H, img.W, crop_h, crop_w, c.swap_rb, (uint8_t *)out_nchw)
                                     : femasr_crop_nhwc_to_nchw(c.s(), img.p, img.B, img.H, img.W, 3, crop_h, crop_w, out_nchw);
@@ -801,7 +841,7 @@
 extern "C" {
 
 const char *femasr_last_error(void) { return g_err; }
-int femasr_version(void) { return 106; }
+int femasr_version(void) { return 107; }
 
 int femasr_create(const femasr_config *cfg, femasr_handle **out)
 {
@@ -1136,6 +1176,8 @@
     return FEMASR_OK;
 }
 
+int femasr_debug_need_rect(int on) { return g_need_rect.exchange(on ? 1 : 0, std::memory_order_relaxed); }
+
 int femasr_debug_set_wino_limits(femasr_handle *h, int log2_total, int log2_image)
 {
     FEMASR_REQUIRE(h && log2_total >= 0 && log2_total <= FEMASR_WINO_LOG2_TOTAL && log2_image >= 0 && log2_image <= FEMASR_WINO_LOG2_IMAGE,
diff --git a/include/femasr_hip.h b/include/femasr_hip.h
--- a/include/femasr_hip.h
+++ b/include/femasr_hip.h
@@ -100,8 +100,11 @@
     int32_t fast_act;
     const float *in_add;
     const void *w_bf16s;
+    int32_t need_h, need_w;
 } femasr_conv_args;
 int femasr_conv2d(void *stream, const femasr_conv_args *a);
+
+int femasr_out_conv_crop(void *stream, const femasr_conv_args *a, int crop_h, int crop_w, int out_u8, int swap_rb, void *out);
 
 size_t femasr_gn_scratch_bytes(int B, int H, int W, int C, int G);
 int femasr_gn_coeffs(void *stream, const float *x, int B, int H, int W, int C, int G,
diff --git a/include/femasr_hip_debug.h b/include/femasr_hip_debug.h
--- a/include/femasr_hip_debug.h
+++ b/include/femasr_hip_debug.h
@@ -14,6 +14,9 @@
 
 int femasr_debug_conv_variant_name(const femasr_conv_args *a, char *name, int cap);
 
+int femasr_debug_need_rect(int on);
+int femasr_debug_wino_blocks(int B, int H, int W, int Cout, int need_h, int need_w);
+
 #ifdef __cplusplus
 }
 #endif
```

New measurement: 67.74, median of 6. About the same (+0.3%).
